# SnowCheetos/CassMantle

Hardware: AMD Instinct MI355X
Metric: SD-1.5 512^2 50-step images/sec (whole node) + p50 guess-score latency (higher is better)
Workload: dtype bf16; 1 GPU; model=sd15 UNet/VAE/CLIP (512x512, 50 steps pndm, cfg 7.5), global_batch=4, seq_len=4096, parallelism=dp1 (rooms)

## Files before the change

### cassmantle_amd/models/layers.py

```python
from __future__ import annotations

import math
import os
from typing import Optional

import torch
import torch.nn as nn

from .. import ops


def _param(shape, std, gen: Optional[torch.Generator], dtype) -> nn.Parameter:
    t = torch.randn(*shape, generator=gen, dtype=torch.float32) * std
    return nn.Parameter(t.to(dtype), requires_grad=False)


def _zeros(shape, dtype) -> nn.Parameter:
    return nn.Parameter(torch.zeros(*shape, dtype=dtype), requires_grad=False)


def _ones(shape, dtype) -> nn.Parameter:
    return nn.Parameter(torch.ones(*shape, dtype=dtype), requires_grad=False)


_GN_FUSE = os.environ.get("CASSMANTLE_GN_FUSE", "1") != "0"
_UP2 = os.environ.get("CASSMANTLE_UP2", "1") != "0"


class StatsArena:

    def __init__(self) -> None:
        self._bufs: dict = {}
        self._need: dict = {}
        self.key = None
        self.buf: Optional[torch.Tensor] = None
        self.off = 0
        self.on = False

    def begin(self, key, x: torch.Tensor) -> "StatsArena":
        self.on = x.device.type == "cuda" and ops.get_mode() == "hip" and _GN_FUSE
        self.key, self.off = key, 0
        if not self.on:
            return self
        self.buf = self._bufs.get(key)
        need = self._need.get(key, 0)
        if need and self.buf is None:
            self.buf = self._bufs[key] = torch.empty(need, device=x.device, dtype=torch.int64)
        if self.buf is not None:
            ops.zero_(self.buf)
        self.device = x.device
        return self

    def take_rows(self, rows: int) -> Optional[torch.Tensor]:
        s = self.take(1, rows)
        return None if s is None else s.view(rows, 2)

    def take(self, B: int, C: int) -> Optional[torch.Tensor]:
        if not self.on:
            return None
        n = B * C * 2
        end = self.off + n
        if self.buf is not None and end <= self.buf.numel():
            s = self.buf[self.off:end].view(B, C, 2)
        else:
            self._need[self.key] = max(self._need.get(self.key, 0), end)
            s = ops.new_stats(B, C, self.device)
        self.off = end
        return s


class Linear(nn.Module):
    def __init__(self, fin: int, fout: int, bias: bool = True, gen=None, dtype=torch.bfloat16,
                 std: Optional[float] = None):
        super().__init__()
        self.fin, self.fout = fin, fout
        self.weight = _param((fout, fin), std if std is not None else 1.0 / math.sqrt(fin), gen, dtype)
        self.bias = _param((fout,), 0.02, gen, dtype) if bias else None

    def forward(self, x, residual=None, act=None, stats=None, row_stats=None):
        return ops.linear(x, self.weight, self.bias, residual=residual, act=act, stats=stats, row_stats=row_stats)


class Conv2d(nn.Module):

    def __init__(self, cin: int, cout: int, k: int = 3, stride: int = 1, padding: Optional[int] = None,
                 bias: bool = True, gen=None, dtype=torch.bfloat16):
        super().__init__()
        self.cin, self.cout, self.k, self.stride = cin, cout, k, stride
        self.padding = (k // 2) if padding is None else padding
        self.weight = _param((cout, k, k, cin), 1.0 / math.sqrt(cin * k * k), gen, dtype)
        self.bias = _param((cout,), 0.02, gen, dtype) if bias else None

    upsampling = False
    pad_in = 0

    def _derived(self, name: str, key, fn):
        buf = self._buffers.get(name)
        if buf is None or getattr(self, "_key_" + name, None) != key or buf.device != self.weight.device:
            self.register_buffer(name, fn(), persistent=False)
            setattr(self, "_key_" + name, key)
        return self._buffers[name]

    def up2_weights(self):
        return self._derived("w4", self.weight._version, lambda: ops.fold_upsample_weights(self.weight))

    def padded_weight(self, cin: int):
        return self._derived("wpad", (self.weight._version, cin),
                             lambda: torch.nn.functional.pad(self.weight, (0, cin - self.cin)).contiguous())

    def prepare(self) -> None:
        if self.upsampling and self.k == 3 and self.cin % 64 == 0:
            self.up2_weights()
        if self.pad_in > self.cin:
            self.padded_weight(self.pad_in)

    def forward(self, x, residual=None, upsample=False, chan_bias=None, stats=None, out=None):
        if out is not None:
            w = self.padded_weight(x.shape[-1]) if x.shape[-1] > self.cin else self.weight
            return ops.conv2d(x, w, self.bias, self.stride, self.padding, residual=residual,
                              upsample=upsample, chan_bias=chan_bias, stats=stats, out=out)
        if x.shape[-1] > self.cin:
            return ops.conv2d(x, self.padded_weight(x.shape[-1]), self.bias, self.stride, self.padding,
                              residual=residual, upsample=upsample, chan_bias=chan_bias, stats=stats)
        if upsample and self.k == 3 and self.stride == 1 and _UP2 and x.device.type == "cuda" \
                and ops.get_mode() == "hip" and self.cin % 64 == 0:
            return ops.conv2d_up2(x, self.weight, self.up2_weights(), self.bias, residual=residual,
                                  chan_bias=chan_bias, stats=stats)
        if self.k == 1 and self.stride == 1 and not upsample and chan_bias is None:
            return ops.linear(x, self.weight.view(self.cout, self.cin), self.bias, residual=residual, stats=stats)
        return ops.conv2d(x, self.weight, self.bias, self.stride, self.padding, residual=residual,
                          upsample=upsample, chan_bias=chan_bias, stats=stats)


class GroupNorm(nn.Module):
    def __init__(self, groups: int, channels: int, eps: float = 1e-5, dtype=torch.bfloat16):
        super().__init__()
        self.groups, self.eps = groups, eps
        self.weight = _ones((channels,), dtype)
        self.bias = _zeros((channels,), dtype)

    def forward(self, x, silu=False, stats=None, stats2=None):
        return ops.group_norm(x, self.groups, self.weight, self.bias, self.eps, silu, stats=stats, stats2=stats2)


class LayerNorm(nn.Module):
    def __init__(self, dim: int, eps: float = 1e-5, dtype=torch.bfloat16):
        super().__init__()
        self.eps = eps
        self.weight = _ones((dim,), dtype)
        self.bias = _zeros((dim,), dtype)

    def forward(self, x):
        return ops.layer_norm(x, self.weight, self.bias, self.eps)


class SelfAttention(nn.Module):

    def __init__(self, dim: int, heads: int, gen=None, dtype=torch.bfloat16, qkv_bias=False,
                 out_bias=True):
        super().__init__()
        self.dim, self.heads = dim, heads
        self.head_dim = dim // heads
        self.to_qkv = Linear(dim, 3 * dim, bias=qkv_bias, gen=gen, dtype=dtype)
        self.to_out = Linear(dim, dim, bias=out_bias, gen=gen, dtype=dtype)

    def forward(self, x, residual=None, causal=False, kv_lens=None, fp8=False, qkv=None, kv8=None,
                row_stats=None):
        if qkv is None:
            qkv = self.to_qkv(x)
        B, N = qkv.shape[0], qkv.shape[1]
        C = self.dim
        qkv = qkv.view(B, N, 3, self.heads, self.head_dim)
        if kv8 is not None:
            assert fp8 and kv_lens is None, "kv8: fp8 self-attention without key lengths"
            o = ops.attention(qkv[:, :, 0], qkv[:, :, 1], qkv[:, :, 2], causal=causal, fp8=True, kv8=kv8)
        else:
            o = ops.attention(qkv[:, :, 0], qkv[:, :, 1], qkv[:, :, 2], causal=causal, kv_lens=kv_lens, fp8=fp8)
        return self.to_out(o.reshape(B, N, C), residual=residual, row_stats=row_stats)


class CrossAttention(nn.Module):
    def __init__(self, dim: int, ctx_dim: int, heads: int, gen=None, dtype=torch.bfloat16):
        super().__init__()
        self.dim, self.heads = dim, heads
        self.head_dim = dim // heads
        self.to_q = Linear(dim, dim, bias=False, gen=gen, dtype=dtype)
        self.to_kv = Linear(ctx_dim, 2 * dim, bias=False, gen=gen, dtype=dtype)
        self.to_out = Linear(dim, dim, bias=True, gen=gen, dtype=dtype)

    _kv = None
    _kv8 = None

    def forward(self, x, ctx, residual=None, fp8=False, q=None, row_stats=None):
        if q is None:
            q = self.to_q(x)
        B, N = q.shape[0], q.shape[1]
        C = self.dim
        q = q.view(B, N, self.heads, self.head_dim)
        kv8 = None
        if self._kv is not None and self._kv.shape[0] == B:
            kv = self._kv.view(B, self._kv.shape[1], 2, self.heads, self.head_dim)
            kv8 = self._kv8 if fp8 else None
        else:
            kv = self.to_kv(ctx).view(B, ctx.shape[1], 2, self.heads, self.head_dim)
        o = ops.attention(q, kv[:, :, 0], kv[:, :, 1], fp8=fp8, kv8=kv8)
        return self.to_out(o.reshape(B, N, C), residual=residual, row_stats=row_stats)


class GEGLUFeedForward(nn.Module):
    def __init__(self, dim: int, mult: int = 4, gen=None, dtype=torch.bfloat16):
        super().__init__()
        inner = dim * mult
        self.proj_in = Linear(dim, 2 * inner, gen=gen, dtype=dtype)
        self.proj_out = Linear(inner, dim, gen=gen, dtype=dtype)

    def forward(self, x, residual=None):
        return self.proj_out(self.proj_in(x, act="geglu"), residual=residual)
```

### cassmantle_amd/models/unet.py

```python
from __future__ import annotations

import os
from dataclasses import dataclass, field
from typing import List, Optional, Sequence, Tuple

import torch
import torch.nn as nn

from .. import ops
from .layers import (Conv2d, CrossAttention, GEGLUFeedForward, GroupNorm, LayerNorm, Linear,
                     SelfAttention, StatsArena)


@dataclass
class UNetConfig:
    in_channels: int = 4
    out_channels: int = 4
    block_out_channels: Tuple[int, ...] = (320, 640, 1280, 1280)
    down_attn: Tuple[bool, ...] = (True, True, True, False)
    transformer_depth: Tuple[int, ...] = (1, 1, 1, 1)
    mid_transformer_depth: int = 1
    layers_per_block: int = 2
    heads: Tuple[int, ...] = (8, 8, 8, 8)
    head_dim: Optional[int] = None
    cross_attention_dim: int = 768
    norm_groups: int = 32
    norm_eps: float = 1e-5
    transformer_norm_eps: float = 1e-6
    time_proj_dim: int = 320
    time_embed_dim: int = 1280
    linear_projection: bool = False
    addition_embed: bool = False
    addition_time_embed_dim: int = 256
    projection_class_embeddings_input_dim: int = 2816
    sample_size: int = 64

    def level_heads(self, i: int) -> int:
        if self.head_dim is not None:
            return self.block_out_channels[i] // self.head_dim
        return self.heads[i]


SD15_UNET = UNetConfig()
SDXL_UNET = UNetConfig(block_out_channels=(320, 640, 1280), down_attn=(False, True, True),
                       transformer_depth=(0, 2, 10), mid_transformer_depth=10, heads=(5, 10, 20),
                       head_dim=64, cross_attention_dim=2048, linear_projection=True,
                       addition_embed=True, sample_size=128)
TINY_UNET = UNetConfig(block_out_channels=(32, 64), down_attn=(True, False), transformer_depth=(1, 1),
                       heads=(2, 2), layers_per_block=1, cross_attention_dim=32, norm_groups=8,
                       time_proj_dim=32, time_embed_dim=64, sample_size=8)


class ResnetBlock(nn.Module):
    def __init__(self, cin: int, cout: int, temb: int, groups: int, eps: float, gen, dtype):
        super().__init__()
        self.norm1 = GroupNorm(groups, cin, eps, dtype)
        self.conv1 = Conv2d(cin, cout, 3, gen=gen, dtype=dtype)
        self.time_emb_proj = Linear(temb, cout, gen=gen, dtype=dtype)
        self.norm2 = GroupNorm(groups, cout, eps, dtype)
        self.conv2 = Conv2d(cout, cout, 3, gen=gen, dtype=dtype)
        self.conv_shortcut = Conv2d(cin, cout, 1, padding=0, gen=gen, dtype=dtype) if cin != cout else None

    def forward(self, x, temb_silu, tb_all=None, arena: Optional[StatsArena] = None, xs=None, xs2=None):
        pair = isinstance(x, tuple)
        B = x[0].shape[0] if pair else x.shape[0]
        cout = self.conv1.cout
        if pair:
            g = self.norm1
            h = ops.group_norm_cat(x[0], x[1], g.groups, g.weight, g.bias, g.eps, True, stats=xs, stats2=xs2)
        else:
            h = self.norm1(x, silu=True, stats=xs, stats2=xs2)
        if tb_all is not None:
            tb = tb_all[:, self._tb_off:self._tb_off + self.time_emb_proj.fout]
        else:
            tb = self.time_emb_proj(temb_silu)
        s1 = arena.take(B, cout) if arena is not None else None
        h = self.conv1(h, chan_bias=tb, stats=s1)
        h = self.norm2(h, silu=True, stats=s1)
        if pair and self.conv_shortcut is None:
            sc = torch.cat(x, dim=-1)
        elif pair:
            cs = self.conv_shortcut
            sc = ops.linear_cat(x[0], x[1], cs.weight.view(cs.cout, cs.cin), cs.bias)
        else:
            sc = self.conv_shortcut(x) if self.conv_shortcut is not None else x
        s2 = arena.take(B, cout) if arena is not None else None
        return self.conv2(h, residual=sc, stats=s2), s2


_LN_FOLD = os.environ.get("CASSMANTLE_LN_FOLD", "1") == "1"
_LN_ROWSTATS = os.environ.get("CASSMANTLE_LN_ROWSTATS", "1") == "1"
_GN_FOLD = os.environ.get("CASSMANTLE_GN_FOLD", "1") == "1"
_FF_ROWSTATS = os.environ.get("CASSMANTLE_FF_ROWSTATS", "1") == "1"


def _row_stats_wanted(x: torch.Tensor) -> bool:
    return (_LN_ROWSTATS and x.device.type == "cuda" and ops.get_mode() == "hip" and ops.LN_FOLD_MODE == 1
            and x.shape[-1] not in (320, 640) and x.shape[-1] % 8 == 0 and x.numel() // x.shape[-1] >= 1024)


_FP8_KV_EPILOGUE = os.environ.get("CASSMANTLE_FP8_KV_EPILOGUE", "1") == "1"


class BasicTransformerBlock(nn.Module):
    def __init__(self, dim: int, heads: int, ctx_dim: int, gen, dtype):
        super().__init__()
        self.norm1 = LayerNorm(dim, 1e-5, dtype)
        self.attn1 = SelfAttention(dim, heads, gen=gen, dtype=dtype)
        self.norm2 = LayerNorm(dim, 1e-5, dtype)
        self.attn2 = CrossAttention(dim, ctx_dim, heads, gen=gen, dtype=dtype)
        self.norm3 = LayerNorm(dim, 1e-5, dtype)
        self.ff = GEGLUFeedForward(dim, 4, gen=gen, dtype=dtype)

    _folds = None

    def _fold_sources(self):
        return ((self.norm1, self.attn1.to_qkv), (self.norm2, self.attn2.to_q), (self.norm3, self.ff.proj_in))

    def folds(self):
        key = tuple((n.weight._version, None if n.bias is None else n.bias._version, l.weight._version,
                     None if l.bias is None else l.bias._version) for n, l in self._fold_sources())
        buf = self._buffers.get("fold0_w")
        if buf is None or self._fold_key != key or buf.device != self.norm1.weight.device:
            for i, (n, l) in enumerate(self._fold_sources()):
                for tag, t in zip(("w", "s", "b"), ops.ln_fold(n.weight, n.bias, l.weight, l.bias)):
                    self.register_buffer(f"fold{i}_{tag}", t, persistent=False)
            self._fold_key = key
        return tuple((self._buffers[f"fold{i}_w"], self._buffers[f"fold{i}_s"], self._buffers[f"fold{i}_b"])
                     for i in range(3))

    def forward(self, x, ctx, fp8=False, arena: Optional[StatsArena] = None, xrs=None, out_stats=False):
        if _LN_FOLD and x.device.type == "cuda" and ops.get_mode() == "hip":
            f = self.folds()
            n1, n2, n3 = self.norm1, self.norm2, self.norm3
            want = arena is not None and _row_stats_wanted(x)
            rows = x.numel() // x.shape[-1]
            kv8 = None
            if fp8 and _FP8_KV_EPILOGUE and ops.kv8_ok(x, self.attn1.head_dim):
                kv8 = ops.kv8_image(x.shape[0], x.shape[1], x.shape[2], x.device)
            qkv = ops.ln_linear(x, n1.weight, n1.bias, n1.eps, self.attn1.to_qkv.weight, fold=f[0], kv8=kv8,
                                row_stats=xrs if want else None)
            r2 = arena.take_rows(rows) if want else None
            x = self.attn1(None, residual=x, fp8=fp8, qkv=qkv, kv8=kv8, row_stats=r2)
            q = ops.ln_linear(x, n2.weight, n2.bias, n2.eps, self.attn2.to_q.weight, fold=f[1], row_stats=r2)
            r3 = arena.take_rows(rows) if want else None
            x = self.attn2(None, ctx, residual=x, fp8=fp8, q=q, row_stats=r3)
            h = ops.ln_linear(x, n3.weight, n3.bias, n3.eps, self.ff.proj_in.weight, act="geglu", fold=f[2],
                              row_stats=r3)
            r4 = arena.take_rows(rows) if (want and out_stats and _FF_ROWSTATS) else None
            return self.ff.proj_out(h, residual=x, row_stats=r4), r4
        x = self.attn1(self.norm1(x), residual=x, fp8=fp8)
        x = self.attn2(self.norm2(x), ctx, residual=x, fp8=fp8)
        x = self.ff(self.norm3(x), residual=x)
        return x, None


class Transformer2D(nn.Module):
    def __init__(self, dim: int, heads: int, depth: int, ctx_dim: int, groups: int, gen, dtype):
        super().__init__()
        self.norm = GroupNorm(groups, dim, 1e-6, dtype)
        self.proj_in = Linear(dim, dim, gen=gen, dtype=dtype)
        self.transformer_blocks = nn.ModuleList(
            [BasicTransformerBlock(dim, heads, ctx_dim, gen, dtype) for _ in range(depth)])
        self.proj_out = Linear(dim, dim, gen=gen, dtype=dtype)

    def forward(self, x, ctx, fp8=False, arena: Optional[StatsArena] = None, xs=None):
        B, H, W, C = x.shape
        hrs = None
        if (_GN_FOLD and xs is not None and C == 320 and (H * W) % 256 == 0 and x.device.type == "cuda"
                and ops.get_mode() == "hip"):
            n = self.norm
            h = ops.gn_linear(x.view(B, H * W, C), xs, n.weight, n.bias, n.groups, n.eps, self.proj_in.weight,
                              self.proj_in.bias)
        else:
            h = self.norm(x, stats=xs).view(B, H * W, C)
            hrs = arena.take_rows(B * H * W) if (arena is not None and _LN_FOLD and _row_stats_wanted(h)) else None
            h = self.proj_in(h, row_stats=hrs)
        rs = hrs
        nblk = len(self.transformer_blocks)
        for i, blk in enumerate(self.transformer_blocks):
            h, rs = blk(h, ctx, fp8=fp8, arena=arena, xrs=rs, out_stats=i + 1 < nblk)
        so = arena.take(B, C) if arena is not None else None
        return self.proj_out(h, residual=x.view(B, H * W, C), stats=so).view(B, H, W, C), so


class Downsample(nn.Module):
    def __init__(self, c: int, gen, dtype):
        super().__init__()
        self.conv = Conv2d(c, c, 3, stride=2, padding=1, gen=gen, dtype=dtype)

    def forward(self, x, arena: Optional[StatsArena] = None):
        so = arena.take(x.shape[0], self.conv.cout) if arena is not None else None
        return self.conv(x, stats=so), so


class Upsample(nn.Module):
    def __init__(self, c: int, gen, dtype):
        super().__init__()
        self.conv = Conv2d(c, c, 3, gen=gen, dtype=dtype)
        self.conv.upsampling = True

    def forward(self, x, arena: Optional[StatsArena] = None):
        so = arena.take(x.shape[0], self.conv.cout) if arena is not None else None
        return self.conv(x, upsample=True, stats=so), so


class UNet(nn.Module):
    def __init__(self, cfg: UNetConfig = SD15_UNET, seed: int = 0, dtype=torch.bfloat16):
        super().__init__()
        self.cfg = cfg
        gen = torch.Generator().manual_seed(seed)
        ch = cfg.block_out_channels
        g, eps, te = cfg.norm_groups, cfg.norm_eps, cfg.time_embed_dim
        self.conv_in = Conv2d(cfg.in_channels, ch[0], 3, gen=gen, dtype=dtype)
        self.conv_in.pad_in = 8 if cfg.in_channels % 8 else 0
        self.time_linear_1 = Linear(cfg.time_proj_dim, te, gen=gen, dtype=dtype)
        self.time_linear_2 = Linear(te, te, gen=gen, dtype=dtype)
        if cfg.addition_embed:
            self.add_linear_1 = Linear(cfg.projection_class_embeddings_input_dim, te, gen=gen, dtype=dtype)
            self.add_linear_2 = Linear(te, te, gen=gen, dtype=dtype)
        self.down = nn.ModuleList()
        skip_ch: List[int] = [ch[0]]
        cur = ch[0]
        n = len(ch)
        for i in range(n):
            blk = nn.Module()
            blk.resnets = nn.ModuleList()
            blk.attentions = nn.ModuleList()
            for j in range(cfg.layers_per_block):
                blk.resnets.append(ResnetBlock(cur, ch[i], te, g, eps, gen, dtype))
                cur = ch[i]
                if cfg.down_attn[i]:
                    blk.attentions.append(Transformer2D(cur, cfg.level_heads(i), cfg.transformer_depth[i],
                                                       cfg.cross_attention_dim, g, gen, dtype))
                skip_ch.append(cur)
            blk.downsampler = Downsample(cur, gen, dtype) if i < n - 1 else None
            if i < n - 1:
                skip_ch.append(cur)
            self.down.append(blk)
        self.mid_res1 = ResnetBlock(cur, cur, te, g, eps, gen, dtype)
        self.mid_attn = Transformer2D(cur, cfg.level_heads(n - 1), cfg.mid_transformer_depth,
                                      cfg.cross_attention_dim, g, gen, dtype)
        self.mid_res2 = ResnetBlock(cur, cur, te, g, eps, gen, dtype)
        self.up = nn.ModuleList()
        rev = list(reversed(range(n)))
        for ui, i in enumerate(rev):
            blk = nn.Module()
            blk.resnets = nn.ModuleList()
            blk.attentions = nn.ModuleList()
            for j in range(cfg.layers_per_block + 1):
                sk = skip_ch.pop()
                blk.resnets.append(ResnetBlock(cur + sk, ch[i], te, g, eps, gen, dtype))
                cur = ch[i]
                if cfg.down_attn[i]:
                    blk.attentions.append(Transformer2D(cur, cfg.level_heads(i), cfg.transformer_depth[i],
                                                       cfg.cross_attention_dim, g, gen, dtype))
            blk.upsampler = Upsample(cur, gen, dtype) if ui < n - 1 else None
            self.up.append(blk)
        self.conv_norm_out = GroupNorm(g, cur, eps, dtype)
        self.conv_out = Conv2d(cur, cfg.out_channels, 3, gen=gen, dtype=dtype)
        self._arena = StatsArena()

    def time_embed(self, t: torch.Tensor, added: Optional[dict] = None) -> torch.Tensor:
        dt = self.time_linear_1.weight.dtype
        tp = ops.timestep_embedding(t, self.cfg.time_proj_dim, out_dtype=dt)
        h = self.time_linear_1(tp, act="silu")
        if not (self.cfg.addition_embed and added is not None):
            return self.time_linear_2(h, act="silu")
        emb = self.time_linear_2(h)
        tid = added["time_ids"]
        B = tid.shape[0]
        te = ops.timestep_embedding(tid.reshape(-1), self.cfg.addition_time_embed_dim).reshape(B, -1)
        a_in = ops.concat_last(added["text_embeds"], te)
        emb = self.add_linear_2(self.add_linear_1(a_in, act="silu"), residual=emb)
        return ops.silu_(emb)

    def resnets(self) -> List[ResnetBlock]:
        return [m for m in self.modules() if isinstance(m, ResnetBlock)]

    def cross_attns(self) -> List[CrossAttention]:
        ca = self.__dict__.get("_ca_list")
        if ca is None:
            ca = self.__dict__["_ca_list"] = [m for m in self.modules() if isinstance(m, CrossAttention)]
        return ca

    def fuse_projections(self) -> None:
        rs = self.resnets()
        off = 0
        for r in rs:
            r._tb_off = off
            off += r.time_emb_proj.fout
        self.register_buffer("_tb_w", torch.cat([r.time_emb_proj.weight for r in rs], 0).contiguous(), persistent=False)
        self.register_buffer("_tb_b", torch.cat([r.time_emb_proj.bias for r in rs], 0).contiguous(), persistent=False)
        ca = self.cross_attns()
        off = 0
        for m in ca:
            m._kv_off = off
            off += m.to_kv.fout
        self.register_buffer("_kv_w", torch.cat([m.to_kv.weight for m in ca], 0).contiguous() if ca else None,
                             persistent=False)
        self._kv_bufs: dict = {}
        self._fused = True

    def prepare(self) -> "UNet":
        self.fuse_projections()
        for m in self.modules():
            if isinstance(m, BasicTransformerBlock):
                m.folds()
            elif isinstance(m, Conv2d):
                m.prepare()
        return self

    def set_context(self, ctx: Optional[torch.Tensor], fp8: bool = False) -> None:
        if not getattr(self, "_fused", False):
            self.fuse_projections()
        ca = self.cross_attns()
        if ctx is None or self._kv_w is None:
            for m in ca:
                m._kv = None
                m._kv8 = None
            return
        key = (*ctx.shape[:-1], self._kv_w.shape[0])
        buf = self._kv_bufs.get(key)
        if buf is None or buf.device != ctx.device:
            self._kv_bufs[key] = buf = ops.linear(ctx, self._kv_w)
        else:
            ops.linear(ctx, self._kv_w, out=buf)
        for m in ca:
            m._kv = buf[:, :, m._kv_off:m._kv_off + m.to_kv.fout]
            m._kv8 = None
            if fp8 and m.head_dim == 64 and ops._use_hip(buf):
                bufs8 = m.__dict__.setdefault("_kv8_bufs", {})
                kv = m._kv.view(buf.shape[0], buf.shape[1], 2, m.heads, m.head_dim)
                k8 = (key, str(buf.device))
                bufs8[k8] = m._kv8 = ops.pack_kv_fp8(kv[:, :, 0], kv[:, :, 1], out=bufs8.get(k8))

    def time_table(self, tsteps: torch.Tensor, nb: int, added: Optional[dict] = None,
                   t_rep: Optional[torch.Tensor] = None, rep_ids: Optional[torch.Tensor] = None):
        if not getattr(self, "_fused", False):
            self.fuse_projections()
        E = tsteps.shape[0]
        t = t_rep if t_rep is not None else tsteps.float().repeat_interleave(nb)
        rep = None
        if added is not None:
            if rep_ids is not None and ops._use_hip(added["text_embeds"]):
                rep = {"text_embeds": ops.gather_add(added["text_embeds"], rep_ids),
                       "time_ids": added["time_ids_rep"] if "time_ids_rep" in added
                       else added["time_ids"].repeat(E, 1)}
            else:
                rep = {k: v.repeat(E, *([1] * (v.dim() - 1))) for k, v in added.items() if k != "time_ids_rep"}
        temb = self.time_embed(t, rep)
        tb = ops.linear(temb, self._tb_w, self._tb_b)
        return temb.view(E, nb, -1), tb.view(E, nb, -1)

    def forward(self, x: torch.Tensor, t: Optional[torch.Tensor], ctx: torch.Tensor,
                added: Optional[dict] = None, fp8: bool = False, time_cond=None,
                out: Optional[torch.Tensor] = None) -> torch.Tensor:
        if not getattr(self, "_fused", False):
            self.fuse_projections()
        if time_cond is not None:
            temb, tb = time_cond
        else:
            temb = self.time_embed(t, added)
            tb = ops.linear(temb, self._tb_w, self._tb_b)
        ar = self._arena.begin(tuple(x.shape), x)
        B = x.shape[0]
        hs = ar.take(B, self.conv_in.cout)
        h = self.conv_in(x, stats=hs)
        skips = [(h, hs)]
        for blk in self.down:
            for j, res in enumerate(blk.resnets):
                h, hs = res(h, temb, tb, ar, hs)
                if len(blk.attentions):
                    h, hs = blk.attentions[j](h, ctx, fp8, ar, hs)
                skips.append((h, hs))
            if blk.downsampler is not None:
                h, hs = blk.downsampler(h, ar)
                skips.append((h, hs))
        h, hs = self.mid_res1(h, temb, tb, ar, hs)
        h, hs = self.mid_attn(h, ctx, fp8, ar, hs)
        h, hs = self.mid_res2(h, temb, tb, ar, hs)
        for blk in self.up:
            for j, res in enumerate(blk.resnets):
                sk, sks = skips.pop()
                two = hs is not None and sks is not None
                h, hs = res((h, sk), temb, tb, ar, hs if two else None, sks if two else None)
                if len(blk.attentions):
                    h, hs = blk.attentions[j](h, ctx, fp8, ar, hs)
            if blk.upsampler is not None:
                h, hs = blk.upsampler(h, ar)
        h = self.conv_norm_out(h, silu=True, stats=hs)
        return self.conv_out(h, out=out)


def _silu(x: torch.Tensor) -> torch.Tensor:
    return torch.nn.functional.silu(x.float()).to(x.dtype)
```

### cassmantle_amd/ops/__init__.py

```python
from __future__ import annotations

import math
import os
import weakref
from typing import List, Optional

import torch

from . import reference as ref
from ._ext import ext, ext_available, ext_error

_MODE = os.environ.get("CASSMANTLE_OPS", "hip").lower()


def set_mode(mode: str) -> None:
    global _MODE
    assert mode in ("hip", "torch")
    _MODE = mode


def get_mode() -> str:
    return _MODE


def _use_hip(t: torch.Tensor) -> bool:
    if t.device.type != "cuda":
        return False
    if _MODE == "torch":
        return False
    if not ext_available():
        raise RuntimeError(
            "cassmantle_amd HIP extension is not loaded on a GPU device "
            f"({ext_error()}); run `python -m cassmantle_amd.build` or set CASSMANTLE_OPS=torch "
            "explicitly for the stock-PyTorch baseline")
    return True


_TUNE_PATH = os.path.join(os.path.dirname(os.path.abspath(__file__)), "gemm_tuning.json")
_RECORD: Optional[list] = None
_tune_loaded = False
_DIAG_TWICE = os.environ.get("CASSMANTLE_DIAG_TWICE", "0") == "1"
if _DIAG_TWICE and os.environ.get("CASSMANTLE_DIAG_TWICE_ACK") != "wrong-results":
    raise RuntimeError("CASSMANTLE_DIAG_TWICE=1 makes every GEMM / conv result WRONG (epilogue "
                       "statistics and residuals applied twice); it is a timing diagnostic for "
                       "tools/diag_twice.py only: also set CASSMANTLE_DIAG_TWICE_ACK=wrong-results")


def load_gemm_tuning(path: Optional[str] = None) -> int:
    global _tune_loaded
    if os.environ.get("CASSMANTLE_GEMM_TUNE", "1") == "0" or not ext_available():
        return 0
    if _tune_loaded and path is None:
        return ext().gemm_tune_size()
    import json
    p = path or os.environ.get("CASSMANTLE_GEMM_TUNE_PATH") or _TUNE_PATH
    _tune_loaded = True
    if not os.path.exists(p):
        return 0
    with open(p) as f:
        data = json.load(f)
    for e in data.get("entries", []):
        ext().gemm_tune_set(e["key"], int(e["cfg"]), int(e["split"]))
    return ext().gemm_tune_size()


def record_gemms(on: bool) -> Optional[list]:
    global _RECORD
    if on:
        _RECORD = []
        ext().gemm_record_keys(True)
        return _RECORD
    rec, _RECORD = _RECORD, None
    ext().gemm_record_keys(False)
    return rec


_PF_SERIAL = os.environ.get("CASSMANTLE_PF_SERIAL", "0") == "1"


def _launch(fn, *args, **kw):
    if not _tune_loaded:
        load_gemm_tuning()
    if _PF_SERIAL:
        prefetch(args[2] if fn is ext().gemm_cat else args[1])
    if _DIAG_TWICE:
        fn(*args, **kw)
    fn(*args, **kw)
    if _RECORD is not None:
        call = lambda: fn(*args, **kw)
        call.fn, call.args, call.kw = fn, args, kw
        _RECORD.append((ext().gemm_last_key(), call))


_ACT = {None: 0, "none": 0, "gelu": 1, "silu": 2, "quick_gelu": 3, "geglu": 4, "gelu_tanh": 5, "swiglu": 6}


STAT_SCALE = (2.0 ** 24, 2.0 ** 16)


def h2d(t: torch.Tensor, device) -> torch.Tensor:
    device = torch.device(device)
    if device.type != "cuda":
        return t.to(device)
    return t.pin_memory().to(device, non_blocking=True)


def new_stats(B: int, C: int, device) -> torch.Tensor:
    return zero_(torch.empty((B, C, 2), device=device, dtype=torch.int64))


def stats_to_float(stats: torch.Tensor) -> torch.Tensor:
    sc = torch.tensor([1.0 / STAT_SCALE[0], 1.0 / STAT_SCALE[1]], dtype=torch.float64, device=stats.device)
    return stats.double() * sc


def channel_stats_ref(y: torch.Tensor, stats: torch.Tensor) -> None:
    B, C = y.shape[0], y.shape[-1]
    yf = y.reshape(B, -1, C).double()
    stats[..., 0] += torch.round(yf.sum(1) * STAT_SCALE[0]).to(torch.int64)
    stats[..., 1] += torch.round((yf * yf).sum(1) * STAT_SCALE[1]).to(torch.int64)


def channel_stats(y: torch.Tensor, stats: torch.Tensor) -> None:
    if _use_hip(y):
        ext().channel_stats(y.contiguous(), stats)
    else:
        channel_stats_ref(y, stats)


def linear(x: torch.Tensor, w: torch.Tensor, bias: Optional[torch.Tensor] = None,
           residual: Optional[torch.Tensor] = None, act: Optional[str] = None,
           stats: Optional[torch.Tensor] = None, out: Optional[torch.Tensor] = None,
           row_stats: Optional[torch.Tensor] = None) -> torch.Tensor:
    if not _use_hip(x):
        if x.device.type == "cuda":
            y = _torch_linear(x, w, bias, residual, act)
        else:
            y = ref.linear(x, w, bias, residual, act)
        if stats is not None:
            channel_stats_ref(y, stats)
        return y if out is None else out.copy_(y)
    K = x.shape[-1]
    x2 = x.reshape(-1, K)
    if not x2.is_contiguous():
        x2 = x2.contiguous()
    N = w.shape[0] // 2 if act in ("geglu", "swiglu") else w.shape[0]
    if out is None:
        out = torch.empty((x2.shape[0], N), device=x.device, dtype=x.dtype)
    else:
        assert out.is_contiguous() and out.dtype == x.dtype and out.numel() == x2.shape[0] * N, "linear: bad out"
    o2 = out.view(x2.shape[0], N)
    r2 = residual.reshape(-1, N) if residual is not None else None
    hw = x2.shape[0] // x.shape[0] if stats is not None else 0
    if row_stats is not None:
        _launch(ext().gemm, x2, w, bias, r2, o2, _ACT[act], stats, hw, row_stats=row_stats)
    else:
        _launch(ext().gemm, x2, w, bias, r2, o2, _ACT[act], stats, hw)
    return out.view(*x.shape[:-1], N)


def gn_linear(x: torch.Tensor, stats: torch.Tensor, gamma: torch.Tensor, beta: torch.Tensor, groups: int,
              eps: float, w: torch.Tensor, bias: Optional[torch.Tensor] = None,
              residual: Optional[torch.Tensor] = None) -> torch.Tensor:
    B, C = x.shape[0], x.shape[-1]
    if not _use_hip(x):
        xn = group_norm(x, groups, gamma, beta, eps, False, stats=stats)
        return linear(xn, w, bias, residual=residual)
    rows = x.numel() // C
    x2 = x.reshape(rows, C)
    if not x2.is_contiguous():
        x2 = x2.contiguous()
    N = w.shape[0]
    out = torch.empty((rows, N), device=x.device, dtype=x.dtype)
    r2 = residual.reshape(rows, N) if residual is not None else None
    _launch(ext().gemm, x2, w, bias, r2, out, 0, None, 0, gn_stats=stats, gn_gamma=gamma, gn_beta=beta,
            gn_groups=int(groups), gn_hw=rows // B, gn_eps=float(eps))
    return out.reshape(*x.shape[:-1], N)


def ln_fold(ln_weight: torch.Tensor, ln_bias: Optional[torch.Tensor], w: torch.Tensor,
            bias: Optional[torch.Tensor] = None):
    wf = (w.float() * ln_weight.float()[None, :]).to(w.dtype).contiguous()
    wsum = wf.float().sum(1).contiguous()
    b = torch.zeros(w.shape[0], device=w.device, dtype=torch.float32)
    if ln_bias is not None:
        b = b + w.float() @ ln_bias.float()
    if bias is not None:
        b = b + bias.float()
    return wf, wsum, b.to(w.dtype).contiguous()


def row_stats(x: torch.Tensor, eps: float) -> torch.Tensor:
    if not _use_hip(x):
        xf = x.float().reshape(-1, x.shape[-1])
        mean = xf.mean(-1)
        var = xf.var(-1, unbiased=False)
        return torch.stack([mean, (var + eps).rsqrt()], dim=-1)
    out = torch.empty((x.numel() // x.shape[-1], 2), device=x.device, dtype=torch.float32)
    ext().row_stats(x.contiguous(), out, float(eps))
    return out


LN_FOLD_MODE = int(os.environ.get("CASSMANTLE_LN_FOLD_MODE", "1"))


def ln_linear(x: torch.Tensor, ln_weight: torch.Tensor, ln_bias: Optional[torch.Tensor], eps: float,
              w: torch.Tensor, bias: Optional[torch.Tensor] = None, residual: Optional[torch.Tensor] = None,
              act: Optional[str] = None, fold=None, kv8: Optional[torch.Tensor] = None,
              row_stats: Optional[torch.Tensor] = None) -> torch.Tensor:
    K = x.shape[-1]
    rows = x.numel() // K
    if fold is None or not _use_hip(x) or rows <= 8 or K % 8 or (LN_FOLD_MODE == 2 and K not in (320, 640)):
        y = linear(layer_norm(x, ln_weight, ln_bias, eps), w, bias, residual=residual, act=act)
        if kv8 is not None:
            _pack_qkv8(y, kv8)
        return y
    wf, wsum, bf = fold
    x2 = x.reshape(rows, K)
    if not x2.is_contiguous():
        x2 = x2.contiguous()
    N = wf.shape[0] // 2 if act in ("geglu", "swiglu") else wf.shape[0]
    out = torch.empty((rows, N), device=x.device, dtype=x.dtype)
    r2 = residual.reshape(rows, N) if residual is not None else None
    fx = {"ln_rows_fx": row_stats} if row_stats is not None else {}
    if kv8 is not None:
        C = N // 3
        _launch(ext().gemm, x2, wf, bf, r2, out, _ACT[act], None, 0, None, wsum, float(eps), kv8, C,
                int(x.shape[-2]), C // 64, **fx)
    elif fx:
        _launch(ext().gemm, x2, wf, bf, r2, out, _ACT[act], None, 0, None, wsum, float(eps), **fx)
    else:
        _launch(ext().gemm, x2, wf, bf, r2, out, _ACT[act], None, 0, None, wsum, float(eps))
    return out.reshape(*x.shape[:-1], N)


def kv8_image(B: int, N: int, C: int, device) -> torch.Tensor:
    return torch.empty(2 * B * N * C, device=device, dtype=torch.uint8)


def kv8_ok(x: torch.Tensor, head_dim: int) -> bool:
    return (_use_hip(x) and x.dim() == 3 and head_dim == 64 and x.shape[1] % 64 == 0 and x.shape[-1] % 64 == 0
            and x.shape[-1] not in (320, 640))


def _pack_qkv8(y: torch.Tensor, kv8: torch.Tensor) -> None:
    B, N, C3 = y.shape
    C = C3 // 3
    qkv = y.view(B, N, 3, C // 64, 64)
    pack_kv_fp8(qkv[:, :, 1], qkv[:, :, 2], out=kv8)


def linear_cat(x: torch.Tensor, x2: torch.Tensor, w: torch.Tensor, bias: Optional[torch.Tensor] = None,
               residual: Optional[torch.Tensor] = None, stats: Optional[torch.Tensor] = None) -> torch.Tensor:
    Ca, K = x.shape[-1], x.shape[-1] + x2.shape[-1]
    rows = x.numel() // Ca
    if not _use_hip(x) or Ca % 64 or K % 64 or rows <= 8:
        return linear(torch.cat([x, x2], dim=-1), w, bias, residual=residual, stats=stats)
    N = w.shape[0]
    out = torch.empty((rows, N), device=x.device, dtype=x.dtype)
    r2 = residual.reshape(rows, N) if residual is not None else None
    hw = rows // x.shape[0] if stats is not None else 0
    _launch(ext().gemm_cat, x.reshape(rows, Ca).contiguous(), x2.reshape(rows, K - Ca).contiguous(), w, bias, r2, out,
            stats, hw)
    return out.reshape(*x.shape[:-1], N)


def _torch_linear(x, w, bias, residual, act):
    import torch.nn.functional as F
    y = F.linear(x, w, bias)
    if act == "geglu":
        h, g = y.chunk(2, dim=-1)
        y = h * F.gelu(g)
    elif act == "swiglu":
        h, g = y.chunk(2, dim=-1)
        y = h * F.silu(g)
    elif act == "gelu":
        y = F.gelu(y)
    elif act == "gelu_tanh":
        y = F.gelu(y, approximate="tanh")
    elif act == "silu":
        y = F.silu(y)
    elif act == "quick_gelu":
        y = y * torch.sigmoid(1.702 * y)
    if residual is not None:
        y = y + residual
    return y


def conv2d(x: torch.Tensor, w: torch.Tensor, bias: Optional[torch.Tensor] = None, stride: int = 1,
           padding: int = 1, residual: Optional[torch.Tensor] = None, upsample: bool = False,
           chan_bias: Optional[torch.Tensor] = None, stats: Optional[torch.Tensor] = None,
           out: Optional[torch.Tensor] = None) -> torch.Tensor:
    if not _use_hip(x):
        if x.device.type == "cuda":
            y = _torch_conv(x, w, bias, stride, padding, residual, upsample, chan_bias)
        else:
            y = ref.conv2d(x, w, bias, stride, padding, residual, upsample, chan_bias)
        if stats is not None:
            channel_stats_ref(y, stats)
        return y if out is None else out.copy_(y)
    B, H, W, Cin = x.shape
    Cout, kh, kw, _ = w.shape
    if Cin % 8 != 0:
        pad = 8 - Cin % 8
        x = torch.nn.functional.pad(x, (0, pad))
        w = torch.nn.functional.pad(w, (0, pad))
        Cin += pad
    Hi, Wi = (2 * H, 2 * W) if upsample else (H, W)
    Ho = (Hi + 2 * padding - kh) // stride + 1
    Wo = (Wi + 2 * padding - kw) // stride + 1
    if out is None:
        out = torch.empty((B, Ho, Wo, Cout), device=x.device, dtype=x.dtype)
    else:
        assert out.shape == (B, Ho, Wo, Cout) and out.dtype == x.dtype and out.is_contiguous(), "conv2d: bad out"
    _launch(ext().conv2d, x.contiguous(), w, bias, residual, chan_bias, out, stride, padding, int(upsample), stats)
    return out


_UP2_ROWS = ([[1.0, 0.0, 0.0], [0.0, 1.0, 1.0]], [[1.0, 1.0, 0.0], [0.0, 0.0, 1.0]])


def fold_upsample_weights(w: torch.Tensor) -> torch.Tensor:
    wf = w.float()
    outs = []
    for a in (0, 1):
        ra = torch.tensor(_UP2_ROWS[a], device=w.device)
        for b in (0, 1):
            rb = torch.tensor(_UP2_ROWS[b], device=w.device)
            outs.append(torch.einsum("tk,sl,oklc->otsc", ra, rb, wf))
    return torch.stack(outs).to(w.dtype).contiguous()


def conv2d_up2(x: torch.Tensor, w: torch.Tensor, w4: Optional[torch.Tensor] = None,
               bias: Optional[torch.Tensor] = None, residual: Optional[torch.Tensor] = None,
               chan_bias: Optional[torch.Tensor] = None, stats: Optional[torch.Tensor] = None) -> torch.Tensor:
    B, H, W, Cin = x.shape
    if not _use_hip(x) or Cin % 64 or w.shape[1] != 3:
        return conv2d(x, w, bias, 1, 1, residual=residual, upsample=True, chan_bias=chan_bias, stats=stats)
    if w4 is None:
        w4 = fold_upsample_weights(w)
    out = torch.empty((B, 2 * H, 2 * W, w.shape[0]), device=x.device, dtype=x.dtype)
    _launch(ext().conv2d_up2, x.contiguous(), w4, bias, residual, chan_bias, out, stats)
    return out


def _torch_conv(x, w, bias, stride, padding, residual, upsample, chan_bias):
    import torch.nn.functional as F
    xi = x.permute(0, 3, 1, 2)
    if upsample:
        xi = F.interpolate(xi, scale_factor=2.0, mode="nearest")
    wi = w.permute(0, 3, 1, 2)
    y = F.conv2d(xi.contiguous(memory_format=torch.channels_last),
                 wi.contiguous(memory_format=torch.channels_last), bias, stride=stride, padding=padding)
    y = y.permute(0, 2, 3, 1)
    if chan_bias is not None:
        y = y + chan_bias[:, None, None, :]
    if residual is not None:
        y = y + residual
    return y.contiguous()


def _group_norm_from_stats_ref(x, num_groups, weight, bias, eps, silu, stats):
    B, C = x.shape[0], x.shape[-1]
    S = x.numel() // (B * C)
    st = stats_to_float(stats).view(B, num_groups, C // num_groups, 2).sum(2)
    n = S * (C // num_groups)
    mean = st[..., 0] / n
    var = (st[..., 1] / n - mean * mean).clamp_min(0)
    rstd = (var + eps).rsqrt()
    cg = C // num_groups
    mean_c = mean.repeat_interleave(cg, 1).float()
    rstd_c = rstd.repeat_interleave(cg, 1).float()
    shape = [B] + [1] * (x.dim() - 2) + [C]
    y = (x.float() - mean_c.view(shape)) * rstd_c.view(shape) * weight.float() + bias.float()
    if silu:
        y = torch.nn.functional.silu(y)
    return y.to(x.dtype)


def group_norm(x: torch.Tensor, num_groups: int, weight: torch.Tensor, bias: torch.Tensor,
               eps: float, silu: bool = False, stats: Optional[torch.Tensor] = None,
               stats2: Optional[torch.Tensor] = None) -> torch.Tensor:
    if stats is not None:
        if not _use_hip(x):
            st = stats if stats2 is None else torch.cat([stats, stats2], dim=1)
            return _group_norm_from_stats_ref(x, num_groups, weight, bias, eps, silu, st)
        out = torch.empty_like(x)
        ext().group_norm_stats(x.contiguous(), stats, stats2, weight, bias, out, num_groups, float(eps), int(silu))
        return out
    if not _use_hip(x):
        if x.device.type == "cuda":
            import torch.nn.functional as F
            B, C = x.shape[0], x.shape[-1]
            xi = x.reshape(B, -1, C).transpose(1, 2)
            y = F.group_norm(xi, num_groups, weight, bias, eps)
            if silu:
                y = F.silu(y)
            return y.transpose(1, 2).reshape(x.shape).contiguous()
        return ref.group_norm(x, num_groups, weight, bias, eps, silu)
    out = torch.empty_like(x)
    ext().group_norm(x.contiguous(), weight, bias, out, num_groups, float(eps), int(silu))
    return out


def group_norm_cat(x: torch.Tensor, x2: torch.Tensor, num_groups: int, weight: torch.Tensor, bias: torch.Tensor,
                   eps: float, silu: bool = False, stats: Optional[torch.Tensor] = None,
                   stats2: Optional[torch.Tensor] = None) -> torch.Tensor:
    if stats is None or stats2 is None or not _use_hip(x) or x.shape[-1] % 8 or x2.shape[-1] % 8:
        return group_norm(torch.cat([x, x2], dim=-1), num_groups, weight, bias, eps, silu, stats=stats, stats2=stats2)
    out = torch.empty((*x.shape[:-1], x.shape[-1] + x2.shape[-1]), device=x.device, dtype=x.dtype)
    ext().group_norm_cat(x.contiguous(), x2.contiguous(), stats, stats2, weight, bias, out, num_groups, float(eps),
                         int(silu))
    return out


def layer_norm(x: torch.Tensor, weight: torch.Tensor, bias: Optional[torch.Tensor], eps: float) -> torch.Tensor:
    if not _use_hip(x):
        if x.device.type == "cuda":
            import torch.nn.functional as F
            return F.layer_norm(x, (x.shape[-1],), weight, bias, eps)
        return ref.layer_norm(x, weight, bias, eps)
    out = torch.empty_like(x)
    ext().layer_norm(x.contiguous(), weight, bias, out, float(eps))
    return out


def embed_layer_norm(word: torch.Tensor, ids: torch.Tensor, pos: torch.Tensor, add: Optional[torch.Tensor],
                     weight: torch.Tensor, bias: Optional[torch.Tensor], eps: float) -> torch.Tensor:
    B, T = ids.shape
    if not _use_hip(word):
        x = word[ids] + pos[:T][None]
        if add is not None:
            x = x + add
        return layer_norm(x, weight, bias, eps)
    out = torch.empty((B, T, word.shape[-1]), device=word.device, dtype=word.dtype)
    ext().embed_layer_norm(word, ids.contiguous().view(-1), pos, T, add, weight, bias, out, float(eps))
    return out


def rms_norm(x: torch.Tensor, weight: torch.Tensor, eps: float) -> torch.Tensor:
    if not _use_hip(x):
        return ref.rms_norm(x, weight, eps)
    out = torch.empty_like(x)
    ext().rms_norm(x.contiguous(), weight, out, float(eps))
    return out


def rms_linear(x: torch.Tensor, gamma: torch.Tensor, eps: float, w: torch.Tensor,
               bias: Optional[torch.Tensor] = None, residual: Optional[torch.Tensor] = None,
               act: Optional[str] = None) -> torch.Tensor:
    K = x.shape[-1]
    rows = x.numel() // K
    if not _use_hip(x) or rows > 8 or K % 8:
        return linear(rms_norm(x, gamma, eps), w, bias, residual=residual, act=act)
    x2 = x.reshape(rows, K)
    if not x2.is_contiguous():
        x2 = x2.contiguous()
    N = w.shape[0] // 2 if act in ("geglu", "swiglu") else w.shape[0]
    out = torch.empty((rows, N), device=x.device, dtype=x.dtype)
    r2 = residual.reshape(rows, N) if residual is not None else None
    ext().gemm_rms(x2, gamma, float(eps), w, bias, r2, out, _ACT[act])
    return out.reshape(*x.shape[:-1], N)


def rope_kv(qkv: torch.Tensor, pos0: torch.Tensor, q_out: torch.Tensor, k_cache: torch.Tensor,
            v_cache: torch.Tensor, heads: int, kv_heads: int, theta: float) -> None:
    if not _use_hip(qkv):
# ... 597 lines not shown
```

### cassmantle_amd/ops/csrc/bindings.cpp

```cpp
#include <torch/extension.h>
#include <atomic>
#include <ATen/hip/HIPContext.h>
#include <c10/hip/HIPStream.h>
#include <hip/hip_ext.h>

#include "gemm_tiles.h"
#include "jpeg_layout.h"
#include "kernels.h"

namespace {

hipStream_t cur_stream() { return c10::hip::getCurrentHIPStream().stream(); }

#define CHECK_DEV(t) TORCH_CHECK((t).is_cuda(), #t " must be a GPU tensor")
#define CHECK_BF16(t) TORCH_CHECK((t).scalar_type() == at::kBFloat16, #t " must be bf16")
#define CHECK_CONTIG(t) TORCH_CHECK((t).is_contiguous(), #t " must be contiguous")

const uint16_t* bptr(const at::Tensor& t) { return reinterpret_cast<const uint16_t*>(t.data_ptr()); }
uint16_t* bptr_mut(at::Tensor& t) { return reinterpret_cast<uint16_t*>(t.data_ptr()); }
const uint16_t* opt_bptr(const c10::optional<at::Tensor>& t) {
  if (!t.has_value() || !t->defined()) return nullptr;
  CHECK_DEV(*t);
  CHECK_BF16(*t);
  CHECK_CONTIG(*t);
  return bptr(*t);
}

long long* opt_stats(const c10::optional<at::Tensor>& t, long long images, int N) {
  if (!t.has_value() || !t->defined()) return nullptr;
  CHECK_DEV(*t);
  CHECK_CONTIG(*t);
  TORCH_CHECK(t->scalar_type() == at::kLong && t->numel() == images * N * 2,
              "stats must be a zeroed int64 fixed-point [images, N, 2] tensor (ops.new_stats)");
  return reinterpret_cast<long long*>(t->data_ptr<int64_t>());
}

static std::atomic<int> g_raster[2] = {{-1}, {-1}};
static void raster_from_env() {
  static const bool once = [] {
    const char* e = getenv("CASSMANTLE_GEMM_RASTER");
    int a = 0, b = -1;
    if (e != nullptr) {
      if (sscanf(e, "%d,%d", &a, &b) < 2) b = a;
    } else {
      b = 0;
    }
    int expect = -1;
    g_raster[0].compare_exchange_strong(expect, a);
    expect = -1;
    g_raster[1].compare_exchange_strong(expect, b);
    return true;
  }();
  (void)once;
}
void gemm_set_raster(int64_t plain, int64_t gated) {
  raster_from_env();
  g_raster[0].store((int)plain);
  g_raster[1].store((int)gated);
}

void run_gemm(GemmArgs& p, const at::Tensor& like) {
  raster_from_env();
  p.raster = g_raster[(p.act == 4 || p.act == 6) ? 1 : 0].load(std::memory_order_relaxed);
  TORCH_CHECK(p.stats == nullptr || (p.N % 8 == 0 && p.ldc == p.N),
              "gemm/conv2d stats: the output channel count must be a multiple of 8 (GroupNorm consumers)");
  const GemmPlan plan = gemm_plan(p);
  p.cfg = plan.cfg;
  p.split = plan.split;
  if (p.kv8 != nullptr) p.split = 1;
  long long* post_stats = nullptr;
  if (p.stats != nullptr && (p.out_f32 || p.M <= 8 || (p.batch != 1 && !p.parity) || p.act == 4 || p.act == 6)) {
    post_stats = p.stats;
    p.stats = nullptr;
  }
  if (p.split > 1) {
    auto ws = at::empty({(long long)p.split * p.batch * p.M * p.N}, like.options().dtype(at::kFloat));
    launch_gemm(p, ws.data_ptr<float>(), cur_stream());
  } else {
    launch_gemm(p, nullptr, cur_stream());
  }
  if (post_stats != nullptr)
    launch_channel_stats(reinterpret_cast<const uint16_t*>(p.C), post_stats, p.M / p.stats_hw, p.stats_hw, p.N,
                         cur_stream());
}

void gemm(const at::Tensor& x, const at::Tensor& w, const c10::optional<at::Tensor>& bias,
          const c10::optional<at::Tensor>& residual, at::Tensor& out, int64_t act,
          const c10::optional<at::Tensor>& stats, int64_t stats_hw,
          const c10::optional<at::Tensor>& ln_rows, const c10::optional<at::Tensor>& ln_wsum, double ln_eps,
          const c10::optional<at::Tensor>& kv8, int64_t kv8_col0, int64_t kv8_ntok, int64_t kv8_hk,
          const c10::optional<at::Tensor>& ln_rows_fx, const c10::optional<at::Tensor>& row_stats,
          const c10::optional<at::Tensor>& gn_stats, const c10::optional<at::Tensor>& gn_gamma,
          const c10::optional<at::Tensor>& gn_beta, int64_t gn_groups, int64_t gn_hw, double gn_eps) {
  CHECK_DEV(x); CHECK_BF16(x); CHECK_BF16(w); CHECK_CONTIG(w); CHECK_CONTIG(out);
  TORCH_CHECK(x.dim() == 2 && w.dim() == 2 && out.dim() == 2, "gemm: 2-D operands expected");
  TORCH_CHECK(x.stride(1) == 1, "gemm: x rows must be contiguous");
  GemmArgs p;
  p.A = bptr(x); p.W = bptr(w); p.bias = opt_bptr(bias); p.residual = opt_bptr(residual);
  p.M = (int)x.size(0); p.K = (int)x.size(1); p.N = (int)out.size(1); p.Nw = (int)w.size(0);
  p.lda = (int)x.stride(0); p.ldc = p.N; p.act = (int)act;
  TORCH_CHECK(w.size(1) == p.K, "gemm: K mismatch");
  TORCH_CHECK(out.size(0) == p.M, "gemm: M mismatch");
  if (act == 4 || act == 6) {
    TORCH_CHECK(p.Nw == 2 * p.N && p.K % 8 == 0 && (p.N % 4 == 0 || (p.M >= 1 && p.M <= 8 && p.lda % 8 == 0)),
                "geglu/swiglu: W must be [2N,K], K%8==0, N%4==0 (any N for <= 8 rows with lda%8==0)");
  } else {
    TORCH_CHECK(p.Nw == p.N, "gemm: N mismatch");
  }
  if (residual.has_value() && residual->defined()) TORCH_CHECK(residual->numel() == out.numel(), "gemm: residual shape");
  if (out.scalar_type() == at::kFloat) {
    p.out_f32 = 1;
  } else {
    CHECK_BF16(out);
  }
  p.C = out.data_ptr();
  if (kv8.has_value() && kv8->defined()) {
    CHECK_DEV(*kv8); CHECK_CONTIG(*kv8);
    TORCH_CHECK(kv8->scalar_type() == at::kByte && kv8_ntok > 0 && kv8_ntok % 64 == 0 && p.M % kv8_ntok == 0 &&
                    kv8_hk > 0 && kv8_col0 % 8 == 0 && kv8_col0 + 128 * kv8_hk == p.N && act == 0 &&
                    !p.out_f32 && !(residual.has_value() && residual->defined()) && !(stats.has_value() && stats->defined()),
                "gemm kv8: uint8 image, 64-aligned tokens per image, K|V heads ending the output, plain epilogue");
    TORCH_CHECK(kv8->numel() == 2LL * p.M * kv8_hk * 64, "gemm kv8: image size");
    p.kv8 = kv8->data_ptr<uint8_t>();
    p.kv8_col0 = (int)kv8_col0; p.kv8_ntok = (int)kv8_ntok; p.kv8_hk = (int)kv8_hk;
  }
  if (stats.has_value() && stats->defined()) {
    TORCH_CHECK(stats_hw > 0 && p.M % stats_hw == 0, "gemm: stats_hw must divide the rows");
    p.stats_hw = (int)stats_hw;
    p.stats = opt_stats(stats, p.M / stats_hw, p.N);
  }
  if (gn_stats.has_value() && gn_stats->defined()) {
    TORCH_CHECK(gn_gamma.has_value() && gn_beta.has_value() && gn_groups > 0 && gn_hw > 0 && p.M % gn_hw == 0,
                "gemm: gn_stats needs gamma, beta, groups and rows per image");
    CHECK_DEV(*gn_stats); CHECK_CONTIG(*gn_stats);
    TORCH_CHECK(gn_stats->scalar_type() == at::kLong && gn_stats->numel() == 2LL * (p.M / gn_hw) * p.K,
                "gemm: gn_stats int64 [images, K, 2]");
    TORCH_CHECK(!(ln_wsum.has_value() && ln_wsum->defined()) && !(row_stats.has_value() && row_stats->defined()) &&
                    !(kv8.has_value() && kv8->defined()) && !(stats.has_value() && stats->defined()),
                "gemm: gn_stats excludes LayerNorm folds, row / GroupNorm output statistics and kv8");
    p.gn_stats = reinterpret_cast<const long long*>(gn_stats->data_ptr<int64_t>());
    p.gn_gamma = opt_bptr(gn_gamma);
    p.gn_beta = opt_bptr(gn_beta);
    p.gn_groups = (int)gn_groups;
    p.gn_hw = (int)gn_hw;
    p.gn_eps = (float)gn_eps;
    if (gemm_areg_ok(p)) {
      run_gemm(p, out);
      return;
    }
    TORCH_CHECK(x.is_contiguous() && p.K % 8 == 0 && p.K % gn_groups == 0, "gemm gn fallback: contiguous rows");
    at::Tensor xn = at::empty_like(x);
    launch_group_norm_cs(bptr(x), nullptr, p.gn_stats, p.K, nullptr, p.gn_gamma, p.gn_beta, bptr_mut(xn),
                         p.M / gn_hw, gn_hw, p.K, (int)gn_groups, (float)gn_eps, 0, cur_stream());
    p.gn_stats = nullptr; p.gn_gamma = nullptr; p.gn_beta = nullptr;
    p.A = bptr(xn);
    run_gemm(p, out);
    return;
  }
  if (row_stats.has_value() && row_stats->defined()) {
    CHECK_DEV(*row_stats); CHECK_CONTIG(*row_stats);
    TORCH_CHECK(row_stats->scalar_type() == at::kLong && row_stats->numel() == 2LL * p.M,
                "gemm: row_stats zeroed int64 [M, 2]");
    TORCH_CHECK(p.stats == nullptr && p.kv8 == nullptr && !p.out_f32 && p.batch == 1 && p.M > 8 && p.N % 8 == 0 &&
                    p.ldc % 8 == 0 && p.K % 8 == 0 && p.lda % 8 == 0,
                "gemm: row_stats needs the LDS-staged bf16 epilogue (no GroupNorm stats / kv8, N % 8 == 0, M > 8)");
    p.row_stats = reinterpret_cast<long long*>(row_stats->data_ptr<int64_t>());
  }
  if (ln_rows_fx.has_value() && ln_rows_fx->defined()) {
    TORCH_CHECK(ln_wsum.has_value() && ln_wsum->defined() && ln_eps > 0 && !(ln_rows.has_value() && ln_rows->defined()),
                "gemm: ln_rows_fx needs ln_wsum and ln_eps, and excludes ln_rows");
    CHECK_DEV(*ln_rows_fx); CHECK_CONTIG(*ln_rows_fx); CHECK_DEV(*ln_wsum); CHECK_CONTIG(*ln_wsum);
    TORCH_CHECK(ln_rows_fx->scalar_type() == at::kLong && ln_rows_fx->numel() == 2LL * p.M, "gemm: ln_rows_fx int64 [M, 2]");
    TORCH_CHECK(ln_wsum->scalar_type() == at::kFloat && ln_wsum->numel() == p.Nw, "gemm: ln_wsum fp32 [Nw]");
    TORCH_CHECK(p.M > 8 && p.K % 8 == 0 && p.lda % 8 == 0 && !p.out_f32, "gemm: folded LayerNorm needs the MFMA path");
    p.ln_rows_fx = reinterpret_cast<const long long*>(ln_rows_fx->data_ptr<int64_t>());
    p.ln_wsum = ln_wsum->data_ptr<float>();
    p.ln_eps = (float)ln_eps;
    run_gemm(p, out);
    return;
  }
  if (ln_rows.has_value() && ln_rows->defined()) {
    TORCH_CHECK(ln_wsum.has_value() && ln_wsum->defined(), "gemm: ln_rows needs ln_wsum");
    CHECK_DEV(*ln_rows); CHECK_CONTIG(*ln_rows); CHECK_DEV(*ln_wsum); CHECK_CONTIG(*ln_wsum);
    TORCH_CHECK(ln_rows->scalar_type() == at::kFloat && ln_rows->numel() == 2LL * p.M, "gemm: ln_rows fp32 [M, 2]");
    TORCH_CHECK(ln_wsum->scalar_type() == at::kFloat && ln_wsum->numel() == p.Nw, "gemm: ln_wsum fp32 [Nw]");
    TORCH_CHECK(p.M > 8 && p.K % 8 == 0 && p.lda % 8 == 0, "gemm: folded LayerNorm needs the MFMA path (M > 8)");
    TORCH_CHECK(!p.out_f32 || p.act == 0, "gemm: folded LayerNorm with fp32 output supports no activation");
    p.ln_rows = ln_rows->data_ptr<float>();
    p.ln_wsum = ln_wsum->data_ptr<float>();
  } else if (ln_wsum.has_value() && ln_wsum->defined() && ln_eps > 0) {
    CHECK_DEV(*ln_wsum); CHECK_CONTIG(*ln_wsum);
    TORCH_CHECK(ln_wsum->scalar_type() == at::kFloat && ln_wsum->numel() == p.Nw, "gemm: ln_wsum fp32 [Nw]");
    TORCH_CHECK(p.M > 8 && p.K % 8 == 0 && p.lda % 8 == 0 && !p.out_f32, "gemm: folded LayerNorm needs the MFMA path");
    p.ln_wsum = ln_wsum->data_ptr<float>();
    p.ln_eps = (float)ln_eps;
    static const bool inkernel = [] { const char* e = getenv("CASSMANTLE_LN_INKERNEL"); return !(e && e[0] == '0'); }();
    if (!inkernel || !gemm_areg_ok(p)) {
      TORCH_CHECK(x.is_contiguous() && p.K <= 4096, "gemm: folded LayerNorm row statistics need contiguous rows");
      at::Tensor rows = at::empty({p.M, 2}, x.options().dtype(at::kFloat));
      launch_row_stats(bptr(x), rows.data_ptr<float>(), p.M, p.K, (float)ln_eps, cur_stream());
      p.ln_rows = rows.data_ptr<float>();
      p.ln_eps = 0.f;
      run_gemm(p, out);
      return;
    }
  }
  run_gemm(p, out);
}

void row_stats(const at::Tensor& x, at::Tensor& out, double eps) {
  CHECK_DEV(x); CHECK_BF16(x); CHECK_CONTIG(x); CHECK_CONTIG(out);
  const int D = (int)x.size(-1);
  TORCH_CHECK(D % 8 == 0 && D <= 4096, "row_stats: D % 8 == 0 and D <= 4096");
  TORCH_CHECK(out.scalar_type() == at::kFloat && out.numel() == 2 * (x.numel() / D), "row_stats: out fp32 [rows, 2]");
  launch_row_stats(bptr(x), out.data_ptr<float>(), x.numel() / D, D, (float)eps, cur_stream());
}

void gemm_cat(const at::Tensor& x, const at::Tensor& x2, const at::Tensor& w, const c10::optional<at::Tensor>& bias,
              const c10::optional<at::Tensor>& residual, at::Tensor& out, const c10::optional<at::Tensor>& stats,
              int64_t stats_hw) {
  CHECK_DEV(x); CHECK_BF16(x); CHECK_CONTIG(x); CHECK_BF16(x2); CHECK_CONTIG(x2); CHECK_BF16(w); CHECK_CONTIG(w);
  CHECK_BF16(out); CHECK_CONTIG(out);
  TORCH_CHECK(x.dim() == 2 && x2.dim() == 2 && w.dim() == 2 && out.dim() == 2 && x.size(0) == x2.size(0),
              "gemm_cat: 2-D operands with equal rows expected");
  GemmArgs p;
  p.A = bptr(x); p.A2 = bptr(x2); p.W = bptr(w); p.bias = opt_bptr(bias); p.residual = opt_bptr(residual);
  p.M = (int)x.size(0); p.ka = (int)x.size(1); p.K = p.ka + (int)x2.size(1);
  p.N = (int)out.size(1); p.Nw = (int)w.size(0);
  p.lda = p.ka; p.lda2 = (int)x2.size(1); p.ldc = p.N;
  TORCH_CHECK(w.size(1) == p.K && p.Nw == p.N && out.size(0) == p.M, "gemm_cat: shape mismatch");
  TORCH_CHECK(p.ka % 64 == 0 && p.K % 64 == 0 && p.M > 8, "gemm_cat: Ca and K must be multiples of 64, M > 8");
  const long long lim = (1LL << 31) - 1;
  TORCH_CHECK(x.numel() * 2 <= lim && x2.numel() * 2 <= lim && w.numel() * 2 <= lim, "gemm_cat: operand too large");
  if (residual.has_value() && residual->defined()) TORCH_CHECK(residual->numel() == out.numel(), "gemm_cat: residual shape");
  p.C = out.data_ptr();
  if (stats.has_value() && stats->defined()) {
    TORCH_CHECK(stats_hw > 0 && p.M % stats_hw == 0, "gemm_cat: stats_hw must divide the rows");
    p.stats_hw = (int)stats_hw;
    p.stats = opt_stats(stats, p.M / stats_hw, p.N);
  }
  run_gemm(p, out);
}

void gemm_rms(const at::Tensor& x, const at::Tensor& gamma, double eps, const at::Tensor& w,
              const c10::optional<at::Tensor>& bias, const c10::optional<at::Tensor>& residual, at::Tensor& out,
              int64_t act) {
  CHECK_DEV(x); CHECK_BF16(x); CHECK_BF16(gamma); CHECK_CONTIG(gamma); CHECK_BF16(w); CHECK_CONTIG(w);
  CHECK_CONTIG(out);
  TORCH_CHECK(x.dim() == 2 && x.stride(1) == 1 && x.size(0) <= 8, "gemm_rms: x [<=8, K] rows contiguous");
  GemmArgs p;
  p.A = bptr(x); p.W = bptr(w); p.bias = opt_bptr(bias); p.residual = opt_bptr(residual);
  p.M = (int)x.size(0); p.K = (int)x.size(1); p.N = (int)out.size(1); p.Nw = (int)w.size(0);
  p.lda = (int)x.stride(0); p.ldc = p.N; p.act = (int)act;
  p.rms_gamma = bptr(gamma); p.rms_eps = (float)eps;
  TORCH_CHECK(gamma.numel() == p.K && w.size(1) == p.K, "gemm_rms: K mismatch");
  TORCH_CHECK(p.Nw == ((act == 4 || act == 6) ? 2 * p.N : p.N), "gemm_rms: N mismatch");
  if (out.scalar_type() == at::kFloat) p.out_f32 = 1;
  else CHECK_BF16(out);
  p.C = out.data_ptr();
  TORCH_CHECK(launch_gemv(p, cur_stream()), "gemm_rms: shape not supported by the GEMV path (K % 8)");
}

void conv2d(const at::Tensor& x, const at::Tensor& w, const c10::optional<at::Tensor>& bias,
            const c10::optional<at::Tensor>& residual, const c10::optional<at::Tensor>& chan_bias, at::Tensor& out,
            int64_t stride, int64_t pad, int64_t upsample, const c10::optional<at::Tensor>& stats) {
  CHECK_DEV(x); CHECK_BF16(x); CHECK_CONTIG(x); CHECK_BF16(w); CHECK_CONTIG(w); CHECK_CONTIG(out); CHECK_BF16(out);
  TORCH_CHECK(x.dim() == 4 && w.dim() == 4 && out.dim() == 4, "conv2d: NHWC 4-D tensors expected");
  GemmArgs p;
  p.conv = 1;
  p.A = bptr(x); p.W = bptr(w); p.bias = opt_bptr(bias); p.residual = opt_bptr(residual);
  if (chan_bias.has_value() && chan_bias->defined()) {
    CHECK_DEV(*chan_bias);
    CHECK_BF16(*chan_bias);
    TORCH_CHECK(chan_bias->dim() == 2 && chan_bias->stride(1) == 1, "conv2d: chan_bias must be [B, Cout] rows");
    p.chan_bias = bptr(*chan_bias);
    p.ldcb = (int)chan_bias->stride(0);
  }
  p.IH = (int)x.size(1); p.IW = (int)x.size(2); p.Cin = (int)x.size(3);
  p.ksize = (int)w.size(1);
  TORCH_CHECK(w.size(2) == p.ksize && w.size(3) == p.Cin, "conv2d: weight must be [Cout,k,k,Cin]");
  p.Ho = (int)out.size(1); p.Wo = (int)out.size(2);
  p.N = (int)out.size(3); p.Nw = (int)w.size(0);
  TORCH_CHECK(p.Nw == p.N && out.size(0) == x.size(0), "conv2d: shape mismatch");
  p.M = (int)(x.size(0) * p.Ho * p.Wo);
  p.K = p.ksize * p.ksize * p.Cin;
  p.lda = p.Cin; p.ldc = p.N;
  p.stride = (int)stride; p.pad = (int)pad; p.upsample = (int)upsample;
  if (residual.has_value() && residual->defined()) TORCH_CHECK(residual->numel() == out.numel(), "conv2d: residual shape");
  if (chan_bias.has_value() && chan_bias->defined())
    TORCH_CHECK(chan_bias->size(0) == x.size(0) && chan_bias->size(1) == p.N, "conv2d: chan_bias must be [B, Cout]");
  p.C = out.data_ptr();
  p.stats_hw = p.Ho * p.Wo;
  p.stats = opt_stats(stats, x.size(0), p.N);
  run_gemm(p, out);
}

void conv2d_up2(const at::Tensor& x, const at::Tensor& w4, const c10::optional<at::Tensor>& bias,
                const c10::optional<at::Tensor>& residual, const c10::optional<at::Tensor>& chan_bias, at::Tensor& out,
                const c10::optional<at::Tensor>& stats) {
  CHECK_DEV(x); CHECK_BF16(x); CHECK_CONTIG(x); CHECK_BF16(w4); CHECK_CONTIG(w4); CHECK_CONTIG(out); CHECK_BF16(out);
  TORCH_CHECK(x.dim() == 4 && w4.dim() == 5 && w4.size(0) == 4 && w4.size(2) == 2 && w4.size(3) == 2 &&
              w4.size(4) == x.size(3), "conv2d_up2: x [B,H,W,Cin], w4 [4,Cout,2,2,Cin]");
  TORCH_CHECK(out.dim() == 4 && out.size(0) == x.size(0) && out.size(1) == 2 * x.size(1) &&
              out.size(2) == 2 * x.size(2) && out.size(3) == w4.size(1), "conv2d_up2: out [B,2H,2W,Cout]");
  GemmArgs p;
  p.conv = 1;
  p.parity = 1;
  p.A = bptr(x); p.W = bptr(w4); p.bias = opt_bptr(bias); p.residual = opt_bptr(residual);
  if (chan_bias.has_value() && chan_bias->defined()) {
    CHECK_DEV(*chan_bias);
    CHECK_BF16(*chan_bias);
    TORCH_CHECK(chan_bias->dim() == 2 && chan_bias->stride(1) == 1 && chan_bias->size(0) == x.size(0) &&
                chan_bias->size(1) == out.size(3), "conv2d_up2: chan_bias must be [B, Cout] rows");
    p.chan_bias = bptr(*chan_bias);
    p.ldcb = (int)chan_bias->stride(0);
  }
  p.IH = (int)x.size(1); p.IW = (int)x.size(2); p.Cin = (int)x.size(3);
  p.ksize = 2; p.stride = 1; p.pad = 1; p.upsample = 0;
  p.Ho = p.IH; p.Wo = p.IW;
  p.N = (int)out.size(3); p.Nw = p.N;
  p.M = (int)(x.size(0) * p.Ho * p.Wo);
  p.K = 4 * p.Cin;
  p.lda = p.Cin; p.ldc = p.N;
  p.batch = 4;
  p.sA = 0; p.sW = (long long)p.N * 4 * p.Cin; p.sC = 0;
  TORCH_CHECK(p.Cin % 64 == 0, "conv2d_up2: Cin % 64 == 0 (buffer-DMA conv path)");
  if (residual.has_value() && residual->defined()) TORCH_CHECK(residual->numel() == out.numel(), "conv2d_up2: residual shape");
  p.C = out.data_ptr();
  p.stats_hw = p.Ho * p.Wo;
  p.stats = opt_stats(stats, x.size(0), p.N);
  run_gemm(p, out);
}

void bmm_nt(const at::Tensor& a, const at::Tensor& b, at::Tensor& out, double alpha) {
  CHECK_DEV(a); CHECK_BF16(a); CHECK_BF16(b); CHECK_CONTIG(out);
  TORCH_CHECK(a.dim() == 3 && b.dim() == 3 && out.dim() == 3, "bmm_nt: 3-D operands");
  TORCH_CHECK(a.stride(2) == 1 && b.stride(2) == 1, "bmm_nt: K must be contiguous");
  GemmArgs p;
  p.A = bptr(a); p.W = bptr(b);
  p.batch = (int)a.size(0);
  p.M = (int)a.size(1); p.K = (int)a.size(2); p.N = (int)b.size(1); p.Nw = p.N;
  p.lda = (int)a.stride(1); p.ldw = (int)b.stride(1); p.sA = a.stride(0); p.sW = b.stride(0);
  p.ldc = p.N; p.sC = (long long)p.M * p.N;
  p.alpha = (float)alpha;
  if (out.scalar_type() == at::kFloat) {
    p.out_f32 = 1;
  } else {
    CHECK_BF16(out);
  }
  p.C = out.data_ptr();
  run_gemm(p, out);
}

void group_norm(const at::Tensor& x, const at::Tensor& gamma, const at::Tensor& beta, at::Tensor& out,
                int64_t groups, double eps, int64_t silu) {
  CHECK_DEV(x); CHECK_BF16(x); CHECK_CONTIG(x); CHECK_BF16(gamma); CHECK_BF16(beta); CHECK_CONTIG(out);
  const int B = (int)x.size(0);
  const int C = (int)x.size(-1);
  const long long S = x.numel() / ((long long)B * C);
  TORCH_CHECK(C % 8 == 0 && C % groups == 0, "group_norm: C must be a multiple of 8 and of groups");
  auto ws = at::empty({group_norm_workspace(B, S, C)}, x.options().dtype(at::kFloat));
  launch_group_norm(bptr(x), bptr(gamma), bptr(beta), bptr_mut(out), ws.data_ptr<float>(), B, S, C, (int)groups,
                    (float)eps, (int)silu, cur_stream());
}

void group_norm_stats(const at::Tensor& x, const at::Tensor& stats_a, const c10::optional<at::Tensor>& stats_b,
                      const at::Tensor& gamma, const at::Tensor& beta, at::Tensor& out, int64_t groups, double eps,
                      int64_t silu) {
  CHECK_DEV(x); CHECK_BF16(x); CHECK_CONTIG(x); CHECK_BF16(gamma); CHECK_BF16(beta); CHECK_CONTIG(out);
  const int B = (int)x.size(0);
  const int C = (int)x.size(-1);
  const long long S = x.numel() / ((long long)B * C);
  TORCH_CHECK(C % 8 == 0 && C % groups == 0, "group_norm_stats: C must be a multiple of 8 and of groups");
  TORCH_CHECK(stats_a.scalar_type() == at::kLong && stats_a.is_contiguous() && stats_a.dim() == 3 &&
              stats_a.size(0) == B && stats_a.size(2) == 2, "group_norm_stats: stats_a must be int64 [B, Ca, 2]");
  const int Ca = (int)stats_a.size(1);
  const long long* sb = nullptr;
  if (stats_b.has_value() && stats_b->defined()) {
    TORCH_CHECK(stats_b->scalar_type() == at::kLong && stats_b->is_contiguous() && stats_b->dim() == 3 &&
                stats_b->size(0) == B && stats_b->size(1) == C - Ca && stats_b->size(2) == 2,
                "group_norm_stats: stats_b must be int64 [B, C - Ca, 2]");
    sb = reinterpret_cast<const long long*>(stats_b->data_ptr<int64_t>());
  } else {
    TORCH_CHECK(Ca == C, "group_norm_stats: stats_a must cover every channel");
  }
  launch_group_norm_cs(bptr(x), nullptr, reinterpret_cast<const long long*>(stats_a.data_ptr<int64_t>()), Ca, sb, bptr(gamma), bptr(beta), bptr_mut(out), B, S, C,
                       (int)groups, (float)eps, (int)silu, cur_stream());
}

void group_norm_cat(const at::Tensor& x, const at::Tensor& x2, const at::Tensor& stats_a, const at::Tensor& stats_b,
                    const at::Tensor& gamma, const at::Tensor& beta, at::Tensor& out, int64_t groups, double eps,
                    int64_t silu) {
  CHECK_DEV(x); CHECK_BF16(x); CHECK_CONTIG(x); CHECK_BF16(x2); CHECK_CONTIG(x2); CHECK_BF16(gamma); CHECK_BF16(beta);
  CHECK_CONTIG(out); CHECK_BF16(out);
  const int B = (int)x.size(0);
  const int Ca = (int)x.size(-1), Cb = (int)x2.size(-1), C = Ca + Cb;
  const long long S = x.numel() / ((long long)B * Ca);
  TORCH_CHECK(x2.size(0) == B && x2.numel() == (long long)B * S * Cb && out.numel() == (long long)B * S * C &&
              out.size(-1) == C, "group_norm_cat: shapes must agree on batch and pixels");
  TORCH_CHECK(Ca % 8 == 0 && Cb % 8 == 0 && C % groups == 0, "group_norm_cat: channel counts");
  TORCH_CHECK(stats_a.scalar_type() == at::kLong && stats_a.is_contiguous() && stats_a.numel() == (long long)B * Ca * 2 &&
              stats_b.scalar_type() == at::kLong && stats_b.is_contiguous() && stats_b.numel() == (long long)B * Cb * 2,
              "group_norm_cat: int64 [B, C, 2] statistics of both inputs expected");
  launch_group_norm_cs(bptr(x), bptr(x2), reinterpret_cast<const long long*>(stats_a.data_ptr<int64_t>()), Ca, reinterpret_cast<const long long*>(stats_b.data_ptr<int64_t>()), bptr(gamma),
                       bptr(beta), bptr_mut(out), B, S, C, (int)groups, (float)eps, (int)silu, cur_stream());
}

void channel_stats(const at::Tensor& x, at::Tensor& stats) {
  CHECK_DEV(x); CHECK_BF16(x); CHECK_CONTIG(x);
  const int B = (int)x.size(0);
  const int C = (int)x.size(-1);
  const long long S = x.numel() / ((long long)B * C);
  TORCH_CHECK(C % 8 == 0, "channel_stats: C % 8 == 0");
  launch_channel_stats(bptr(x), opt_stats(stats, B, C), B, S, C, cur_stream());
}

void layer_norm(const at::Tensor& x, const at::Tensor& gamma, const c10::optional<at::Tensor>& beta, at::Tensor& out,
                double eps) {
  CHECK_DEV(x); CHECK_BF16(x); CHECK_CONTIG(x); CHECK_BF16(gamma); CHECK_CONTIG(out);
  const int D = (int)x.size(-1);
  TORCH_CHECK(D % 8 == 0 && D <= 4096, "layer_norm: D % 8 == 0 and D <= 4096");
  launch_layer_norm(bptr(x), bptr(gamma), opt_bptr(beta), bptr_mut(out), x.numel() / D, D, (float)eps, cur_stream());
}

void embed_layer_norm(const at::Tensor& word, const at::Tensor& ids, const at::Tensor& pos, int64_t seq,
                      const c10::optional<at::Tensor>& add, const at::Tensor& gamma,
                      const c10::optional<at::Tensor>& beta, at::Tensor& out, double eps) {
  CHECK_DEV(word); CHECK_BF16(word); CHECK_CONTIG(word); CHECK_DEV(ids); CHECK_CONTIG(ids);
  CHECK_BF16(pos); CHECK_CONTIG(pos); CHECK_BF16(gamma); CHECK_BF16(out); CHECK_CONTIG(out);
  TORCH_CHECK(ids.scalar_type() == at::kLong, "embed_layer_norm: int64 ids");
  const int D = (int)word.size(-1);
  TORCH_CHECK(D % 8 == 0 && D <= 4096 && pos.size(-1) == D && out.numel() == ids.numel() * D,
              "embed_layer_norm: D % 8 == 0, D <= 4096, out [rows, D]");
  TORCH_CHECK(seq > 0 && pos.size(0) >= seq, "embed_layer_norm: position table shorter than seq");
  launch_embed_layer_norm(bptr(word), reinterpret_cast<const long long*>(ids.data_ptr<int64_t>()), bptr(pos), (int)seq,
                          opt_bptr(add), bptr(gamma), opt_bptr(beta), bptr_mut(out), ids.numel(), D, (float)eps,
                          cur_stream());
}

static AttnArgs attn_args(const at::Tensor& q, const at::Tensor& k, const at::Tensor& v, at::Tensor& out, double scale,
                          int64_t causal, const c10::optional<at::Tensor>& kv_lens) {
  CHECK_DEV(q); CHECK_BF16(q); CHECK_BF16(k); CHECK_BF16(v); CHECK_BF16(out);
  TORCH_CHECK(q.dim() == 4 && k.dim() == 4 && v.dim() == 4 && out.dim() == 4, "attention: [B,N,H,d] tensors");
  TORCH_CHECK(q.stride(3) == 1 && k.stride(3) == 1 && v.stride(3) == 1 && out.stride(3) == 1,
              "attention: head dim must be contiguous");
  AttnArgs a;
  a.q = bptr(q); a.k = bptr(k); a.v = bptr(v); a.o = bptr_mut(out);
// ... 476 lines not shown
  if (l.refusal != nullptr) throw py::value_error(l.refusal);
  using namespace py::literals;
  return py::dict("nb"_a = l.g.nb, "mx"_a = l.g.mx, "my"_a = l.g.my, "mcus"_a = l.g.mcus, "restart"_a = l.g.restart,
                  "per"_a = l.g.per, "nint"_a = l.g.nint, "coef"_a = l.coef, "work"_a = l.work, "blk"_a = l.blk,
                  "scratch"_a = l.scratch, "hopt"_a = l.hopt, "hdrs"_a = l.hdrs, "stride"_a = l.stride,
                  "hdr_cap"_a = l.hdr_cap, "prefix"_a = l.prefix, "err"_a = l.err, "hdr_lens"_a = l.hdr_lens,
                  "lens"_a = l.lens, "offs"_a = l.offs, "slack"_a = l.slack);
}

void jpeg_reconstruct(const at::Tensor& coef, const at::Tensor& tables, at::Tensor& planes, at::Tensor& out,
                      int64_t H, int64_t W, int64_t s420) {
  CHECK_DEV(coef); CHECK_CONTIG(coef); CHECK_DEV(tables); CHECK_CONTIG(tables); CHECK_DEV(planes);
  CHECK_CONTIG(planes); CHECK_DEV(out); CHECK_CONTIG(out);
  TORCH_CHECK(tables.scalar_type() == at::kInt && tables.numel() == 128 + 544, "jpeg: tables int32 [672]");
  TORCH_CHECK(H > 0 && W > 0 && H < 65536 && W < 65536, "jpeg: image sides must be in 1..65535");
  TORCH_CHECK(out.scalar_type() == at::kByte && out.dim() == 4 && out.size(0) > 0 && out.size(1) == H &&
              out.size(2) == W && out.size(3) == 3, "jpeg: out uint8 [B, H, W, 3]");
  const JpegGeometry g = jpeg_geometry(H, W, s420 != 0, 0);
  JpegArgs a;
  a.B = (int)out.size(0); a.H = (int)H; a.W = (int)W;
  a.nb = g.nb; a.mx = g.mx; a.my = g.my;
  const long long ncoef = a.B * g.mcus * g.nb * 64;
  TORCH_CHECK(coef.scalar_type() == at::kShort && coef.numel() == ncoef, "jpeg: coef int16 [B, mcus, blocks, 64]");
  TORCH_CHECK(planes.scalar_type() == at::kByte && planes.numel() == ncoef, "jpeg: planes uint8 [B * mcus * blocks * 64]");
  TORCH_CHECK((double)a.B * a.H * ((a.W + 3) / 4) < 256.0 * 2147483647.0, "jpeg: batch too large for one launch");
  a.qtab = tables.data_ptr<int>();
  a.coef = coef.data_ptr<int16_t>();
  a.planes = planes.data_ptr<uint8_t>();
  a.dec = out.data_ptr<uint8_t>();
  TORCH_CHECK(reinterpret_cast<uintptr_t>(a.planes) % 4 == 0 && reinterpret_cast<uintptr_t>(a.dec) % 4 == 0 &&
              reinterpret_cast<uintptr_t>(a.coef) % 4 == 0, "jpeg: buffers must be 4-byte aligned");
  launch_jpeg_reconstruct(a, cur_stream());
}

struct JpegDecodeCall {
  JpegArgs a;
  JpegDecodeIn d;
  JpegDecodeLayout l;
};

JpegDecodeCall jpeg_decode_args(const at::Tensor& staged, int64_t nbytes, const at::Tensor& tables, at::Tensor& buf,
                                int64_t B, int64_t H, int64_t W, int64_t s420, int64_t restart, int64_t extra = -1,
                                int64_t ngroups = 0) {
  const bool chunked = extra >= 0;
  CHECK_DEV(staged); CHECK_CONTIG(staged); CHECK_DEV(tables); CHECK_CONTIG(tables); CHECK_DEV(buf); CHECK_CONTIG(buf);
  JpegDecodeCall c;
  const JpegDecodeLayout& l = c.l = jpeg_decode_layout(B, H, W, s420 != 0, restart, chunked);
  TORCH_CHECK(l.refusal == nullptr, l.refusal);
  TORCH_CHECK(tables.scalar_type() == at::kInt && tables.numel() == 128 + 544 + 1024,
              "jpeg: decode tables int32 [672 + 1024]");
  TORCH_CHECK(buf.scalar_type() == at::kShort && buf.numel() == l.buf,
              chunked ? "jpeg: buf int16 [B * mcus * blocks * 64 + 16]" : "jpeg: buf int16 [B * mcus * blocks * 64 + 8]");
  const bool bytes_ok = nbytes >= 0 && nbytes < 4294967295LL && staged.scalar_type() == at::kByte;
  if (chunked) {
    TORCH_CHECK(bytes_ok && extra % 4 == 0 && extra >= l.staged_min(nbytes) && staged.numel() >= extra + l.sync_bytes(ngroups),
                "jpeg: staged uint8 [8 * B * intervals + nbytes | 4 * B * intervals + 8 * groups]");
  } else {
    TORCH_CHECK(bytes_ok && staged.numel() >= l.staged_min(nbytes), "jpeg: staged uint8 [8 * B * intervals + nbytes]");
  }
  TORCH_CHECK(reinterpret_cast<uintptr_t>(staged.data_ptr()) % 4 == 0 && reinterpret_cast<uintptr_t>(buf.data_ptr()) % 16 == 0,
              "jpeg: staged 4-byte aligned, buf 16-byte aligned");
  JpegArgs& a = c.a;
  a.B = (int)B; a.H = (int)H; a.W = (int)W;
  a.nb = l.g.nb; a.mx = l.g.mx; a.my = l.g.my;
  a.restart = (int)l.g.restart;
  a.nint = (int)l.g.nint;
  a.coef = buf.data_ptr<int16_t>();
  JpegDecodeIn& d = c.d;
  d.intervals = reinterpret_cast<const uint32_t*>(staged.data_ptr<uint8_t>());
  d.bytes = staged.data_ptr<uint8_t>() + 8 * l.nivals;
  d.nbytes = (uint32_t)nbytes;
  d.tables = reinterpret_cast<const uint32_t*>(tables.data_ptr<int>()) + 128 + 544;
  d.status = reinterpret_cast<unsigned long long*>(a.coef + l.ncoef);
  d.zero_bytes = l.buf * 2;
  return c;
}

void jpeg_entropy_decode(const at::Tensor& staged, int64_t nbytes, const at::Tensor& tables, at::Tensor& buf,
                         int64_t B, int64_t H, int64_t W, int64_t s420, int64_t restart) {
  const JpegDecodeCall c = jpeg_decode_args(staged, nbytes, tables, buf, B, H, W, s420, restart);
  launch_jpeg_entropy_decode(c.a, c.d, cur_stream());
}

void jpeg_entropy_decode_chunked(const at::Tensor& staged, int64_t nbytes, const at::Tensor& tables, at::Tensor& buf,
                                 int64_t B, int64_t H, int64_t W, int64_t s420, int64_t restart, int64_t extra,
                                 int64_t ngroups, int64_t chunk, int64_t threads) {
  TORCH_CHECK(extra >= 0 && ngroups >= 0, "jpeg: staged uint8 [8 * B * intervals + nbytes | 4 * B * intervals + 8 * groups]");
  const JpegDecodeCall c = jpeg_decode_args(staged, nbytes, tables, buf, B, H, W, s420, restart, extra, ngroups);
  TORCH_CHECK(chunk >= 16 && chunk % 16 == 0 && chunk < (1LL << 28), "jpeg: chunk bytes a multiple of 16");
  TORCH_CHECK(threads >= 64 && threads <= 1024 && threads % 64 == 0, "jpeg: 64..1024 lanes per workgroup");
  TORCH_CHECK(ngroups <= c.l.nivals, "jpeg: at most one group per interval");
  JpegSyncIn y;
  y.lane0 = reinterpret_cast<const uint32_t*>(staged.data_ptr<uint8_t>() + extra);
  y.groups = y.lane0 + c.l.nivals;
  y.ngroups = (int)ngroups;
  y.cb = (uint32_t)chunk;
  y.words = reinterpret_cast<uint32_t*>(c.a.coef + c.l.ncoef + 4);
  launch_jpeg_entropy_decode_chunked(c.a, c.d, y, (int)threads, cur_stream());
}

void blur_pil_check(const at::Tensor& img, const at::Tensor& out) {
  CHECK_DEV(img); CHECK_CONTIG(img); CHECK_DEV(out); CHECK_CONTIG(out);
  TORCH_CHECK(img.scalar_type() == at::kByte && img.dim() == 3 && img.size(2) == 3 && img.numel() > 0,
              "blur_pil: img uint8 [H, W, 3]");
  TORCH_CHECK(img.size(0) < 65536 && img.size(1) < 65536, "blur_pil: image sides must be below 65536");
  TORCH_CHECK(out.scalar_type() == at::kByte && out.dim() == 4 && out.size(0) > 0 && out.size(1) == img.size(0) &&
              out.size(2) == img.size(1) && out.size(3) == 3, "blur_pil: out uint8 [N, H, W, 3]");
  TORCH_CHECK(out.device() == img.device(), "blur_pil: img and out on one device");
  const char* i0 = static_cast<const char*>(img.data_ptr());
  const char* o0 = static_cast<const char*>(out.data_ptr());
  TORCH_CHECK(i0 + img.numel() <= o0 || o0 + out.numel() <= i0, "blur_pil: out overlaps img");
}

void blur_pil_tiled(const at::Tensor& img, const at::Tensor& table, at::Tensor& out, int64_t rmax) {
  blur_pil_check(img, out);
  CHECK_DEV(table); CHECK_CONTIG(table);
  TORCH_CHECK(table.scalar_type() == at::kInt && table.dim() == 2 && table.size(1) == 4 && table.size(0) > 0 &&
              table.size(0) < 65536 && table.device() == img.device(), "blur_pil: table int32 [n, 4], n < 65536");
  TORCH_CHECK(rmax >= 0 && rmax <= blur_pil_max_tiled_radius(), "blur_pil: the tiled kernel covers box radius <= ",
              blur_pil_max_tiled_radius());
  launch_blur_pil_tiled(img.data_ptr<uint8_t>(), (int)img.size(0), (int)img.size(1), table.data_ptr<int>(),
                        (int)table.size(0), (int)rmax, (int)out.size(0), out.data_ptr<uint8_t>(), cur_stream());
}

void blur_pil_general(const at::Tensor& img, at::Tensor& out, int64_t slot, at::Tensor& scratch, int64_t r,
                      int64_t ww, int64_t fw) {
  blur_pil_check(img, out);
  blur_pil_check(img, scratch);
  TORCH_CHECK(scratch.size(0) == 2, "blur_pil: scratch uint8 [2, H, W, 3]");
  TORCH_CHECK(slot >= 0 && slot < out.size(0), "blur_pil: slot outside out");
  const int64_t one = (int64_t)1 << 24;
  TORCH_CHECK(r >= 0 && r < 32768 && ww >= 0 && fw >= 0 && (2 * r + 1) * ww + 2 * fw <= one,
              "blur_pil: box weights must sum to at most 2^24");
  const char* s0 = static_cast<const char*>(scratch.data_ptr());
  const char* o0 = static_cast<const char*>(out.data_ptr());
  TORCH_CHECK(s0 + scratch.numel() <= o0 || o0 + out.numel() <= s0, "blur_pil: scratch overlaps out");
  const int64_t n = img.numel();
  uint8_t* sp = scratch.data_ptr<uint8_t>();
  launch_blur_pil_general(img.data_ptr<uint8_t>(), (int)img.size(0), (int)img.size(1), (int)r, (uint32_t)ww,
                          (uint32_t)fw, sp, sp + n, out.data_ptr<uint8_t>() + slot * n, cur_stream());
}

}

using nogil = py::call_guard<py::gil_scoped_release>;

PYBIND11_MODULE(_C, m) {
  m.doc() = "cassmantle_amd gfx950 (CDNA4) HIP kernel library";
  m.def("gemm", &gemm, py::arg("x"), py::arg("w"), py::arg("bias"), py::arg("residual"), py::arg("out"),
        py::arg("act"), py::arg("stats"), py::arg("stats_hw"), py::arg("ln_rows") = py::none(),
        py::arg("ln_wsum") = py::none(), py::arg("ln_eps") = 0.0, py::arg("kv8") = py::none(),
        py::arg("kv8_col0") = 0, py::arg("kv8_ntok") = 0, py::arg("kv8_hk") = 0, py::arg("ln_rows_fx") = py::none(),
        py::arg("row_stats") = py::none(), py::arg("gn_stats") = py::none(), py::arg("gn_gamma") = py::none(),
        py::arg("gn_beta") = py::none(), py::arg("gn_groups") = 0, py::arg("gn_hw") = 0, py::arg("gn_eps") = 0.0, nogil());
  m.def("row_stats", &row_stats, nogil());
  m.def("gemm_cat", &gemm_cat, nogil());
  m.def("group_norm_cat", &group_norm_cat, nogil());
  m.def("gemm_tile_menu", []() {
    static const char* const fam[] = {"static", "pingpong", "deep", "areg"};
    py::list rows;
    for (const GemmTile& t : kGemmTiles)
      rows.append(py::make_tuple(t.id, fam[t.family], t.BM, t.BN, std::to_string(t.WM) + "x" + std::to_string(t.WN), t.stages,
                                 t.producers, t.gated()));
    return rows;
  });
  m.def("gemm_set_override", [](int64_t cfg, int64_t split) { gemm_set_override((int)cfg, (int)split); });
  m.def("gemm_tune_set", [](const std::string& key, int64_t cfg, int64_t split) { gemm_tune_set(key, (int)cfg, (int)split); });
  m.def("gemm_tune_clear", []() { gemm_tune_clear(); });
  m.def("gemm_tune_size", []() { return (int64_t)gemm_tune_size(); });
  m.def("gemm_record_keys", [](bool on) { gemm_record_keys(on); });
  m.def("gemm_last_key", []() { return gemm_last_key(); });
  m.def("gemm_last_plan", []() { int c, sp; gemm_last_plan(&c, &sp); return std::vector<int64_t>{c, sp}; });
  m.def("gemm_rms", &gemm_rms, nogil());
  m.def("conv2d", &conv2d, nogil());
  m.def("conv2d_up2", &conv2d_up2, nogil());
  m.def("bmm_nt", &bmm_nt, nogil());
  m.def("group_norm", &group_norm, nogil());
  m.def("layer_norm", &layer_norm, nogil());
  m.def("embed_layer_norm", &embed_layer_norm, nogil());
  m.def("group_norm_stats", &group_norm_stats, nogil());
  m.def("channel_stats", &channel_stats, nogil());
  m.def("attention", &attention, nogil());
  m.def("attention_fp8_pack", &attention_fp8_pack, nogil());
  m.def("attention_fp8_bytes", &attention_fp8_bytes, nogil());
  m.def("gather_cosine", &gather_cosine, nogil());
  m.def("pair_cosine", &pair_cosine, nogil());
  m.def("cosine_gemv", &cosine_gemv, nogil());
  m.def("cosine_topk", &cosine_topk, nogil());
  m.def("mean_pool_l2", &mean_pool_l2, nogil());
  m.def("gaussian_blur", &gaussian_blur, nogil());
  m.def("blur_pil_tiled", &blur_pil_tiled, nogil());
  m.def("blur_pil_general", &blur_pil_general, nogil());
  m.def("blur_pil_max_tiled_radius", []() { return (int64_t)blur_pil_max_tiled_radius(); });
  m.def("to_uint8", &to_uint8, nogil());
  m.def("jpeg_count", &jpeg_count, nogil());
  m.def("jpeg_write", &jpeg_write, nogil());
  m.def("jpeg_encode_layout", &jpeg_encode_layout_dict);
  m.def("jpeg_reconstruct", &jpeg_reconstruct, nogil());
  m.def("jpeg_entropy_decode", &jpeg_entropy_decode, nogil());
  m.def("jpeg_entropy_decode_chunked", &jpeg_entropy_decode_chunked, nogil());
  m.def("timestep_embedding", &timestep_embedding, nogil());
  m.def("gather_add", &gather_add, nogil());
  m.def("concat2", &concat2, nogil());
  m.def("silu_", &silu_, nogil());
  m.def("latent_init", &latent_init, nogil());
  m.def("finalize_latents", &finalize_latents, nogil());
  m.def("dcopy", &dcopy, nogil());
  m.def("set_fp8_attn_variant", [](int64_t v) { set_fp8_attn_variant((int)v); });
  m.def("set_attn_d40_variant", [](int64_t v) { set_attn_d40_variant((int)v); });
  m.def("gemm_set_raster", &gemm_set_raster);
  m.def("latent_step", &latent_step, nogil());
  m.def("advance_step", &advance_step, nogil());
  m.def("zero_", &zero_, nogil());
  m.def("prefetch", &prefetch, nogil());
  m.def("lm_sample", &lm_sample, nogil());
  m.def("cu_mask_stream", &cu_mask_stream);
  m.def("cu_count", &cu_count);
  m.def("softmax_rows", &softmax_rows, nogil());
  m.def("rms_norm", &rms_norm, nogil());
  m.def("rope_kv", &rope_kv, nogil());
  m.def("decode_attention", &decode_attention, nogil());
  m.attr("arch") = "gfx950";
}
```

### cassmantle_amd/ops/csrc/common.h

```cpp
#pragma once
#include <hip/hip_runtime.h>
#include <stdint.h>

typedef __attribute__((ext_vector_type(8))) __bf16 bf16x8_t;
typedef __attribute__((ext_vector_type(4))) __bf16 bf16x4_t;
typedef __attribute__((ext_vector_type(4))) short s16x4_t;
typedef __attribute__((ext_vector_type(4))) float f32x4_t;
typedef __attribute__((ext_vector_type(16))) float f32x16_t;
typedef __attribute__((ext_vector_type(4))) int i32x4_t;

#define CM_DEVICE __device__ __forceinline__

CM_DEVICE float bf2f(uint16_t u) { return __uint_as_float(((uint32_t)u) << 16); }

typedef __attribute__((ext_vector_type(2))) __bf16 bf16x2_t;

CM_DEVICE uint16_t f2bf(float f) { return __builtin_bit_cast(uint16_t, (__bf16)f); }

CM_DEVICE uint32_t pack2(float a, float b) {
  bf16x2_t v = {(__bf16)a, (__bf16)b};
  return __builtin_bit_cast(uint32_t, v);
}

CM_DEVICE uint32_t f8x4(float a, float b, float c, float d) {
  uint32_t w;
  asm("v_cvt_pk_fp8_f32 %0, %1, %2\n\tv_cvt_pk_fp8_f32 %0, %3, %4 op_sel:[0,0,1]"
      : "=&v"(w) : "v"(a), "v"(b), "v"(c), "v"(d));
  return w;
}

CM_DEVICE int f8_slot(int kk) {
  const int hf = kk >> 5, w = kk & 31;
  const int h = (w >> 2) & 1, r = (w & 3) + 4 * (w >> 3);
  return 32 * h + 16 * hf + r;
}

template <class Args>
CM_DEVICE bool kv8_store4(const Args& p, int m, int n, const float* o) {
  if (p.kv8 == nullptr || n < p.kv8_col0) return false;
  const int C = p.kv8_hk * 64, rel = n - p.kv8_col0;
  const int b = m / p.kv8_ntok, key = m - b * p.kv8_ntok;
  const uint32_t w = f8x4(o[0], o[1], o[2], o[3]);
  if (rel < C) {
    const long long bh = (long long)b * p.kv8_hk + (rel >> 6);
    *reinterpret_cast<uint32_t*>(p.kv8 + (bh * p.kv8_ntok + key) * 64 + (rel & 63)) = w;
  } else {
    const long long B = p.M / p.kv8_ntok;
    uint8_t* V8t = p.kv8 + B * p.kv8_hk * p.kv8_ntok * 64;
    const long long bh = (long long)b * p.kv8_hk + ((rel - C) >> 6);
    const long long col = (key & ~63) + f8_slot(key & 63);
    uint8_t* dst = V8t + (bh * 64 + ((rel - C) & 63)) * p.kv8_ntok + col;
#pragma unroll
    for (int e = 0; e < 4; ++e) dst[(long long)e * p.kv8_ntok] = (uint8_t)(w >> (8 * e));
  }
  return true;
}


CM_DEVICE void unpack8(const uint4& v, float* f) {
  f[0] = __uint_as_float(v.x << 16); f[1] = __uint_as_float(v.x & 0xffff0000u);
  f[2] = __uint_as_float(v.y << 16); f[3] = __uint_as_float(v.y & 0xffff0000u);
  f[4] = __uint_as_float(v.z << 16); f[5] = __uint_as_float(v.z & 0xffff0000u);
  f[6] = __uint_as_float(v.w << 16); f[7] = __uint_as_float(v.w & 0xffff0000u);
}

CM_DEVICE uint4 pack8(const float* f) {
  uint4 v;
  v.x = pack2(f[0], f[1]); v.y = pack2(f[2], f[3]);
  v.z = pack2(f[4], f[5]); v.w = pack2(f[6], f[7]);
  return v;
}

CM_DEVICE bf16x8_t as_bf16x8(const uint4& v) { return __builtin_bit_cast(bf16x8_t, v); }

template <int HI_OFF>
CM_DEVICE void ds_read_tr16_x4x2(const uint32_t (&a)[4], s16x4_t (&lo)[4], s16x4_t (&hi)[4]) {
  asm volatile(
      "ds_read_b64_tr_b16 %0, %8\n\t"
      "ds_read_b64_tr_b16 %1, %8 offset:%c12\n\t"
      "ds_read_b64_tr_b16 %2, %9\n\t"
      "ds_read_b64_tr_b16 %3, %9 offset:%c12\n\t"
      "ds_read_b64_tr_b16 %4, %10\n\t"
      "ds_read_b64_tr_b16 %5, %10 offset:%c12\n\t"
      "ds_read_b64_tr_b16 %6, %11\n\t"
      "ds_read_b64_tr_b16 %7, %11 offset:%c12\n\t"
      "s_waitcnt lgkmcnt(0)"
      : "=&v"(lo[0]), "=&v"(hi[0]), "=&v"(lo[1]), "=&v"(hi[1]), "=&v"(lo[2]), "=&v"(hi[2]), "=&v"(lo[3]), "=&v"(hi[3])
      : "v"(a[0]), "v"(a[1]), "v"(a[2]), "v"(a[3]), "i"(HI_OFF)
      : "memory");
}
CM_DEVICE uint32_t lds_addr(const void* p) {
  return (uint32_t)(uintptr_t)(const __attribute__((address_space(3))) void*)p;
}

template <typename T>
CM_DEVICE void lds_use(T& v) { asm volatile("" : "+v"(v)); }

CM_DEVICE float silu_f(float x) { return x * __builtin_amdgcn_rcpf(1.0f + __expf(-x)); }
CM_DEVICE float erf_fast(float x) {
  const float ax = fabsf(x);
  const float t = __builtin_amdgcn_rcpf(fmaf(0.3275911f, ax, 1.0f));
  float y = fmaf(fmaf(fmaf(fmaf(1.061405429f, t, -1.453152027f), t, 1.421413741f), t, -0.284496736f), t, 0.254829592f) * t;
  y = 1.0f - y * __expf(-ax * ax);
  return copysignf(y, x);
}
CM_DEVICE float gelu_f(float x) { return 0.5f * x * (1.0f + erf_fast(x * 0.70710678118654752f)); }
CM_DEVICE float gelu_tanh_f(float x) {
  const float k = 0.7978845608028654f;
  return 0.5f * x * (1.0f + tanhf(k * (x + 0.044715f * x * x * x)));
}
CM_DEVICE float quick_gelu_f(float x) { return x * __builtin_amdgcn_rcpf(1.0f + __expf(-1.702f * x)); }

constexpr double STAT_SCALE_SUM = 16777216.0;
constexpr double STAT_SCALE_SQ = 65536.0;
CM_DEVICE void stat_atomic_add(long long* st, int which, float v) {
  const double sc = which ? STAT_SCALE_SQ : STAT_SCALE_SUM;
  atomicAdd(reinterpret_cast<unsigned long long*>(st), (unsigned long long)__double2ll_rn((double)v * sc));
}
CM_DEVICE double stat_decode(long long v, int which) {
  return (double)v * (which ? (1.0 / STAT_SCALE_SQ) : (1.0 / STAT_SCALE_SUM));
}

enum Act { ACT_NONE = 0, ACT_GELU = 1, ACT_SILU = 2, ACT_QUICK_GELU = 3, ACT_GEGLU = 4, ACT_GELU_TANH = 5,
           ACT_SWIGLU = 6 };

__host__ __device__ inline bool is_gated(int act) { return act == ACT_GEGLU || act == ACT_SWIGLU; }
CM_DEVICE float gelu_geglu_f(float x) {
#ifdef CASSMANTLE_GELU_EXACT
  return gelu_f(x);
#else
  const float xc = __builtin_amdgcn_fmed3f(x, -8.f, 8.f);
  const float x2 = xc * xc;
  const float z = xc * fmaf(x2, fmaf(x2, 0.0010350826722789555f, -0.10690469751684778f), -2.300978763043183f);
  return x * __builtin_amdgcn_rcpf(1.f + __builtin_amdgcn_exp2f(z));
#endif
}

CM_DEVICE float gate_f(float h, float g, int act) { return h * (act == ACT_SWIGLU ? silu_f(g) : gelu_geglu_f(g)); }

CM_DEVICE float apply_act(float x, int act) {
  switch (act) {
    case ACT_GELU: return gelu_f(x);
    case ACT_SILU: return silu_f(x);
    case ACT_QUICK_GELU: return quick_gelu_f(x);
    case ACT_GELU_TANH: return gelu_tanh_f(x);
    default: return x;
  }
}

CM_DEVICE float wave_sum(float v) {
#pragma unroll
  for (int o = 32; o > 0; o >>= 1) v += __shfl_xor(v, o, 64);
  return v;
}
CM_DEVICE float wave_max(float v) {
#pragma unroll
  for (int o = 32; o > 0; o >>= 1) v = fmaxf(v, __shfl_xor(v, o, 64));
  return v;
}

CM_DEVICE int xcd_remap(int bid, int nblocks) {
  const int nx = 8;
  int q = nblocks / nx, r = nblocks % nx;
  int xcd = bid % nx, idx = bid / nx;
  return (xcd < r ? xcd * (q + 1) : r * (q + 1) + (xcd - r) * q) + idx;
}
```

### cassmantle_amd/ops/csrc/gemm_impl.h

```cpp
#pragma once
#include <stdlib.h>

#include "common.h"
#include "gemm_tiles.h"
#include "kernels.h"

#ifndef GEMM_DIAG_APRO
#define GEMM_DIAG_APRO 0
#endif
#ifndef GEMM_FRAG_PREFETCH
#define GEMM_FRAG_PREFETCH 0
#endif

namespace {

__device__ uint4 g_zero_page[4];

constexpr int BK = 64;

CM_DEVICE int swz(int row, int chunk) { return chunk ^ ((row >> 1) & 7); }

#ifndef GEMM_PF_SELF
#define GEMM_PF_SELF 0
#endif
#ifndef GEMM_RASTER_G
#define GEMM_RASTER_G 4
#endif
CM_DEVICE void tile_of(int lin, int nM, int nN, int raster, int& tm, int& tn) {
  const int G = min(raster > 0 ? raster : GEMM_RASTER_G, nM);
  if (G > 1) {
    const int grp = lin / (G * nN);
    const int gs = min(G, nM - grp * G);
    const int r = lin - grp * G * nN;
    tm = grp * G + r % gs;
    tn = r / gs;
  } else {
    tn = lin % nN;
    tm = lin / nN;
  }
}

typedef __attribute__((address_space(3))) void lds_void;

CM_DEVICE void glds16(const void* src, uint4* lds_wave_base) {
  __builtin_amdgcn_global_load_lds(src, (lds_void*)lds_wave_base, 16, 0, 0);
}

CM_DEVICE void blds16(__amdgpu_buffer_rsrc_t rs, uint4* lds_wave_base, int voff, int soff) {
  __builtin_amdgcn_raw_ptr_buffer_load_lds(rs, (lds_void*)lds_wave_base, 16, voff, soff, 0, 0);
}

CM_DEVICE __amdgpu_buffer_rsrc_t make_rsrc(const void* base, long long bytes) {
  return __builtin_amdgcn_make_buffer_rsrc(const_cast<void*>(base), (short)0, (int)bytes, 0x00020000);
}

template <int N>
CM_DEVICE void wait_vmcnt() { asm volatile("s_waitcnt vmcnt(%0)" ::"n"(N) : "memory"); }

CM_DEVICE void add4(float* o, uint2 v) {
  o[0] += bf2f(v.x & 0xffff); o[1] += bf2f(v.x >> 16); o[2] += bf2f(v.y & 0xffff); o[3] += bf2f(v.y >> 16);
}

CM_DEVICE float2 ln_row(const GemmArgs& p, int m, double inv_k) {
  if (p.ln_rows_fx != nullptr) {
    const longlong2 v = reinterpret_cast<const longlong2*>(p.ln_rows_fx)[m];
    const double mean = (double)v.x * (inv_k * (1.0 / STAT_SCALE_SUM));
    const double var = fmax((double)v.y * (inv_k * (1.0 / STAT_SCALE_SQ)) - mean * mean, 0.0);
    return make_float2((float)mean, rsqrtf((float)var + p.ln_eps));
  }
  return reinterpret_cast<const float2*>(p.ln_rows)[m];
}
CM_DEVICE void ln_apply4(float2 ms, const float* __restrict__ wsum, float* o) {
#pragma unroll
  for (int r = 0; r < 4; ++r) o[r] = ms.y * fmaf(-ms.x, wsum[r], o[r]);
}
CM_DEVICE void ln_fold4(const GemmArgs& p, int m, int wn, float* o) {
  const float2 ms = ln_row(p, m, 1.0 / (double)p.K);
#pragma unroll
  for (int r = 0; r < 4; ++r) o[r] = ms.y * fmaf(-ms.x, p.ln_wsum[wn + r], o[r]);
}

CM_DEVICE long long out_row(const GemmArgs& p, int m, int z) {
  if (!p.parity) return m;
  const int hw = p.Ho * p.Wo;
  const int img = m / hw;
  const int r = m - img * hw;
  const int i = r / p.Wo, j = r - i * p.Wo;
  return ((long long)img * 2 * p.Ho + 2 * i + (z >> 1)) * (2 * p.Wo) + 2 * j + (z & 1);
}

template <bool OUTF32>
CM_DEVICE void epilogue4(const GemmArgs& p, int batch, int m, int n, float* o) {
  const int hw = p.Ho * p.Wo;
  const int bimg = (p.chan_bias != nullptr) ? (m / hw) : 0;
  const long long cbs = p.ldcb ? p.ldcb : p.N;
  const bool full = (n + 4 <= p.N) && (p.N % 4 == 0) && (p.ldc % 4 == 0) && (cbs % 4 == 0);
  const long long om = out_row(p, m, batch);
  if (p.ln_rows || p.ln_rows_fx) ln_fold4(p, m, n, o);
#pragma unroll
  for (int r = 0; r < 4; ++r) o[r] *= p.alpha;
  if (full) {
    if (p.bias) add4(o, *reinterpret_cast<const uint2*>(p.bias + n));
    if (p.chan_bias) add4(o, *reinterpret_cast<const uint2*>(p.chan_bias + (long long)bimg * cbs + n));
    if (p.act != ACT_NONE) {
#pragma unroll
      for (int r = 0; r < 4; ++r) o[r] = apply_act(o[r], p.act);
    }
    if (p.residual) add4(o, *reinterpret_cast<const uint2*>(p.residual + om * p.ldc + n));
    if (!OUTF32 && kv8_store4(p, m, n, o)) return;
    if constexpr (OUTF32) {
      float* C = reinterpret_cast<float*>(p.C) + (long long)batch * p.sC + om * p.ldc + n;
      *reinterpret_cast<float4*>(C) = make_float4(o[0], o[1], o[2], o[3]);
    } else {
      uint16_t* C = reinterpret_cast<uint16_t*>(p.C) + (long long)batch * p.sC + om * p.ldc + n;
      *reinterpret_cast<uint2*>(C) = make_uint2(pack2(o[0], o[1]), pack2(o[2], o[3]));
    }
  } else {
#pragma unroll
    for (int r = 0; r < 4; ++r) {
      if (n + r >= p.N) break;
      float v = o[r];
      if (p.bias) v += bf2f(p.bias[n + r]);
      if (p.chan_bias) v += bf2f(p.chan_bias[(long long)bimg * cbs + n + r]);
      v = apply_act(v, p.act);
      if (p.residual) v += bf2f(p.residual[om * p.ldc + n + r]);
      if constexpr (OUTF32)
        reinterpret_cast<float*>(p.C)[(long long)batch * p.sC + om * p.ldc + n + r] = v;
      else
        reinterpret_cast<uint16_t*>(p.C)[(long long)batch * p.sC + om * p.ldc + n + r] = f2bf(v);
    }
  }
}

template <bool OUTF32>
CM_DEVICE void epilogue4_call(const GemmArgs& p, int batch, int m, int n, f32x4_t v) {
  float o[4] = {v[0], v[1], v[2], v[3]};
  epilogue4<OUTF32>(p, batch, m, n, o);
}

CM_DEVICE void gated_epilogue4_call(const GemmArgs& p, int batch, int m, int n, f32x4_t hv, f32x4_t gv) {
  float o[4], hh[4] = {hv[0], hv[1], hv[2], hv[3]}, gg[4] = {gv[0], gv[1], gv[2], gv[3]};
  if (p.ln_rows || p.ln_rows_fx) { ln_fold4(p, m, n, hh); ln_fold4(p, m, p.N + n, gg); }
#pragma unroll
  for (int r = 0; r < 4; ++r) {
    float h = hh[r], g = gg[r];
    if (p.bias) { h += bf2f(p.bias[n + r]); g += bf2f(p.bias[p.N + n + r]); }
    o[r] = gate_f(h, g, p.act);
  }
  uint16_t* C = reinterpret_cast<uint16_t*>(p.C) + (long long)batch * p.sC + (long long)m * p.ldc + n;
  if (p.residual) add4(o, *reinterpret_cast<const uint2*>(p.residual + (long long)m * p.ldc + n));
  *reinterpret_cast<uint2*>(C) = make_uint2(pack2(o[0], o[1]), pack2(o[2], o[3]));
}

template <int BM, int BN, int WM, int WN, bool GEGLU, bool OUTF32, int TI, int TJ, int THREADS, bool SPLIT_DIRECT = false>
CM_DEVICE void tile_epilogue(const GemmArgs& p, f32x4_t (&acc)[TI][TJ], uint4* smem, float* __restrict__ partial,
                             int m0, int n0, int batch, int wm, int wn, int tid, int nsplit, int split_id,
                             bool has_acc = true) {
  const int lane = tid & 63;
  const int fr = lane & 15, fq = lane >> 4;
  if constexpr (!OUTF32) {
    constexpr int OBN = GEGLU ? BN / 2 : BN;
    constexpr int OST = OBN + 8;
    const long long cbs = p.ldcb ? p.ldcb : p.N;
    const bool lds_ok = nsplit == 1 && (p.N % 8 == 0) && (p.ldc % 8 == 0) && (cbs % 4 == 0);
    if (lds_ok) {
      __syncthreads();
      uint16_t* T = reinterpret_cast<uint16_t*>(smem);
      const int hw = p.Ho * p.Wo;
      const double inv_k = 1.0 / (double)p.K;
      if (has_acc) {
#pragma unroll
      for (int j = 0; j < TJ; ++j) {
        const int ml = wm * (BM / WM) + 16 * j + fr;
        const int m = m0 + ml;
        const int bimg = (p.chan_bias != nullptr && m < p.M) ? (m / hw) : 0;
        const bool lnf = (p.ln_rows != nullptr || p.ln_rows_fx != nullptr) && m < p.M;
        const float2 lnm = lnf ? ln_row(p, m, inv_k) : make_float2(0.f, 1.f);
        if constexpr (GEGLU) {
#pragma unroll
          for (int pi = 0; pi < TI / 2; ++pi) {
            const int nl = wn * (BN / WN / 2) + 16 * pi + 4 * fq;
            const int n = n0 + nl;
            float o[4], hh[4], gg[4];
#pragma unroll
            for (int r = 0; r < 4; ++r) { hh[r] = acc[2 * pi][j][r]; gg[r] = acc[2 * pi + 1][j][r]; }
            if (lnf && n < p.N) { ln_apply4(lnm, p.ln_wsum + n, hh); ln_apply4(lnm, p.ln_wsum + p.N + n, gg); }
#pragma unroll
            for (int r = 0; r < 4; ++r) {
              float h = hh[r], g = gg[r];
              if (p.bias && n < p.N) { h += bf2f(p.bias[n + r]); g += bf2f(p.bias[p.N + n + r]); }
              o[r] = gate_f(h, g, p.act);
            }
            *reinterpret_cast<uint2*>(T + ml * OST + nl) = make_uint2(pack2(o[0], o[1]), pack2(o[2], o[3]));
          }
        } else {
#pragma unroll
          for (int i = 0; i < TI; ++i) {
            const int nl = wn * (BN / WN) + 16 * i + 4 * fq;
            const int n = n0 + nl;
            float o[4] = {acc[i][j][0], acc[i][j][1], acc[i][j][2], acc[i][j][3]};
            if (lnf && n < p.N) ln_apply4(lnm, p.ln_wsum + n, o);
#pragma unroll
            for (int r = 0; r < 4; ++r) o[r] *= p.alpha;
            if (n < p.N && m < p.M) {
              if (p.bias) add4(o, *reinterpret_cast<const uint2*>(p.bias + n));
              if (p.chan_bias) add4(o, *reinterpret_cast<const uint2*>(p.chan_bias + (long long)bimg * cbs + n));
              if (p.act != ACT_NONE) {
#pragma unroll
                for (int r = 0; r < 4; ++r) o[r] = apply_act(o[r], p.act);
              }
            }
            *reinterpret_cast<uint2*>(T + ml * OST + nl) = make_uint2(pack2(o[0], o[1]), pack2(o[2], o[3]));
          }
        }
      }
      }
      __syncthreads();
      constexpr int CPR = OBN / 8;
      uint16_t* Cb = reinterpret_cast<uint16_t*>(p.C) + (long long)batch * p.sC;
      auto finish = [&](int row, int c8) -> uint4 {
        const int m = m0 + row, n = n0 + c8 * 8;
        const long long om = out_row(p, m, batch);
        uint4 v = *reinterpret_cast<const uint4*>(T + row * OST + c8 * 8);
        if (p.residual) {
          const uint4 rv = *reinterpret_cast<const uint4*>(p.residual + om * p.ldc + n);
          float a[8], b[8];
          unpack8(v, a);
          unpack8(rv, b);
#pragma unroll
          for (int e = 0; e < 8; ++e) a[e] += b[e];
          v = pack8(a);
        }
        if (p.kv8 != nullptr && n >= p.kv8_col0) {
          if (n < p.kv8_col0 + 64 * p.kv8_hk) {
            float a[8];
            unpack8(v, a);
            const int rel = n - p.kv8_col0, b = m / p.kv8_ntok, key = m - b * p.kv8_ntok;
            const long long bh = (long long)b * p.kv8_hk + (rel >> 6);
            *reinterpret_cast<uint2*>(p.kv8 + (bh * p.kv8_ntok + key) * 64 + (rel & 63)) =
                make_uint2(f8x4(a[0], a[1], a[2], a[3]), f8x4(a[4], a[5], a[6], a[7]));
          }
          return v;
        }
        *reinterpret_cast<uint4*>(Cb + om * p.ldc + n) = v;
        return v;
      };
      if (p.stats == nullptr) {
        for (int c = tid; c < BM * CPR; c += THREADS) {
          const int row = c / CPR, c8 = c - row * CPR;
          if (m0 + row >= p.M || n0 + c8 * 8 >= p.N) continue;
          const uint4 v = finish(row, c8);
          if (p.row_stats != nullptr) *reinterpret_cast<uint4*>(T + row * OST + c8 * 8) = v;
        }
        if (p.row_stats != nullptr) {
          __syncthreads();
          for (int row = tid; row < BM; row += THREADS) {
            const int m = m0 + row;
            if (m >= p.M) break;
            float sm = 0.f, sq = 0.f;
            for (int c8 = 0; c8 < CPR && n0 + c8 * 8 < p.N; ++c8) {
              float f[8];
// ... 469 lines not shown
  }
#endif

  if constexpr (STAGES == 2) {
    if (nk > 0) stage(kt0, 0);
    __syncthreads();
    for (int t = 0; t < nk; t += 2) {
      if (t + 1 < nk) stage(kt0 + t + 1, 1);
      compute(0);
      __syncthreads();
      if (t + 1 >= nk) break;
      if (t + 2 < nk) stage(kt0 + t + 2, 0);
      compute(1);
      __syncthreads();
    }
  } else {
    constexpr int S = STAGES;
    const int npt = w_last_round ? NPT : NPT - 1;
    auto wait_tiles = [&](int k) {
      if (npt == NPT) {
        if (k <= 0) wait_vmcnt<0>();
        else if (k == 1) wait_vmcnt<NPT>();
        else if (k == 2) wait_vmcnt<2 * NPT>();
        else wait_vmcnt<3 * NPT>();
      } else {
        if (k <= 0) wait_vmcnt<0>();
        else if (k == 1) wait_vmcnt<NPT - 1>();
        else if (k == 2) wait_vmcnt<2 * (NPT - 1)>();
        else wait_vmcnt<3 * (NPT - 1)>();
      }
    };
    if (dma_wave) {
#pragma unroll
      for (int s0 = 0; s0 < S - 1; ++s0)
        if (s0 < nk) stage(kt0 + s0, s0);
    }
    for (int t = 0; t < nk; ++t) {
      if (dma_wave) wait_tiles(min(S - 2, nk - 1 - t));
      asm volatile("s_waitcnt lgkmcnt(0)" ::: "memory");
      __builtin_amdgcn_s_barrier();
      if (dma_wave && t + S - 1 < nk) stage(kt0 + t + S - 1, (t + S - 1) % S);
      if (mma_wave) compute(t % S);
    }
  }

  tile_epilogue<BM, BN, WM, WN, GEGLU, OUTF32, TI, TJ, THREADS>(p, acc, smem, partial, m0, n0, batch, wm, wn, tid,
                                                               gridDim.y, blockIdx.y, mma_wave);
#if GEMM_PF_SELF
  asm volatile("" ::"v"(pf_acc));
#endif
}

template <bool OUTF32>
__global__ void splitk_reduce_kernel(GemmArgs p, const float* __restrict__ partial, int split) {
  const int bz = blockIdx.y;
  partial += (long long)bz * split * p.M * p.N;
  const long long nq = (long long)p.M * (p.N / 4);
  for (long long i = (long long)blockIdx.x * blockDim.x + threadIdx.x; i < nq; i += (long long)gridDim.x * blockDim.x) {
    const int m = (int)(i / (p.N / 4));
    const int n = (int)(i - (long long)m * (p.N / 4)) * 4;
    float o[4] = {0.f, 0.f, 0.f, 0.f};
    for (int s = 0; s < split; ++s) {
      const float4 v = *reinterpret_cast<const float4*>(partial + ((long long)s * p.M + m) * p.N + n);
      o[0] += v.x; o[1] += v.y; o[2] += v.z; o[3] += v.w;
    }
    epilogue4<OUTF32>(p, bz, m, n, o);
  }
}

constexpr int SK_RB = 64;
constexpr int SK_QB = 16;
constexpr int SK_RL = 256 / SK_QB;
template <bool OUTF32>
__global__ void __launch_bounds__(256) splitk_reduce_stats_kernel(GemmArgs p, const float* __restrict__ partial,
                                                                  int split, int rb) {
  __shared__ float red[2][SK_RL][SK_QB * 4];
  const int bz = blockIdx.z;
  partial += (long long)bz * split * p.M * p.N;
  const int qd = threadIdx.x % SK_QB, rl = threadIdx.x / SK_QB;
  const int n = (blockIdx.x * SK_QB + qd) * 4;
  const int m0 = blockIdx.y * rb;
  const int m1 = min(p.M, m0 + rb);
  const bool on = n < p.N;
  const int shw = p.stats_hw;
  const bool single = (m0 / shw) == ((m1 - 1) / shw);
  float s4[4] = {0.f, 0.f, 0.f, 0.f}, q4[4] = {0.f, 0.f, 0.f, 0.f};
  int cur = -1;
  auto flush = [&]() {
    if (cur < 0) return;
#pragma unroll
    for (int e = 0; e < 4; ++e) {
      stat_atomic_add(p.stats + ((long long)cur * p.N + n + e) * 2 + 0, 0, s4[e]);
      stat_atomic_add(p.stats + ((long long)cur * p.N + n + e) * 2 + 1, 1, q4[e]);
      s4[e] = 0.f;
      q4[e] = 0.f;
    }
  };
  if (on) {
    for (int m = m0 + rl; m < m1; m += SK_RL) {
      float o[4] = {0.f, 0.f, 0.f, 0.f};
      const float* src = partial + (long long)m * p.N + n;
      const long long slab = (long long)p.M * p.N;
      int sl = 0;
      for (; sl + 4 <= split; sl += 4) {
        const float4 v0 = *reinterpret_cast<const float4*>(src + (sl + 0) * slab);
        const float4 v1 = *reinterpret_cast<const float4*>(src + (sl + 1) * slab);
        const float4 v2 = *reinterpret_cast<const float4*>(src + (sl + 2) * slab);
        const float4 v3 = *reinterpret_cast<const float4*>(src + (sl + 3) * slab);
        o[0] += (v0.x + v1.x) + (v2.x + v3.x);
        o[1] += (v0.y + v1.y) + (v2.y + v3.y);
        o[2] += (v0.z + v1.z) + (v2.z + v3.z);
        o[3] += (v0.w + v1.w) + (v2.w + v3.w);
      }
      for (; sl < split; ++sl) {
        const float4 v = *reinterpret_cast<const float4*>(src + sl * slab);
        o[0] += v.x; o[1] += v.y; o[2] += v.z; o[3] += v.w;
      }
      epilogue4<OUTF32>(p, bz, m, n, o);
      if (!single) {
        const int img = m / shw;
        if (img != cur) { flush(); cur = img; }
      }
#pragma unroll
      for (int e = 0; e < 4; ++e) {
        const float f = OUTF32 ? o[e] : bf2f(f2bf(o[e]));
        s4[e] += f;
        q4[e] = fmaf(f, f, q4[e]);
      }
    }
  }
  if (!single) {
    flush();
    return;
  }
#pragma unroll
  for (int e = 0; e < 4; ++e) {
    red[0][rl][qd * 4 + e] = s4[e];
    red[1][rl][qd * 4 + e] = q4[e];
  }
  __syncthreads();
  const int img = m0 / shw;
  if (threadIdx.x < 2 * SK_QB * 4) {
    const int st = threadIdx.x / (SK_QB * 4), col = threadIdx.x % (SK_QB * 4);
    const int nn = blockIdx.x * SK_QB * 4 + col;
    if (nn < p.N) {
      float a = 0.f;
#pragma unroll
      for (int r = 0; r < SK_RL; ++r) a += red[st][r][col];
      stat_atomic_add(p.stats + ((long long)img * p.N + nn) * 2 + st, st, a);
    }
  }
}

template <bool OUTF32>
void launch_splitk_reduce(const GemmArgs& p, float* ws, int split, hipStream_t s) {
  if (p.stats != nullptr) {
    static const int adapt = [] { const char* e = getenv("CASSMANTLE_SK_ADAPT"); return e ? atoi(e) : 1; }();
    const long long cols = (p.N / 4 + SK_QB - 1) / SK_QB;
    int rb = SK_RB;
    while (adapt && rb > SK_RL && cols * ((p.M + rb - 1) / rb) * p.batch < 512) rb /= 2;
    dim3 g2((unsigned)cols, (unsigned)((p.M + rb - 1) / rb), (unsigned)p.batch);
    hipLaunchKernelGGL(splitk_reduce_stats_kernel<OUTF32>, g2, dim3(256), 0, s, p, ws, split, rb);
  } else {
    const long long nq = (long long)p.M * (p.N / 4);
    const long long nb = (nq + 255) / 256;
    const unsigned rb = (unsigned)(nb < 2048 ? nb : 2048);
    hipLaunchKernelGGL(splitk_reduce_kernel<OUTF32>, dim3(rb, (unsigned)p.batch), dim3(256), 0, s, p, ws, split);
  }
}

template <int BM, int BN, int WM, int WN, int CONV, bool GEGLU, bool OUTF32, int STAGES, bool BUF, int NP = 0>
void launch_t(const GemmArgs& p, float* ws, hipStream_t s) {
  const int nN = GEGLU ? (p.N + BN / 2 - 1) / (BN / 2) : (p.N + BN - 1) / BN;
  const int nM = (p.M + BM - 1) / BM;
  const int split = (ws != nullptr && p.split > 1) ? p.split : 1;
  dim3 grid(nN * nM, split, p.batch);
  constexpr size_t lds_stage = (size_t)STAGES * (BM + BN) * BK * 2;
  constexpr size_t lds_epi = (size_t)BM * ((GEGLU ? BN / 2 : BN) + 8) * 2;
  constexpr size_t lds = lds_stage > lds_epi ? lds_stage : lds_epi;
  auto* kfn = &gemm_kernel<BM, BN, WM, WN, CONV, GEGLU, OUTF32, STAGES, BUF, NP>;
  if constexpr (lds > 65536) {
    static const bool once = [&] {
      (void)hipFuncSetAttribute((const void*)kfn, hipFuncAttributeMaxDynamicSharedMemorySize, (int)lds);
      return true;
    }();
    (void)once;
  }
  hipLaunchKernelGGL(kfn, grid, dim3(64 * (WM * WN + NP)), lds, s, p, ws);
  if (split > 1) launch_splitk_reduce<OUTF32>(p, ws, split, s);
}

template <int I, int CONV, bool GEGLU, bool OUTF32, bool BUF>
bool launch_row(int cfg, const GemmArgs& p, float* ws, hipStream_t s) {
  constexpr GemmTile t = kGemmTiles[I];
  if constexpr ((t.family == kTileStatic || (t.family == kTileDeep && BUF && !OUTF32)) && (!GEGLU || t.gated())) {
    if (t.id != cfg) return false;
    launch_t<t.BM, t.BN, GEGLU ? t.GWM : t.WM, GEGLU ? t.GWN : t.WN, CONV, GEGLU, OUTF32, t.stages, BUF, t.producers>(p, ws, s);
    return true;
  }
  return false;
}

template <int CONV, bool GEGLU, bool OUTF32, bool BUF, int... I>
void launch_cfg(const GemmArgs& p, float* ws, hipStream_t s, std::integer_sequence<int, I...>) {
  if (!(launch_row<I, CONV, GEGLU, OUTF32, BUF>(p.cfg, p, ws, s) || ...))
    (void)(launch_row<I, CONV, GEGLU, OUTF32, BUF>(gemm_default_tile(kTileStatic, GEGLU), p, ws, s) || ...);
}

template <int CONV, bool BUF>
void launch_tiles(const GemmArgs& p, float* ws, hipStream_t s) {
  if (p.act == ACT_GEGLU || p.act == ACT_SWIGLU) launch_cfg<CONV, true, false, BUF>(p, ws, s, GemmTileRows{});
  else if (p.out_f32) launch_cfg<CONV, false, true, BUF>(p, ws, s, GemmTileRows{});
  else launch_cfg<CONV, false, false, BUF>(p, ws, s, GemmTileRows{});
}

}

#define GEMM_TU_ENTRY(NAME, CONV, BUF) \
  void NAME(const GemmArgs& p, float* ws, hipStream_t s) { launch_tiles<CONV, BUF>(p, ws, s); }
```

### cassmantle_amd/ops/csrc/gemm_pp.h

```cpp
#pragma once
#include <type_traits>

#include "gemm_impl.h"

namespace {

template <int N>
CM_DEVICE void wait_lgkm() { asm volatile("s_waitcnt lgkmcnt(%0)" ::"n"(N) : "memory"); }

template <int BM, int BN, int WM, int WN>
struct PPGeom {
  static constexpr int TI = BN / WN / 16, TJ = BM / WM / 16;
  static constexpr int TIa = (TI + 1) / 2, TIb = TI / 2, TJa = (TJ + 1) / 2, TJb = TJ / 2;
  static constexpr int R0 = WM * 16 * TJa, R1 = WN * 16 * TIa, R2 = WM * 16 * TJb, R3 = WN * 16 * TIb;
  static constexpr int O0 = 0, O2 = R0, O1 = BM, O3 = BM + R1;
  static constexpr int TILE_ROWS = BM + BN;
  static constexpr int NR0 = (R0 + 63) / 64, NR1 = (R1 + 63) / 64, NR2 = (R2 + 63) / 64, NR3 = (R3 + 63) / 64;
  static constexpr bool JUNK = (R0 % 64) || (R1 % 64) || (R2 % 64) || (R3 % 64);
  static constexpr int JUNK_ROW = 2 * TILE_ROWS;
  static constexpr int STAGE_ROWS = 2 * TILE_ROWS + (JUNK ? 64 : 0);
  static constexpr int PERIOD = NR0 + NR1 + NR2 + NR3;
  static constexpr int OBN_ = BN;
};

// ... 304 lines not shown
#pragma unroll
    for (int ks = 0; ks < 2; ++ks) {
      if constexpr (J == 0 || J == 1) {
#pragma unroll
        for (int i = 0; i < TIa; ++i) {
          if constexpr (J == 0) {
#pragma unroll
            for (int j = 0; j < TJa; ++j)
              acc[i][j] = __builtin_amdgcn_mfma_f32_16x16x32_bf16(wfa[i][ks], afa[j][ks], acc[i][j], 0, 0, 0);
          } else {
#pragma unroll
            for (int j = 0; j < TJb; ++j)
              acc[i][TJa + j] = __builtin_amdgcn_mfma_f32_16x16x32_bf16(wfa[i][ks], afb[j][ks], acc[i][TJa + j], 0, 0, 0);
          }
        }
      } else {
#pragma unroll
        for (int i = 0; i < TIb; ++i) {
          if constexpr (J == 3) {
#pragma unroll
            for (int j = 0; j < TJa; ++j)
              acc[TIa + i][j] = __builtin_amdgcn_mfma_f32_16x16x32_bf16(wfb[i][ks], afa[j][ks], acc[TIa + i][j], 0, 0, 0);
          } else {
#pragma unroll
            for (int j = 0; j < TJb; ++j)
              acc[TIa + i][TJa + j] =
                  __builtin_amdgcn_mfma_f32_16x16x32_bf16(wfb[i][ks], afb[j][ks], acc[TIa + i][TJa + j], 0, 0, 0);
          }
        }
      }
    }
    __builtin_amdgcn_s_setprio(0);
    if constexpr (!(DIAG & 2)) __builtin_amdgcn_s_barrier();
  };

  auto mphase = [&](auto Pc, auto Bc, int t) {
    constexpr int P = decltype(Pc)::value;
    constexpr int B = decltype(Bc)::value;
    const uint4* Bs = smem + B * TILE;
    if constexpr (P == 0) {
#pragma unroll
      for (int ks = 0; ks < 2; ++ks) {
#pragma unroll
        for (int i = 0; i < TIa; ++i) wfa[i][ks] = as_bf16x8(Bs[wbase_a + 128 * i + lo[ks]]);
#pragma unroll
        for (int j = 0; j < TJa; ++j) afa[j][ks] = as_bf16x8(Bs[abase_a + 128 * j + lo[ks]]);
#pragma unroll
        for (int j = 0; j < TJb; ++j) afb[j][ks] = as_bf16x8(Bs[abase_b + 128 * j + lo[ks]]);
      }
    } else {
#pragma unroll
      for (int ks = 0; ks < 2; ++ks)
#pragma unroll
        for (int i = 0; i < TIb; ++i) wfb[i][ks] = as_bf16x8(Bs[wbase_b + 128 * i + lo[ks]]);
    }
    const int u = t + (P == 0 ? 1 : 2);
    if (!(DIAG & 1) && u < nk) {
      if constexpr (P == 0) {
        stage(I1{}, kt0 + u, B ^ 1);
        stage(I3{}, kt0 + u, B ^ 1);
        wait_vmcnt<G::NR1 + G::NR3>();
      } else {
        stage(I0{}, kt0 + u, B);
        stage(I2{}, kt0 + u, B);
        wait_vmcnt<G::NR0 + G::NR2>();
      }
    } else {
      wait_vmcnt<0>();
    }
    wait_lgkm<0>();
    if constexpr ((DIAG & 4) && P == 0) {
#pragma unroll
      for (int ks = 0; ks < 2; ++ks) {
#pragma unroll
        for (int j = 0; j < TJa; ++j) afa[j][ks] = gn_silu_probe(afa[j][ks], lane);
#pragma unroll
        for (int j = 0; j < TJb; ++j) afb[j][ks] = gn_silu_probe(afb[j][ks], lane);
      }
    }
    if constexpr (!(DIAG & 2)) __builtin_amdgcn_s_barrier();
    __builtin_amdgcn_s_setprio(1);
#pragma unroll
    for (int ks = 0; ks < 2; ++ks) {
      if constexpr (P == 0) {
#pragma unroll
        for (int i = 0; i < TIa; ++i) {
#pragma unroll
          for (int j = 0; j < TJa; ++j)
            acc[i][j] = __builtin_amdgcn_mfma_f32_16x16x32_bf16(wfa[i][ks], afa[j][ks], acc[i][j], 0, 0, 0);
#pragma unroll
          for (int j = 0; j < TJb; ++j)
            acc[i][TJa + j] = __builtin_amdgcn_mfma_f32_16x16x32_bf16(wfa[i][ks], afb[j][ks], acc[i][TJa + j], 0, 0, 0);
        }
      } else {
#pragma unroll
        for (int i = 0; i < TIb; ++i) {
#pragma unroll
          for (int j = 0; j < TJb; ++j)
            acc[TIa + i][TJa + j] =
                __builtin_amdgcn_mfma_f32_16x16x32_bf16(wfb[i][ks], afb[j][ks], acc[TIa + i][TJa + j], 0, 0, 0);
#pragma unroll
          for (int j = 0; j < TJa; ++j)
            acc[TIa + i][j] = __builtin_amdgcn_mfma_f32_16x16x32_bf16(wfb[i][ks], afa[j][ks], acc[TIa + i][j], 0, 0, 0);
        }
      }
    }
    __builtin_amdgcn_s_setprio(0);
    if constexpr (!(DIAG & 2)) __builtin_amdgcn_s_barrier();
  };

  if constexpr (SCHED == 2) {
    for (int t = 0; t < nk; t += 2) {
      mphase(I0{}, I0{}, t);
      mphase(I1{}, I0{}, t);
      if (t + 1 >= nk) break;
      mphase(I0{}, I1{}, t + 1);
      mphase(I1{}, I1{}, t + 1);
    }
  } else {
    for (int t = 0; t < nk; t += 2) {
      phase(I0{}, I0{}, t);
      phase(I1{}, I0{}, t);
      phase(I2{}, I0{}, t);
      phase(I3{}, I0{}, t);
      if (t + 1 >= nk) break;
      phase(I0{}, I1{}, t + 1);
      phase(I1{}, I1{}, t + 1);
      phase(I2{}, I1{}, t + 1);
      phase(I3{}, I1{}, t + 1);
    }
  }
  if (!late) __builtin_amdgcn_s_barrier();
  wait_vmcnt<0>();
  __syncthreads();

  tile_epilogue<BM, BN, WM, WN, GEGLU, false, TI, TJ, 512, true>(p, acc, smem, partial, m0, n0, batch, wm, wn, tid,
                                                          gridDim.y, blockIdx.y);
}

template <int BM, int BN, int WM, int WN, int CONV, bool GEGLU>
void launch_pp(const GemmArgs& p, float* ws, hipStream_t s) {
  const int nN = GEGLU ? (p.N + BN / 2 - 1) / (BN / 2) : (p.N + BN - 1) / BN;
  const int nM = (p.M + BM - 1) / BM;
  const int split = (ws != nullptr && p.split > 1) ? p.split : 1;
  dim3 grid(nN * nM, split, p.batch);
  constexpr size_t lds = pp_lds_bytes<BM, BN, WM, WN, GEGLU>();
  auto* kfn = &gemm_pp_kernel<BM, BN, WM, WN, CONV, GEGLU, 2, PP_DIAG_DEFAULT>;
  static const bool once = [&] {
    (void)hipFuncSetAttribute((const void*)kfn, hipFuncAttributeMaxDynamicSharedMemorySize, (int)lds);
    return true;
  }();
  (void)once;
  hipLaunchKernelGGL(kfn, grid, dim3(512), lds, s, p, ws);
  if (split > 1) launch_splitk_reduce<false>(p, ws, split, s);
}

template <int I, int CONV, bool GEGLU>
bool launch_pp_row(int cfg, const GemmArgs& p, float* ws, hipStream_t s) {
  constexpr GemmTile t = kGemmTiles[I];
  if constexpr (t.family == kTilePingPong && (!GEGLU || t.gated())) {
    if (t.id != cfg) return false;
    launch_pp<t.BM, t.BN, GEGLU ? t.GWM : t.WM, GEGLU ? t.GWN : t.WN, CONV, GEGLU>(p, ws, s);
    return true;
  }
  return false;
}

template <int CONV, bool GEGLU, int... I>
void launch_pp_menu(const GemmArgs& p, float* ws, hipStream_t s, std::integer_sequence<int, I...>) {
  if (!(launch_pp_row<I, CONV, GEGLU>(p.cfg, p, ws, s) || ...))
    (void)(launch_pp_row<I, CONV, GEGLU>(gemm_default_tile(kTilePingPong, GEGLU), p, ws, s) || ...);
}

template <int CONV>
void launch_pp_cfg(const GemmArgs& p, float* ws, hipStream_t s) {
  if (is_gated(p.act)) launch_pp_menu<CONV, true>(p, ws, s, GemmTileRows{});
  else launch_pp_menu<CONV, false>(p, ws, s, GemmTileRows{});
}

}

#define GEMM_PP_TU_ENTRY(NAME, CONV) \
  void NAME(const GemmArgs& p, float* ws, hipStream_t s) { launch_pp_cfg<CONV>(p, ws, s); }
```

### cassmantle_amd/ops/csrc/kernels.h

```cpp
#pragma once
#include <hip/hip_runtime.h>
#include <stdint.h>

struct GemmArgs {
  const uint16_t* A = nullptr;
  const uint16_t* W = nullptr;
  const uint16_t* bias = nullptr;
  const uint16_t* residual = nullptr;
  const uint16_t* chan_bias = nullptr;
  int ldcb = 0;
  void* C = nullptr;
  int M = 0, N = 0, K = 0, Nw = 0;
  int lda = 0, ldc = 0, ldw = 0;
  long long sA = 0, sW = 0, sC = 0;
  int batch = 1;
  float alpha = 1.f;
  int act = 0;
  int out_f32 = 0;
  int split = 1;
  int cfg = 0;
  int raster = 0;
  int conv = 0, IH = 0, IW = 0, Cin = 0, Ho = 0, Wo = 0, stride = 1, pad = 0, ksize = 1, upsample = 0;
  int parity = 0;
  const uint16_t* rms_gamma = nullptr;
  float rms_eps = 0.f;
  const uint16_t* A2 = nullptr;
  int lda2 = 0, ka = 0;
  const float* ln_rows = nullptr;
  const float* ln_wsum = nullptr;
  float ln_eps = 0.f;
  const long long* ln_rows_fx = nullptr;
  long long* row_stats = nullptr;
  const long long* gn_stats = nullptr;
  const uint16_t* gn_gamma = nullptr;
  const uint16_t* gn_beta = nullptr;
  int gn_groups = 0, gn_hw = 0;
  float gn_eps = 0.f;
  long long* stats = nullptr;
  int stats_hw = 0;
  uint8_t* kv8 = nullptr;
  int kv8_col0 = 0, kv8_ntok = 0, kv8_hk = 0;
};
#define GEMM_MAX_SPLIT 16
struct GemmPlan { int cfg; int split; };
GemmPlan gemm_plan(const GemmArgs& p);
int gemm_plan_split(const GemmArgs& p);
void gemm_set_override(int cfg, int split);
#include <string>
std::string gemm_key(const GemmArgs& p);
void gemm_tune_set(const std::string& key, int cfg, int split);
void gemm_tune_clear();
int gemm_tune_size();
void gemm_record_keys(bool on);
std::string gemm_last_key();
void gemm_last_plan(int* cfg, int* split);
void launch_gemm(const GemmArgs& p, float* ws, hipStream_t s);

struct AttnArgs {
  const uint16_t* q; const uint16_t* k; const uint16_t* v; uint16_t* o;
  long long q_sb, q_sn, q_sh;
  long long k_sb, k_sn, k_sh;
  long long v_sb, v_sn, v_sh;
  long long o_sb, o_sn, o_sh;
  int B, H, Nq, Nk, d;
  float scale;
  int causal;
  const int* kv_lens;
  int group = 1;
};
void launch_attention(const AttnArgs& a, hipStream_t s);
long long attention_d512_workspace(const AttnArgs& a);
void launch_attention_d512(const AttnArgs& a, float* ws, hipStream_t s);
long long attention_fp8_workspace(const AttnArgs& a, int Hk);
void set_fp8_attn_variant(int v);
void set_attn_d40_variant(int v);
void launch_attention_fp8(const AttnArgs& a, int Hk, uint8_t* ws, hipStream_t s, bool packed = false);
void launch_attention_fp8_pack(const AttnArgs& a, int Hk, uint8_t* ws, hipStream_t s);

void launch_group_norm(const uint16_t* x, const uint16_t* gamma, const uint16_t* beta, uint16_t* y,
                       float* ws, int B, long long S, int C, int G, float eps, int silu, hipStream_t s);
void launch_group_norm_cs(const uint16_t* x, const uint16_t* x2, const long long* stats_a, int Ca, const long long* stats_b,
                          const uint16_t* gamma, const uint16_t* beta, uint16_t* y, int B, long long S, int C,
                          int G, float eps, int silu, hipStream_t s);
void launch_channel_stats(const uint16_t* x, long long* stats, int B, long long S, int C, hipStream_t s);
long long group_norm_workspace(int B, long long S, int C);
void launch_layer_norm(const uint16_t* x, const uint16_t* gamma, const uint16_t* beta, uint16_t* y,
                       long long rows, int D, float eps, hipStream_t s);
bool gemm_areg_ok(const GemmArgs& p);
void launch_gemm_areg(const GemmArgs& p, hipStream_t s);
void launch_row_stats(const uint16_t* x, float* stats, long long rows, int D, float eps, hipStream_t s);
void launch_embed_layer_norm(const uint16_t* word, const long long* ids, const uint16_t* pos, int seq,
                             const uint16_t* add, const uint16_t* gamma, const uint16_t* beta, uint16_t* y,
                             long long rows, int D, float eps, hipStream_t s);
void launch_rms_norm(const uint16_t* x, const uint16_t* gamma, uint16_t* y, long long rows, int D, float eps,
                     hipStream_t s);

bool launch_gemv(const GemmArgs& p, hipStream_t s);
struct RopeArgs {
  const uint16_t* qkv; long long ld;
  const int* pos0;
  uint16_t* q_out;
  uint16_t* k_cache; uint16_t* v_cache;
  int B, T, H, Hk, d, L;
  float log2_theta;
};
void launch_rope_kv(const RopeArgs& a, hipStream_t s);
struct DecodeArgs {
  const uint16_t* q; long long q_sb;
  const uint16_t* k_cache; const uint16_t* v_cache;
  const int* lens;
  uint16_t* o; long long o_sb;
  float* ws;
  int* tickets;
  int B, H, Hk, d, L;
  float scale;
};
int decode_splits(int B, int Hk, int L);
void launch_lm_sample(const void* logits, int logits_f32, int V, const float* noise, const float* eos_bias, int eos,
                      float temperature, int k, long long* step, long long* out, long long* tok, int* pos, int* lens,
                      hipStream_t s);
void launch_decode_attention(const DecodeArgs& a, int ns, hipStream_t s);

void launch_gather_cosine(const void* table, int table_f32, int D, const int* ia, const int* ib,
                          float* out, int n, hipStream_t s);
void launch_pair_cosine(const float* a, const float* b, int D, float* out, int n, hipStream_t s);
void launch_cosine_gemv(const void* table, int table_f32, int V, int D, const void* vec, int vec_f32,
                        float* out, hipStream_t s);
int cosine_topk_workspace(int V, int k);
void launch_cosine_topk(const void* table, int table_f32, int V, int D, const void* vec, int vec_f32, int k,
                        unsigned long long* ws, float* vals, long long* idx, hipStream_t s);
void launch_mean_pool_l2(const uint16_t* h, const int* lens, float* out, int B, int T, int D, hipStream_t s);

void launch_gaussian_blur(const void* img, int u8, int H, int W, int C, const float* w, int R,
                          float* tmp, void* out, hipStream_t s);
void launch_to_uint8(const uint16_t* x, uint8_t* out, long long n, hipStream_t s);
void launch_timestep_embedding(const float* t, void* out, int B, int dim, int flip, float shift, int out_bf16,
                               hipStream_t s);
void launch_gather_add(const uint16_t* table, const int* ids, const uint16_t* pos, int seq, int D, long long rows,
                       uint16_t* out, hipStream_t s);
void launch_concat2(const uint16_t* a, int Da, const void* b, int Db, int b_f32, long long rows, uint16_t* out,
                    hipStream_t s);
void launch_silu_bf16(uint16_t* x, long long n, hipStream_t s);
void launch_latent_init(const float* x0, float c_in0, float* x, float* xs, float* hist, int nhist, uint16_t* unet_in,
                        long long n, int cfg, int cin, int cstride, hipStream_t s);
void launch_copy(const void* src, void* dst, long long bytes, hipStream_t s);
void launch_finalize_latents(const float* x, uint16_t* z, long long n, uint8_t* finite, hipStream_t s);
void launch_latent_step(const uint16_t* eps, float* x, float* hist, float* xs, const float* coef, const int* step,
                        uint16_t* unet_in, long long n, int cfg, int cin, int cstride, const void* tab0, void* buf0,
                        long long row_bytes0, const void* tab1, void* buf1, long long row_bytes1, int rows,
                        const void* seeds, int images, hipStream_t s);
void launch_advance_step(int* step, hipStream_t s);
void launch_zero(void* p, long long bytes, hipStream_t s);
void launch_prefetch(const void* p, long long bytes, int blocks, void* sink, hipStream_t s);
void launch_softmax_rows(const float* S, uint16_t* P, int rows, int cols, int Nq, int causal,
                         const int* kv_lens, hipStream_t s);

struct JpegArgs {
  const uint8_t* img = nullptr;
  int B = 0, H = 0, W = 0;
  int nb = 0;
  int mx = 0, my = 0;
  int restart = 0, nint = 0;
  const int* qtab = nullptr;
  const int* huff = nullptr;
  int16_t* coef = nullptr;
  uint32_t* lens = nullptr;
  uint32_t* offs = nullptr;
  uint32_t* base = nullptr;
  const uint8_t* header = nullptr;
  int hdr_len = 0;
  int lj = 0;
  uint8_t* out = nullptr;
  uint8_t* planes = nullptr;
  uint8_t* dec = nullptr;
  uint32_t* freq = nullptr;
  uint32_t* ihuff = nullptr;
  uint8_t* hdrs = nullptr;
  uint32_t* hdr_lens = nullptr;
  int hdr_cap = 0, hdr_split = 0;
};
void launch_jpeg_count(const JpegArgs& a, hipStream_t s);
void launch_jpeg_write(const JpegArgs& a, hipStream_t s);
struct JpegBlkArgs {
  uint32_t* bits = nullptr;
  uint32_t* ubits = nullptr;
  uint32_t* scratch = nullptr;
  uint32_t stride = 0;
  uint32_t* err = nullptr;
  uint32_t out_size = 0;
};
void launch_jpeg_count_blocks(const JpegArgs& a, const JpegBlkArgs& k, hipStream_t s);
void launch_jpeg_write_blocks(const JpegArgs& a, const JpegBlkArgs& k, hipStream_t s);
void launch_jpeg_reconstruct(const JpegArgs& a, hipStream_t s);
struct JpegDecodeIn {
  const uint8_t* bytes = nullptr;
  uint32_t nbytes = 0;
  const uint32_t* intervals = nullptr;
  const uint32_t* tables = nullptr;
  unsigned long long* status = nullptr;
  long long zero_bytes = 0;
};
void launch_jpeg_entropy_decode(const JpegArgs& a, const JpegDecodeIn& d, hipStream_t s);
struct JpegSyncIn {
  const uint32_t* lane0 = nullptr;
  const uint32_t* groups = nullptr;
  int ngroups = 0;
  uint32_t cb = 0;
  uint32_t* words = nullptr;
};
// ... 9 lines not shown
```

### cassmantle_amd/ops/csrc/norm.hip

```cpp
#include <stdlib.h>

#include "common.h"
#include "kernels.h"

namespace {

constexpr int GN_THREADS = 256;
constexpr int GN_UNROLL = 4;

struct GnGeom { int V, VPT, T, R; };
GnGeom gn_geom(int C) {
  GnGeom g;
  g.V = C / 8;
  g.VPT = (g.V + GN_THREADS - 1) / GN_THREADS;
  g.T = (g.V + g.VPT - 1) / g.VPT;
  g.R = GN_THREADS / g.T;
  if (g.R < 1) g.R = 1;
  return g;
}

template <int VPT>
__global__ void __launch_bounds__(GN_THREADS) gn_stats_kernel(const uint16_t* __restrict__ x, float* __restrict__ part,
                                                              long long S, int C, int G, int T, int R, int chunks,
                                                              long long rows_per_chunk) {
// ... 102 lines not shown
                                                              const float* __restrict__ stats,
                                                              const uint16_t* __restrict__ gamma,
                                                              const uint16_t* __restrict__ beta,
                                                              uint16_t* __restrict__ y, long long S, int C, int G,
                                                              int T, int R, long long rows_per_block, int silu) {
  const int V = C / 8;
  const int tid = threadIdx.x;
  const int b = blockIdx.y;
  const int tv = tid % T, rl = tid / T;
  if (rl >= R) return;
  const int Cg = C / G;
  float sc[VPT][8], sf[VPT][8];
#pragma unroll
  for (int j = 0; j < VPT; ++j) {
    const int v = tv + T * j;
    if (v >= V) continue;
    float ga[8], be[8];
    unpack8(*reinterpret_cast<const uint4*>(gamma + v * 8), ga);
    unpack8(*reinterpret_cast<const uint4*>(beta + v * 8), be);
#pragma unroll
    for (int i = 0; i < 8; ++i) {
      const int g = (v * 8 + i) / Cg;
      const float2 ms = *reinterpret_cast<const float2*>(stats + ((long long)b * G + g) * 2);
      sc[j][i] = ga[i] * ms.y;
      sf[j][i] = be[i] - ms.x * sc[j][i];
    }
  }
  const long long rbeg = (long long)blockIdx.x * rows_per_block;
  const long long rend = min(S, rbeg + rows_per_block);
  const long long off = (long long)b * S * C;
  const uint16_t* xb = x + off;
  uint16_t* yb = y + off;
  auto emit = [&](long long r, int j, uint4 u) {
    float f[8];
    unpack8(u, f);
#pragma unroll
    for (int i = 0; i < 8; ++i) {
      const float o = fmaf(f[i], sc[j][i], sf[j][i]);
      f[i] = silu ? silu_f(o) : o;
    }
    *reinterpret_cast<uint4*>(yb + r * C + (tv + T * j) * 8) = pack8(f);
  };
  long long r = rbeg + rl;
  for (; r + (GN_UNROLL - 1) * R < rend; r += GN_UNROLL * R) {
    uint4 u[GN_UNROLL][VPT];
#pragma unroll
    for (int k = 0; k < GN_UNROLL; ++k)
#pragma unroll
      for (int j = 0; j < VPT; ++j) {
        const int v = tv + T * j;
        if (v < V) u[k][j] = *reinterpret_cast<const uint4*>(xb + (r + (long long)k * R) * C + v * 8);
      }
#pragma unroll
    for (int k = 0; k < GN_UNROLL; ++k)
#pragma unroll
      for (int j = 0; j < VPT; ++j)
        if (tv + T * j < V) emit(r + (long long)k * R, j, u[k][j]);
  }
  for (; r < rend; r += R)
#pragma unroll
    for (int j = 0; j < VPT; ++j)
      if (tv + T * j < V) emit(r, j, *reinterpret_cast<const uint4*>(xb + r * C + (tv + T * j) * 8));
}

template <int VPT, int U>
__global__ void __launch_bounds__(GN_THREADS) gn_apply_cs_kernel(const uint16_t* __restrict__ x,
                                                                 const uint16_t* __restrict__ x2,
                                                                 const long long* __restrict__ sa, int Ca,
                                                                 const long long* __restrict__ sb,
                                                                 const uint16_t* __restrict__ gamma,
                                                                 const uint16_t* __restrict__ beta,
                                                                 uint16_t* __restrict__ y, long long S, int C,
                                                                 int G, int T, int R, long long rows_per_block,
                                                                 float eps, int silu) {
  extern __shared__ float gst[];
  const int V = C / 8;
  const int tid = threadIdx.x;
  const int b = blockIdx.y;
  const int Cg = C / G;
  const int Cb = C - Ca;
  const int tv = tid % T, rl = tid / T;
  const bool act = rl < R;
  const long long rbeg = (long long)blockIdx.x * rows_per_block;
  const long long rend = min(S, rbeg + rows_per_block);
  uint16_t* yb = y + (long long)b * S * C;
  const uint16_t* src[VPT];
  int lds_[VPT];
  bool von[VPT];
#pragma unroll
  for (int j = 0; j < VPT; ++j) {
    von[j] = act && (tv + T * j) < V;
    const int c0 = (von[j] ? tv + T * j : 0) * 8;
    if (x2 == nullptr) {
      src[j] = x + (long long)b * S * C + c0;
      lds_[j] = C;
    } else if (c0 < Ca) {
      src[j] = x + (long long)b * S * Ca + c0;
      lds_[j] = Ca;
    } else {
      src[j] = x2 + (long long)b * S * Cb + (c0 - Ca);
      lds_[j] = Cb;
    }
  }
  uint4 u[U][VPT];
  long long r = rbeg + rl;
  auto load_group = [&](long long r0) {
#pragma unroll
    for (int k = 0; k < U; ++k)
#pragma unroll
      for (int j = 0; j < VPT; ++j) {
        const long long rr = min(r0 + (long long)k * R, rend - 1);
        u[k][j] = *reinterpret_cast<const uint4*>(src[j] + rr * lds_[j]);
      }
  };
  load_group(r);
  uint4 gv[VPT], bv[VPT];
#pragma unroll
  for (int j = 0; j < VPT; ++j) {
    const int v = von[j] ? tv + T * j : 0;
    gv[j] = *reinterpret_cast<const uint4*>(gamma + v * 8);
    bv[j] = *reinterpret_cast<const uint4*>(beta + v * 8);
  }
  const int tpg = G >= GN_THREADS ? 1 : (GN_THREADS / G >= 8 ? 8 : (GN_THREADS / G >= 4 ? 4 : (GN_THREADS / G >= 2 ? 2 : 1)));
  for (int g0 = 0; g0 < G; g0 += GN_THREADS / tpg) {
    const int g = g0 + tid / tpg, sub = tid % tpg;
    long long si = 0, qi = 0;
    if (g < G) {
      const int c0 = g * Cg + sub, c1 = (g + 1) * Cg;
      longlong2 v[16];
#pragma unroll
      for (int q = 0; q < 16; ++q) {
        const int c = min(c0 + q * tpg, c1 - 1);
        const long long* sp = c < Ca ? sa + ((long long)b * Ca + c) * 2 : sb + ((long long)b * Cb + (c - Ca)) * 2;
        v[q] = *reinterpret_cast<const longlong2*>(sp);
      }
#pragma unroll
      for (int q = 0; q < 16; ++q) {
        const bool live = c0 + q * tpg < c1;
        si += live ? v[q].x : 0;
        qi += live ? v[q].y : 0;
      }
      for (int c = c0 + 16 * tpg; c < c1; c += tpg) {
        const long long* sp = c < Ca ? sa + ((long long)b * Ca + c) * 2 : sb + ((long long)b * Cb + (c - Ca)) * 2;
        const longlong2 vv = *reinterpret_cast<const longlong2*>(sp);
        si += vv.x;
        qi += vv.y;
      }
    }
    for (int o = 1; o < tpg; o <<= 1) {
      si += __shfl_xor(si, o, 64);
      qi += __shfl_xor(qi, o, 64);
    }
    if (g < G && sub == 0) {
      const double sm = stat_decode(si, 0), q = stat_decode(qi, 1);
      const double n = (double)S * Cg;
      const double mean = sm / n;
      double var = q / n - mean * mean;
      if (var < 0) var = 0;
      gst[2 * g] = (float)mean;
      gst[2 * g + 1] = (float)(1.0 / sqrt(var + (double)eps));
    }
  }
  __syncthreads();
  if (!act) return;
  float sc[VPT][8], sf[VPT][8];
#pragma unroll
  for (int j = 0; j < VPT; ++j) {
    const int v = tv + T * j;
    float ga[8], be[8];
    unpack8(gv[j], ga);
    unpack8(bv[j], be);
#pragma unroll
    for (int i = 0; i < 8; ++i) {
      const int g = von[j] ? (v * 8 + i) / Cg : 0;
      sc[j][i] = ga[i] * gst[2 * g + 1];
      sf[j][i] = be[i] - gst[2 * g] * sc[j][i];
    }
  }
  auto emit = [&](long long rr, int j, uint4 w) {
    float f[8];
    unpack8(w, f);
#pragma unroll
    for (int i = 0; i < 8; ++i) {
      const float o = fmaf(f[i], sc[j][i], sf[j][i]);
      f[i] = silu ? silu_f(o) : o;
    }
#if GN_NT_STORE
    typedef __attribute__((ext_vector_type(4))) unsigned int u32x4_nt;
    const uint4 pk = pack8(f);
    __builtin_nontemporal_store(u32x4_nt{pk.x, pk.y, pk.z, pk.w}, reinterpret_cast<u32x4_nt*>(yb + rr * C + (tv + T * j) * 8));
#else
    *reinterpret_cast<uint4*>(yb + rr * C + (tv + T * j) * 8) = pack8(f);
#endif
  };
  for (; r < rend; r += U * R) {
    uint4 cur[U][VPT];
#pragma unroll
    for (int k = 0; k < U; ++k)
#pragma unroll
      for (int j = 0; j < VPT; ++j) cur[k][j] = u[k][j];
    const long long rn = r + (long long)U * R;
    if (rn < rend) load_group(rn);
#pragma unroll
    for (int k = 0; k < U; ++k)
#pragma unroll
      for (int j = 0; j < VPT; ++j)
        if (von[j] && r + (long long)k * R < rend) emit(r + (long long)k * R, j, cur[k][j]);
  }
}

template <int VPT>
__global__ void __launch_bounds__(GN_THREADS) channel_stats_kernel(const uint16_t* __restrict__ x,
                                                                   long long* __restrict__ stats, long long S, int C,
                                                                   int T, int R, long long rows_per_chunk) {
  extern __shared__ float sh[];
  const int V = C / 8;
  const int tid = threadIdx.x;
  const int b = blockIdx.y;
  const long long rbeg = (long long)blockIdx.x * rows_per_chunk;
  const long long rend = min(S, rbeg + rows_per_chunk);
  const uint16_t* base = x + (long long)b * S * C;
  const int tv = tid % T, rl = tid / T;
  float s[VPT][8], q[VPT][8];
#pragma unroll
  for (int j = 0; j < VPT; ++j)
#pragma unroll
    for (int i = 0; i < 8; ++i) { s[j][i] = 0.f; q[j][i] = 0.f; }
  if (rl < R) {
    for (long long r = rbeg + rl; r < rend; r += R)
#pragma unroll
      for (int j = 0; j < VPT; ++j) {
        const int v = tv + T * j;
        if (v >= V) continue;
        float f[8];
        unpack8(*reinterpret_cast<const uint4*>(base + r * C + v * 8), f);
#pragma unroll
        for (int i = 0; i < 8; ++i) { s[j][i] += f[i]; q[j][i] = fmaf(f[i], f[i], q[j][i]); }
      }
#pragma unroll
    for (int j = 0; j < VPT; ++j) {
      const int v = tv + T * j;
      if (v >= V) continue;
#pragma unroll
      for (int i = 0; i < 8; ++i) {
        sh[(long long)rl * C + v * 8 + i] = s[j][i];
        sh[(long long)(R + rl) * C + v * 8 + i] = q[j][i];
      }
    }
  }
  __syncthreads();
  for (int c = tid; c < 2 * C; c += GN_THREADS) {
    const int stat = c / C, ch = c - stat * C;
    float acc = 0.f;
    for (int k = 0; k < R; ++k) acc += sh[(long long)(stat * R + k) * C + ch];
    stat_atomic_add(stats + ((long long)b * C + ch) * 2 + stat, stat, acc);
  }
}

struct EmbArgs {
  const long long* ids = nullptr;
  const uint16_t* pos = nullptr;
  const uint16_t* add = nullptr;
  int seq = 1;
};

template <int VPL, bool RMS, bool STATS = false, bool EMB = false>
__global__ void ln_kernel(const uint16_t* __restrict__ x, const uint16_t* __restrict__ gamma,
                          const uint16_t* __restrict__ beta, uint16_t* __restrict__ y,
                          long long rows, int D, int T, float eps, EmbArgs e = EmbArgs()) {
  const int lane = threadIdx.x & 63;
  const int seg = lane / T, sl = lane - seg * T;
  const int rows_per_wave = 64 / T;
  const long long row = ((long long)blockIdx.x * (blockDim.x / 64) + (threadIdx.x >> 6)) * rows_per_wave + seg;
  const bool ok = row < rows;
  const int V = D / 8;
  const long long src_row = EMB ? (ok ? e.ids[row] : 0) : (ok ? row : 0);
  const uint4* xr = reinterpret_cast<const uint4*>(x + src_row * D);
  float f[VPL][8];
  float s = 0.f;
#pragma unroll
  for (int j = 0; j < VPL; ++j) {
    const int v = sl + T * j;
    if (ok && v < V) {
      unpack8(xr[v], f[j]);
      if constexpr (EMB) {
        float a[8];
        unpack8(reinterpret_cast<const uint4*>(e.pos + (row % e.seq) * D)[v], a);
#pragma unroll
        for (int k = 0; k < 8; ++k) f[j][k] = bf2f(f2bf(f[j][k] + a[k]));
        if (e.add) {
          unpack8(reinterpret_cast<const uint4*>(e.add)[v], a);
#pragma unroll
          for (int k = 0; k < 8; ++k) f[j][k] = bf2f(f2bf(f[j][k] + a[k]));
        }
      }
#pragma unroll
      for (int k = 0; k < 8; ++k) s += f[j][k];
    } else {
#pragma unroll
      for (int k = 0; k < 8; ++k) f[j][k] = 0.f;
    }
  }
  for (int o = T >> 1; o > 0; o >>= 1) s += __shfl_xor(s, o, 64);
  const float mean = RMS ? 0.f : s / D;
  float ss = 0.f;
#pragma unroll
  for (int j = 0; j < VPL; ++j) {
    const int v = sl + T * j;
    if (v < V) {
#pragma unroll
      for (int k = 0; k < 8; ++k) { const float t = f[j][k] - mean; ss = fmaf(t, t, ss); }
    }
  }
  for (int o = T >> 1; o > 0; o >>= 1) ss += __shfl_xor(ss, o, 64);
  const float rstd = rsqrtf(ss / D + eps);
  if (!ok) return;
  if constexpr (STATS) {
    if (sl == 0) reinterpret_cast<float2*>(y)[row] = make_float2(mean, rstd);
    return;
  }
  uint4* yr = reinterpret_cast<uint4*>(y + row * D);
#pragma unroll
  for (int j = 0; j < VPL; ++j) {
    const int v = sl + T * j;
    if (v < V) {
      float g[8], bb[8];
      unpack8(reinterpret_cast<const uint4*>(gamma)[v], g);
      if (beta) unpack8(reinterpret_cast<const uint4*>(beta)[v], bb);
      else for (int k = 0; k < 8; ++k) bb[k] = 0.f;
      float o[8];
#pragma unroll
      for (int k = 0; k < 8; ++k) o[k] = fmaf((f[j][k] - mean) * rstd, g[k], bb[k]);
      yr[v] = pack8(o);
    }
  }
}

int gn_chunks(int B, long long S, int R) {
  long long want = (512 + B - 1) / B;
// ... 178 lines not shown
```

Baseline: 7.792 images/s.

## Fuse following GroupNorm into split-K conv/GEMM reduction epilogue

Adds a GroupNorm-consumer path to conv2d and linear. When split-K is active and one block per (batch, group) fills the GPU, a new reduce kernel sums the partials, computes group statistics in LDS, and writes the normalized (optionally SiLU) output directly. The UNet now passes the next block's GroupNorm into each resnet conv1, conv2 and downsampler, which removes separate group_norm launches and a re-read of the activation. This adds LDS-heavy kernels with one block per group, so parallelism may drop, and falls back to separate norm calls when conditions fail.

```diff
diff --git a/cassmantle_amd/models/layers.py b/cassmantle_amd/models/layers.py
--- a/cassmantle_amd/models/layers.py
+++ b/cassmantle_amd/models/layers.py
@@ -77,7 +77,9 @@
         self.weight = _param((fout, fin), std if std is not None else 1.0 / math.sqrt(fin), gen, dtype)
         self.bias = _param((fout,), 0.02, gen, dtype) if bias else None
 
-    def forward(self, x, residual=None, act=None, stats=None, row_stats=None):
+    def forward(self, x, residual=None, act=None, stats=None, row_stats=None, gn=None):
+        if gn is not None:
+            return ops.linear(x, self.weight, self.bias, residual=residual, act=act, stats=stats, gn=gn)
         return ops.linear(x, self.weight, self.bias, residual=residual, act=act, stats=stats, row_stats=row_stats)
 
 
@@ -114,7 +116,16 @@
         if self.pad_in > self.cin:
             self.padded_weight(self.pad_in)
 
-    def forward(self, x, residual=None, upsample=False, chan_bias=None, stats=None, out=None):
+    def forward(self, x, residual=None, upsample=False, chan_bias=None, stats=None, out=None, gn=None):
+        if gn is not None:
+            if out is None and x.shape[-1] == self.cin and not upsample:
+                if self.k == 1 and self.stride == 1 and chan_bias is None:
+                    return ops.linear(x, self.weight.view(self.cout, self.cin), self.bias, residual=residual,
+                                      stats=stats, gn=gn)
+                return ops.conv2d(x, self.weight, self.bias, self.stride, self.padding, residual=residual,
+                                  chan_bias=chan_bias, stats=stats, gn=gn)
+            y = self.forward(x, residual, upsample, chan_bias, stats, out)
+            return (y if gn.keep_raw else None), gn_module_apply(y, gn, stats)
         if out is not None:
             w = self.padded_weight(x.shape[-1]) if x.shape[-1] > self.cin else self.weight
             return ops.conv2d(x, w, self.bias, self.stride, self.padding, residual=residual,
@@ -142,6 +153,13 @@
     def forward(self, x, silu=False, stats=None, stats2=None):
         return ops.group_norm(x, self.groups, self.weight, self.bias, self.eps, silu, stats=stats, stats2=stats2)
 
+    def of(self, silu=False, keep_raw=True) -> "ops.GroupNormOf":
+        return ops.GroupNormOf(self.weight, self.bias, self.groups, self.eps, silu, keep_raw)
+
+
+def gn_module_apply(y, gn, stats):
+    return ops.group_norm(y, gn.groups, gn.weight, gn.bias, gn.eps, gn.silu, stats=stats)
+
 
 class LayerNorm(nn.Module):
     def __init__(self, dim: int, eps: float = 1e-5, dtype=torch.bfloat16):
diff --git a/cassmantle_amd/models/unet.py b/cassmantle_amd/models/unet.py
--- a/cassmantle_amd/models/unet.py
+++ b/cassmantle_amd/models/unet.py
@@ -61,11 +61,17 @@
         self.conv2 = Conv2d(cout, cout, 3, gen=gen, dtype=dtype)
         self.conv_shortcut = Conv2d(cin, cout, 1, padding=0, gen=gen, dtype=dtype) if cin != cout else None
 
-    def forward(self, x, temb_silu, tb_all=None, arena: Optional[StatsArena] = None, xs=None, xs2=None):
+    def input_gn(self):
+        return self.norm1.of(silu=True)
+
+    def forward(self, x, temb_silu, tb_all=None, arena: Optional[StatsArena] = None, xs=None, xs2=None, xn=None,
+                next_gn=None):
         pair = isinstance(x, tuple)
         B = x[0].shape[0] if pair else x.shape[0]
         cout = self.conv1.cout
-        if pair:
+        if xn is not None:
+            h = xn
+        elif pair:
             g = self.norm1
             h = ops.group_norm_cat(x[0], x[1], g.groups, g.weight, g.bias, g.eps, True, stats=xs, stats2=xs2)
         else:
@@ -75,8 +81,7 @@
         else:
             tb = self.time_emb_proj(temb_silu)
         s1 = arena.take(B, cout) if arena is not None else None
-        h = self.conv1(h, chan_bias=tb, stats=s1)
-        h = self.norm2(h, silu=True, stats=s1)
+        _, h = self.conv1(h, chan_bias=tb, stats=s1, gn=self.norm2.of(silu=True, keep_raw=False))
         if pair and self.conv_shortcut is None:
             sc = torch.cat(x, dim=-1)
         elif pair:
@@ -85,7 +90,10 @@
         else:
             sc = self.conv_shortcut(x) if self.conv_shortcut is not None else x
         s2 = arena.take(B, cout) if arena is not None else None
-        return self.conv2(h, residual=sc, stats=s2), s2
+        if next_gn is not None:
+            out, outn = self.conv2(h, residual=sc, stats=s2, gn=next_gn)
+            return out, s2, outn
+        return self.conv2(h, residual=sc, stats=s2), s2, None
 
 
 _LN_FOLD = os.environ.get("CASSMANTLE_LN_FOLD", "1") == "1"
@@ -164,16 +172,22 @@
             [BasicTransformerBlock(dim, heads, ctx_dim, gen, dtype) for _ in range(depth)])
         self.proj_out = Linear(dim, dim, gen=gen, dtype=dtype)
 
-    def forward(self, x, ctx, fp8=False, arena: Optional[StatsArena] = None, xs=None):
+    def _folds_norm(self, H, W, C, device, have_stats) -> bool:
+        return (_GN_FOLD and have_stats and C == 320 and (H * W) % 256 == 0 and device.type == "cuda"
+                and ops.get_mode() == "hip")
+
+    def input_gn(self, H, W, device, have_stats):
+        return None if self._folds_norm(H, W, self.proj_in.fin, device, have_stats) else self.norm.of()
+
+    def forward(self, x, ctx, fp8=False, arena: Optional[StatsArena] = None, xs=None, xn=None):
         B, H, W, C = x.shape
         hrs = None
-        if (_GN_FOLD and xs is not None and C == 320 and (H * W) % 256 == 0 and x.device.type == "cuda"
-                and ops.get_mode() == "hip"):
+        if xn is None and self._folds_norm(H, W, C, x.device, xs is not None):
             n = self.norm
             h = ops.gn_linear(x.view(B, H * W, C), xs, n.weight, n.bias, n.groups, n.eps, self.proj_in.weight,
                               self.proj_in.bias)
         else:
-            h = self.norm(x, stats=xs).view(B, H * W, C)
+            h = (xn if xn is not None else self.norm(x, stats=xs)).view(B, H * W, C)
             hrs = arena.take_rows(B * H * W) if (arena is not None and _LN_FOLD and _row_stats_wanted(h)) else None
             h = self.proj_in(h, row_stats=hrs)
         rs = hrs
@@ -189,9 +203,12 @@
         super().__init__()
         self.conv = Conv2d(c, c, 3, stride=2, padding=1, gen=gen, dtype=dtype)
 
-    def forward(self, x, arena: Optional[StatsArena] = None):
+    def forward(self, x, arena: Optional[StatsArena] = None, next_gn=None):
         so = arena.take(x.shape[0], self.conv.cout) if arena is not None else None
-        return self.conv(x, stats=so), so
+        if next_gn is not None:
+            y, yn = self.conv(x, stats=so, gn=next_gn)
+            return y, so, yn
+        return self.conv(x, stats=so), so, None
 
 
 class Upsample(nn.Module):
@@ -368,25 +385,36 @@
         hs = ar.take(B, self.conv_in.cout)
         h = self.conv_in(x, stats=hs)
         skips = [(h, hs)]
-        for blk in self.down:
+        tgn = lambda t, x: t.input_gn(x.shape[1], x.shape[2], x.device, ar.on)
+        hn = None
+        for bi, blk in enumerate(self.down):
+            nres = len(blk.resnets)
             for j, res in enumerate(blk.resnets):
-                h, hs = res(h, temb, tb, ar, hs)
                 if len(blk.attentions):
-                    h, hs = blk.attentions[j](h, ctx, fp8, ar, hs)
+                    nxt = tgn(blk.attentions[j], h)
+                elif j + 1 < nres:
+                    nxt = blk.resnets[j + 1].input_gn()
+                else:
+                    nxt = self.mid_res1.input_gn() if blk.downsampler is None else None
+                h, hs, hn = res(h, temb, tb, ar, hs, xn=hn, next_gn=nxt)
+                if len(blk.attentions):
+                    h, hs = blk.attentions[j](h, ctx, fp8, ar, hs, hn)
+                    hn = None
                 skips.append((h, hs))
             if blk.downsampler is not None:
-                h, hs = blk.downsampler(h, ar)
+                h, hs, hn = blk.downsampler(h, ar, self.down[bi + 1].resnets[0].input_gn())
                 skips.append((h, hs))
-        h, hs = self.mid_res1(h, temb, tb, ar, hs)
-        h, hs = self.mid_attn(h, ctx, fp8, ar, hs)
-        h, hs = self.mid_res2(h, temb, tb, ar, hs)
+        h, hs, hn = self.mid_res1(h, temb, tb, ar, hs, xn=hn, next_gn=tgn(self.mid_attn, h))
+        h, hs = self.mid_attn(h, ctx, fp8, ar, hs, hn)
+        h, hs, _ = self.mid_res2(h, temb, tb, ar, hs)
         for blk in self.up:
             for j, res in enumerate(blk.resnets):
                 sk, sks = skips.pop()
                 two = hs is not None and sks is not None
-                h, hs = res((h, sk), temb, tb, ar, hs if two else None, sks if two else None)
+                nxt = tgn(blk.attentions[j], h) if len(blk.attentions) else None
+                h, hs, hn = res((h, sk), temb, tb, ar, hs if two else None, sks if two else None, next_gn=nxt)
                 if len(blk.attentions):
-                    h, hs = blk.attentions[j](h, ctx, fp8, ar, hs)
+                    h, hs = blk.attentions[j](h, ctx, fp8, ar, hs, hn)
             if blk.upsampler is not None:
                 h, hs = blk.upsampler(h, ar)
         h = self.conv_norm_out(h, silu=True, stats=hs)
diff --git a/cassmantle_amd/ops/__init__.py b/cassmantle_amd/ops/__init__.py
--- a/cassmantle_amd/ops/__init__.py
+++ b/cassmantle_amd/ops/__init__.py
@@ -3,7 +3,7 @@
 import math
 import os
 import weakref
-from typing import List, Optional
+from typing import List, NamedTuple, Optional
 
 import torch
 
@@ -128,10 +128,29 @@
         channel_stats_ref(y, stats)
 
 
+class GroupNormOf(NamedTuple):
+    weight: torch.Tensor
+    bias: torch.Tensor
+    groups: int
+    eps: float
+    silu: bool = False
+    keep_raw: bool = True
+
+
+def _gn_of(y: torch.Tensor, gn: GroupNormOf, stats: Optional[torch.Tensor]):
+    yn = group_norm(y, gn.groups, gn.weight, gn.bias, gn.eps, gn.silu, stats=stats)
+    return (y if gn.keep_raw else None), yn
+
+
+def _gn_kw(gn: GroupNormOf, out: torch.Tensor) -> dict:
+    return dict(cgn_out=torch.empty_like(out), cgn_gamma=gn.weight, cgn_beta=gn.bias, cgn_groups=int(gn.groups),
+                cgn_eps=float(gn.eps), cgn_silu=int(gn.silu), cgn_keep_raw=int(gn.keep_raw))
+
+
 def linear(x: torch.Tensor, w: torch.Tensor, bias: Optional[torch.Tensor] = None,
            residual: Optional[torch.Tensor] = None, act: Optional[str] = None,
            stats: Optional[torch.Tensor] = None, out: Optional[torch.Tensor] = None,
-           row_stats: Optional[torch.Tensor] = None) -> torch.Tensor:
+           row_stats: Optional[torch.Tensor] = None, gn: Optional[GroupNormOf] = None):
     if not _use_hip(x):
         if x.device.type == "cuda":
             y = _torch_linear(x, w, bias, residual, act)
@@ -139,7 +158,10 @@
             y = ref.linear(x, w, bias, residual, act)
         if stats is not None:
             channel_stats_ref(y, stats)
-        return y if out is None else out.copy_(y)
+        y = y if out is None else out.copy_(y)
+        return y if gn is None else _gn_of(y, gn, stats)
+    if gn is not None and (stats is None or row_stats is not None or act in ("geglu", "swiglu")):
+        return _gn_of(linear(x, w, bias, residual, act, stats, out, row_stats), gn, stats)
     K = x.shape[-1]
     x2 = x.reshape(-1, K)
     if not x2.is_contiguous():
@@ -152,6 +174,10 @@
     o2 = out.view(x2.shape[0], N)
     r2 = residual.reshape(-1, N) if residual is not None else None
     hw = x2.shape[0] // x.shape[0] if stats is not None else 0
+    if gn is not None:
+        kw = _gn_kw(gn, out)
+        _launch(ext().gemm, x2, w, bias, r2, o2, _ACT[act], stats, hw, **kw)
+        return (out.view(*x.shape[:-1], N) if gn.keep_raw else None), kw["cgn_out"].view(*x.shape[:-1], N)
     if row_stats is not None:
         _launch(ext().gemm, x2, w, bias, r2, o2, _ACT[act], stats, hw, row_stats=row_stats)
     else:
@@ -290,7 +316,7 @@
 def conv2d(x: torch.Tensor, w: torch.Tensor, bias: Optional[torch.Tensor] = None, stride: int = 1,
            padding: int = 1, residual: Optional[torch.Tensor] = None, upsample: bool = False,
            chan_bias: Optional[torch.Tensor] = None, stats: Optional[torch.Tensor] = None,
-           out: Optional[torch.Tensor] = None) -> torch.Tensor:
+           out: Optional[torch.Tensor] = None, gn: Optional[GroupNormOf] = None):
     if not _use_hip(x):
         if x.device.type == "cuda":
             y = _torch_conv(x, w, bias, stride, padding, residual, upsample, chan_bias)
@@ -298,7 +324,10 @@
             y = ref.conv2d(x, w, bias, stride, padding, residual, upsample, chan_bias)
         if stats is not None:
             channel_stats_ref(y, stats)
-        return y if out is None else out.copy_(y)
+        y = y if out is None else out.copy_(y)
+        return y if gn is None else _gn_of(y, gn, stats)
+    if gn is not None and stats is None:
+        return _gn_of(conv2d(x, w, bias, stride, padding, residual, upsample, chan_bias, None, out), gn, None)
     B, H, W, Cin = x.shape
     Cout, kh, kw, _ = w.shape
     if Cin % 8 != 0:
@@ -313,6 +342,11 @@
         out = torch.empty((B, Ho, Wo, Cout), device=x.device, dtype=x.dtype)
     else:
         assert out.shape == (B, Ho, Wo, Cout) and out.dtype == x.dtype and out.is_contiguous(), "conv2d: bad out"
+    if gn is not None:
+        kw = _gn_kw(gn, out)
+        _launch(ext().conv2d, x.contiguous(), w, bias, residual, chan_bias, out, stride, padding, int(upsample), stats,
+                **kw)
+        return (out if gn.keep_raw else None), kw["cgn_out"]
     _launch(ext().conv2d, x.contiguous(), w, bias, residual, chan_bias, out, stride, padding, int(upsample), stats)
     return out
 
diff --git a/cassmantle_amd/ops/csrc/bindings.cpp b/cassmantle_amd/ops/csrc/bindings.cpp
--- a/cassmantle_amd/ops/csrc/bindings.cpp
+++ b/cassmantle_amd/ops/csrc/bindings.cpp
@@ -59,7 +59,39 @@
   g_raster[1].store((int)gated);
 }
 
-void run_gemm(GemmArgs& p, const at::Tensor& like) {
+int compute_units() {
+  static std::atomic<int> cus[64];
+  int dev = 0;
+  if (hipGetDevice(&dev) != hipSuccess || dev < 0 || dev >= 64) return 1 << 30;
+  int n = cus[dev].load(std::memory_order_relaxed);
+  if (n == 0) {
+    if (hipDeviceGetAttribute(&n, hipDeviceAttributeMultiprocessorCount, dev) != hipSuccess || n <= 0) n = 1 << 30;
+    cus[dev].store(n, std::memory_order_relaxed);
+  }
+  return n;
+}
+static std::atomic<long long> g_gn_reduce_calls{0};
+bool opt_gn_consumer(GnConsumer& g, const c10::optional<at::Tensor>& y, const c10::optional<at::Tensor>& gamma,
+                     const c10::optional<at::Tensor>& beta, int64_t groups, double eps, int64_t silu, int64_t keep_raw,
+                     const at::Tensor& out) {
+  if (!y.has_value() || !y->defined()) return false;
+  TORCH_CHECK(gamma.has_value() && beta.has_value() && groups > 0, "cgn_out needs cgn_gamma, cgn_beta and cgn_groups");
+  CHECK_DEV(*y); CHECK_BF16(*y); CHECK_CONTIG(*y); CHECK_BF16(out);
+  const int64_t C = out.size(-1);
+  TORCH_CHECK(y->numel() == out.numel() && y->data_ptr() != out.data_ptr(), "cgn_out: a second tensor shaped like out");
+  TORCH_CHECK(C % 8 == 0 && C % groups == 0, "cgn: the output channels must be a multiple of 8 and of the groups");
+  TORCH_CHECK(gamma->numel() == C && beta->numel() == C, "cgn: gamma / beta must have one value per output channel");
+  g.gamma = opt_bptr(gamma);
+  g.beta = opt_bptr(beta);
+  g.y = reinterpret_cast<uint16_t*>(y->data_ptr());
+  g.groups = (int)groups;
+  g.eps = (float)eps;
+  g.silu = (int)silu;
+  g.keep_raw = keep_raw != 0;
+  return true;
+}
+
+void run_gemm(GemmArgs& p, const at::Tensor& like, const GnConsumer* gn = nullptr) {
   raster_from_env();
   p.raster = g_raster[(p.act == 4 || p.act == 6) ? 1 : 0].load(std::memory_order_relaxed);
   TORCH_CHECK(p.stats == nullptr || (p.N % 8 == 0 && p.ldc == p.N),
@@ -73,6 +105,23 @@
     post_stats = p.stats;
     p.stats = nullptr;
   }
+  if (gn != nullptr) {
+    TORCH_CHECK((p.stats != nullptr || post_stats != nullptr) && p.stats_hw > 0 && !p.out_f32,
+                "cgn_out needs stats (the GroupNorm's statistics) and a bf16 output");
+    const char* e = getenv("CASSMANTLE_GN_REDUCE");
+    const int mode = e ? atoi(e) : 1;
+    const bool fills = mode == 2 || (long long)gn->groups * (p.M / p.stats_hw) >= compute_units();
+    const bool slabs = p.split > 1 && post_stats == nullptr && p.M > 8 && p.K % 8 == 0 && (!p.conv || p.Cin % 8 == 0) &&
+                       (p.conv || p.lda % 8 == 0) && p.ldw % 8 == 0;
+    if (mode != 0 && fills && slabs && splitk_reduce_gn_lds(p, *gn) > 0) {
+      auto ws = at::empty({(long long)p.split * p.M * p.N}, like.options().dtype(at::kFloat));
+      p.defer_reduce = true;
+      launch_gemm(p, ws.data_ptr<float>(), cur_stream());
+      launch_splitk_reduce_gn(p, *gn, ws.data_ptr<float>(), cur_stream());
+      g_gn_reduce_calls.fetch_add(1, std::memory_order_relaxed);
+      return;
+    }
+  }
   if (p.split > 1) {
     auto ws = at::empty({(long long)p.split * p.batch * p.M * p.N}, like.options().dtype(at::kFloat));
     launch_gemm(p, ws.data_ptr<float>(), cur_stream());
@@ -82,6 +131,10 @@
   if (post_stats != nullptr)
     launch_channel_stats(reinterpret_cast<const uint16_t*>(p.C), post_stats, p.M / p.stats_hw, p.stats_hw, p.N,
                          cur_stream());
+  if (gn != nullptr)
+    launch_group_norm_cs(reinterpret_cast<const uint16_t*>(p.C), nullptr, post_stats != nullptr ? post_stats : p.stats,
+                         p.N, nullptr, gn->gamma, gn->beta, gn->y, p.M / p.stats_hw, p.stats_hw, p.N, gn->groups,
+                         gn->eps, gn->silu, cur_stream());
 }
 
 void gemm(const at::Tensor& x, const at::Tensor& w, const c10::optional<at::Tensor>& bias,
@@ -91,7 +144,10 @@
           const c10::optional<at::Tensor>& kv8, int64_t kv8_col0, int64_t kv8_ntok, int64_t kv8_hk,
           const c10::optional<at::Tensor>& ln_rows_fx, const c10::optional<at::Tensor>& row_stats,
           const c10::optional<at::Tensor>& gn_stats, const c10::optional<at::Tensor>& gn_gamma,
-          const c10::optional<at::Tensor>& gn_beta, int64_t gn_groups, int64_t gn_hw, double gn_eps) {
+          const c10::optional<at::Tensor>& gn_beta, int64_t gn_groups, int64_t gn_hw, double gn_eps,
+          const c10::optional<at::Tensor>& cgn_out, const c10::optional<at::Tensor>& cgn_gamma,
+          const c10::optional<at::Tensor>& cgn_beta, int64_t cgn_groups, double cgn_eps, int64_t cgn_silu,
+          int64_t cgn_keep_raw) {
   CHECK_DEV(x); CHECK_BF16(x); CHECK_BF16(w); CHECK_CONTIG(w); CHECK_CONTIG(out);
   TORCH_CHECK(x.dim() == 2 && w.dim() == 2 && out.dim() == 2, "gemm: 2-D operands expected");
   TORCH_CHECK(x.stride(1) == 1, "gemm: x rows must be contiguous");
@@ -128,6 +184,15 @@
     TORCH_CHECK(stats_hw > 0 && p.M % stats_hw == 0, "gemm: stats_hw must divide the rows");
     p.stats_hw = (int)stats_hw;
     p.stats = opt_stats(stats, p.M / stats_hw, p.N);
+  }
+  GnConsumer cgn;
+  if (opt_gn_consumer(cgn, cgn_out, cgn_gamma, cgn_beta, cgn_groups, cgn_eps, cgn_silu, cgn_keep_raw, out)) {
+    TORCH_CHECK(p.stats != nullptr && p.row_stats == nullptr && p.kv8 == nullptr && act != 4 && act != 6 &&
+                    !(gn_stats.has_value() && gn_stats->defined()) && !(row_stats.has_value() && row_stats->defined()) &&
+                    !(ln_wsum.has_value() && ln_wsum->defined()),
+                "gemm: cgn_out needs stats and excludes gated acts, LayerNorm / GroupNorm folds, row statistics and kv8");
+    run_gemm(p, out, &cgn);
+    return;
   }
   if (gn_stats.has_value() && gn_stats->defined()) {
     TORCH_CHECK(gn_gamma.has_value() && gn_beta.has_value() && gn_groups > 0 && gn_hw > 0 && p.M % gn_hw == 0,
@@ -263,7 +328,10 @@
 
 void conv2d(const at::Tensor& x, const at::Tensor& w, const c10::optional<at::Tensor>& bias,
             const c10::optional<at::Tensor>& residual, const c10::optional<at::Tensor>& chan_bias, at::Tensor& out,
-            int64_t stride, int64_t pad, int64_t upsample, const c10::optional<at::Tensor>& stats) {
+            int64_t stride, int64_t pad, int64_t upsample, const c10::optional<at::Tensor>& stats,
+            const c10::optional<at::Tensor>& cgn_out, const c10::optional<at::Tensor>& cgn_gamma,
+            const c10::optional<at::Tensor>& cgn_beta, int64_t cgn_groups, double cgn_eps, int64_t cgn_silu,
+            int64_t cgn_keep_raw) {
   CHECK_DEV(x); CHECK_BF16(x); CHECK_CONTIG(x); CHECK_BF16(w); CHECK_CONTIG(w); CHECK_CONTIG(out); CHECK_BF16(out);
   TORCH_CHECK(x.dim() == 4 && w.dim() == 4 && out.dim() == 4, "conv2d: NHWC 4-D tensors expected");
   GemmArgs p;
@@ -292,7 +360,10 @@
   p.C = out.data_ptr();
   p.stats_hw = p.Ho * p.Wo;
   p.stats = opt_stats(stats, x.size(0), p.N);
-  run_gemm(p, out);
+  GnConsumer cgn;
+  const bool has = opt_gn_consumer(cgn, cgn_out, cgn_gamma, cgn_beta, cgn_groups, cgn_eps, cgn_silu, cgn_keep_raw, out);
+  TORCH_CHECK(!has || p.stats != nullptr, "conv2d: cgn_out needs stats");
+  run_gemm(p, out, has ? &cgn : nullptr);
 }
 
 void conv2d_up2(const at::Tensor& x, const at::Tensor& w4, const c10::optional<at::Tensor>& bias,
@@ -1075,7 +1146,9 @@
         py::arg("ln_wsum") = py::none(), py::arg("ln_eps") = 0.0, py::arg("kv8") = py::none(),
         py::arg("kv8_col0") = 0, py::arg("kv8_ntok") = 0, py::arg("kv8_hk") = 0, py::arg("ln_rows_fx") = py::none(),
         py::arg("row_stats") = py::none(), py::arg("gn_stats") = py::none(), py::arg("gn_gamma") = py::none(),
-        py::arg("gn_beta") = py::none(), py::arg("gn_groups") = 0, py::arg("gn_hw") = 0, py::arg("gn_eps") = 0.0, nogil());
+        py::arg("gn_beta") = py::none(), py::arg("gn_groups") = 0, py::arg("gn_hw") = 0, py::arg("gn_eps") = 0.0,
+        py::arg("cgn_out") = py::none(), py::arg("cgn_gamma") = py::none(), py::arg("cgn_beta") = py::none(),
+        py::arg("cgn_groups") = 0, py::arg("cgn_eps") = 0.0, py::arg("cgn_silu") = 0, py::arg("cgn_keep_raw") = 0, nogil());
   m.def("row_stats", &row_stats, nogil());
   m.def("gemm_cat", &gemm_cat, nogil());
   m.def("group_norm_cat", &group_norm_cat, nogil());
@@ -1094,8 +1167,12 @@
   m.def("gemm_record_keys", [](bool on) { gemm_record_keys(on); });
   m.def("gemm_last_key", []() { return gemm_last_key(); });
   m.def("gemm_last_plan", []() { int c, sp; gemm_last_plan(&c, &sp); return std::vector<int64_t>{c, sp}; });
+  m.def("gn_reduce_calls", []() { return (int64_t)g_gn_reduce_calls.load(); });
   m.def("gemm_rms", &gemm_rms, nogil());
-  m.def("conv2d", &conv2d, nogil());
+  m.def("conv2d", &conv2d, py::arg("x"), py::arg("w"), py::arg("bias"), py::arg("residual"), py::arg("chan_bias"),
+        py::arg("out"), py::arg("stride"), py::arg("pad"), py::arg("upsample"), py::arg("stats"),
+        py::arg("cgn_out") = py::none(), py::arg("cgn_gamma") = py::none(), py::arg("cgn_beta") = py::none(),
+        py::arg("cgn_groups") = 0, py::arg("cgn_eps") = 0.0, py::arg("cgn_silu") = 0, py::arg("cgn_keep_raw") = 0, nogil());
   m.def("conv2d_up2", &conv2d_up2, nogil());
   m.def("bmm_nt", &bmm_nt, nogil());
   m.def("group_norm", &group_norm, nogil());
diff --git a/cassmantle_amd/ops/csrc/common.h b/cassmantle_amd/ops/csrc/common.h
--- a/cassmantle_amd/ops/csrc/common.h
+++ b/cassmantle_amd/ops/csrc/common.h
@@ -121,6 +121,22 @@
   return (double)v * (which ? (1.0 / STAT_SCALE_SQ) : (1.0 / STAT_SCALE_SUM));
 }
 
+CM_DEVICE float2 gn_mean_rstd(long long si, long long qi, double n, float eps) {
+  const double sm = stat_decode(si, 0), q = stat_decode(qi, 1);
+  const double mean = sm / n;
+  double var = q / n - mean * mean;
+  if (var < 0) var = 0;
+  return make_float2((float)mean, (float)(1.0 / sqrt(var + (double)eps)));
+}
+CM_DEVICE void gn_scale_shift(float gamma, float beta, float mean, float rstd, float& sc, float& sf) {
+  sc = gamma * rstd;
+  sf = beta - mean * sc;
+}
+CM_DEVICE float gn_norm(float f, float sc, float sf, int silu) {
+  const float o = fmaf(f, sc, sf);
+  return silu ? silu_f(o) : o;
+}
+
 enum Act { ACT_NONE = 0, ACT_GELU = 1, ACT_SILU = 2, ACT_QUICK_GELU = 3, ACT_GEGLU = 4, ACT_GELU_TANH = 5,
            ACT_SWIGLU = 6 };
 
diff --git a/cassmantle_amd/ops/csrc/gemm_impl.h b/cassmantle_amd/ops/csrc/gemm_impl.h
--- a/cassmantle_amd/ops/csrc/gemm_impl.h
+++ b/cassmantle_amd/ops/csrc/gemm_impl.h
@@ -89,7 +89,7 @@
   return ((long long)img * 2 * p.Ho + 2 * i + (z >> 1)) * (2 * p.Wo) + 2 * j + (z & 1);
 }
 
-template <bool OUTF32>
+template <bool OUTF32, bool STORE = true>
 CM_DEVICE void epilogue4(const GemmArgs& p, int batch, int m, int n, float* o) {
   const int hw = p.Ho * p.Wo;
   const int bimg = (p.chan_bias != nullptr) ? (m / hw) : 0;
@@ -107,6 +107,7 @@
       for (int r = 0; r < 4; ++r) o[r] = apply_act(o[r], p.act);
     }
     if (p.residual) add4(o, *reinterpret_cast<const uint2*>(p.residual + om * p.ldc + n));
+    if constexpr (!STORE) return;
     if (!OUTF32 && kv8_store4(p, m, n, o)) return;
     if constexpr (OUTF32) {
       float* C = reinterpret_cast<float*>(p.C) + (long long)batch * p.sC + om * p.ldc + n;
@@ -882,13 +883,19 @@
   }
 }
 
+inline int splitk_stats_rows(const GemmArgs& p) {
+  static const int adapt = [] { const char* e = getenv("CASSMANTLE_SK_ADAPT"); return e ? atoi(e) : 1; }();
+  const long long cols = (p.N / 4 + SK_QB - 1) / SK_QB;
+  int rb = SK_RB;
+  while (adapt && rb > SK_RL && cols * ((p.M + rb - 1) / rb) * p.batch < 512) rb /= 2;
+  return rb;
+}
+
 template <bool OUTF32>
 void launch_splitk_reduce(const GemmArgs& p, float* ws, int split, hipStream_t s) {
   if (p.stats != nullptr) {
-    static const int adapt = [] { const char* e = getenv("CASSMANTLE_SK_ADAPT"); return e ? atoi(e) : 1; }();
     const long long cols = (p.N / 4 + SK_QB - 1) / SK_QB;
-    int rb = SK_RB;
-    while (adapt && rb > SK_RL && cols * ((p.M + rb - 1) / rb) * p.batch < 512) rb /= 2;
+    const int rb = splitk_stats_rows(p);
     dim3 g2((unsigned)cols, (unsigned)((p.M + rb - 1) / rb), (unsigned)p.batch);
     hipLaunchKernelGGL(splitk_reduce_stats_kernel<OUTF32>, g2, dim3(256), 0, s, p, ws, split, rb);
   } else {
@@ -917,7 +924,7 @@
     (void)once;
   }
   hipLaunchKernelGGL(kfn, grid, dim3(64 * (WM * WN + NP)), lds, s, p, ws);
-  if (split > 1) launch_splitk_reduce<OUTF32>(p, ws, split, s);
+  if (split > 1 && !p.defer_reduce) launch_splitk_reduce<OUTF32>(p, ws, split, s);
 }
 
 template <int I, int CONV, bool GEGLU, bool OUTF32, bool BUF>
diff --git a/cassmantle_amd/ops/csrc/gemm_pp.h b/cassmantle_amd/ops/csrc/gemm_pp.h
--- a/cassmantle_amd/ops/csrc/gemm_pp.h
+++ b/cassmantle_amd/ops/csrc/gemm_pp.h
@@ -480,7 +480,7 @@
   }();
   (void)once;
   hipLaunchKernelGGL(kfn, grid, dim3(512), lds, s, p, ws);
-  if (split > 1) launch_splitk_reduce<false>(p, ws, split, s);
+  if (split > 1 && !p.defer_reduce) launch_splitk_reduce<false>(p, ws, split, s);
 }
 
 template <int I, int CONV, bool GEGLU>
diff --git a/cassmantle_amd/ops/csrc/kernels.h b/cassmantle_amd/ops/csrc/kernels.h
--- a/cassmantle_amd/ops/csrc/kernels.h
+++ b/cassmantle_amd/ops/csrc/kernels.h
@@ -18,6 +18,7 @@
   int act = 0;
   int out_f32 = 0;
   int split = 1;
+  bool defer_reduce = false;
   int cfg = 0;
   int raster = 0;
   int conv = 0, IH = 0, IW = 0, Cin = 0, Ho = 0, Wo = 0, stride = 1, pad = 0, ksize = 1, upsample = 0;
@@ -55,6 +56,18 @@
 std::string gemm_last_key();
 void gemm_last_plan(int* cfg, int* split);
 void launch_gemm(const GemmArgs& p, float* ws, hipStream_t s);
+
+struct GnConsumer {
+  const uint16_t* gamma = nullptr;
+  const uint16_t* beta = nullptr;
+  uint16_t* y = nullptr;
+  int groups = 0;
+  float eps = 0.f;
+  int silu = 0;
+  bool keep_raw = false;
+};
+size_t splitk_reduce_gn_lds(const GemmArgs& p, const GnConsumer& g);
+void launch_splitk_reduce_gn(const GemmArgs& p, const GnConsumer& g, const float* ws, hipStream_t s);
 
 struct AttnArgs {
   const uint16_t* q; const uint16_t* k; const uint16_t* v; uint16_t* o;
diff --git a/cassmantle_amd/ops/csrc/norm.hip b/cassmantle_amd/ops/csrc/norm.hip
--- a/cassmantle_amd/ops/csrc/norm.hip
+++ b/cassmantle_amd/ops/csrc/norm.hip
@@ -278,13 +278,9 @@
       qi += __shfl_xor(qi, o, 64);
     }
     if (g < G && sub == 0) {
-      const double sm = stat_decode(si, 0), q = stat_decode(qi, 1);
-      const double n = (double)S * Cg;
-      const double mean = sm / n;
-      double var = q / n - mean * mean;
-      if (var < 0) var = 0;
-      gst[2 * g] = (float)mean;
-      gst[2 * g + 1] = (float)(1.0 / sqrt(var + (double)eps));
+      const float2 ms = gn_mean_rstd(si, qi, (double)S * Cg, eps);
+      gst[2 * g] = ms.x;
+      gst[2 * g + 1] = ms.y;
     }
   }
   __syncthreads();
@@ -299,18 +295,14 @@
 #pragma unroll
     for (int i = 0; i < 8; ++i) {
       const int g = von[j] ? (v * 8 + i) / Cg : 0;
-      sc[j][i] = ga[i] * gst[2 * g + 1];
-      sf[j][i] = be[i] - gst[2 * g] * sc[j][i];
+      gn_scale_shift(ga[i], be[i], gst[2 * g], gst[2 * g + 1], sc[j][i], sf[j][i]);
     }
   }
   auto emit = [&](long long rr, int j, uint4 w) {
     float f[8];
     unpack8(w, f);
 #pragma unroll
-    for (int i = 0; i < 8; ++i) {
-      const float o = fmaf(f[i], sc[j][i], sf[j][i]);
-      f[i] = silu ? silu_f(o) : o;
-    }
+    for (int i = 0; i < 8; ++i) f[i] = gn_norm(f[i], sc[j][i], sf[j][i], silu);
 #if GN_NT_STORE
     typedef __attribute__((ext_vector_type(4))) unsigned int u32x4_nt;
     const uint4 pk = pack8(f);
diff --git a/cassmantle_amd/ops/csrc/splitk_gn.hip b/cassmantle_amd/ops/csrc/splitk_gn.hip
--- /dev/null
+++ b/cassmantle_amd/ops/csrc/splitk_gn.hip
@@ -0,0 +1,208 @@
+#include <algorithm>
+
+#include "gemm_impl.h"
+
+namespace {
+
+constexpr int GN_RL = SK_RL;
+constexpr size_t GN_LDS_MAX = 65536;
+
+struct GnLds {
+  size_t red, scsf, xs, total;
+};
+__host__ __device__ inline GnLds gn_lds(int S, int Cg, int cp) {
+  GnLds l;
+  l.red = (size_t)16 * Cg;
+  l.scsf = l.red + (size_t)2 * cp * GN_RL * Cg * 4;
+  l.xs = l.scsf + (size_t)8 * Cg;
+  l.total = l.xs + (((size_t)2 * S * Cg + 15) & ~(size_t)15);
+  return l;
+}
+
+constexpr int GN_MAX_THREADS = 768;
+
+template <bool KEEP>
+__global__ void __launch_bounds__(GN_MAX_THREADS) splitk_reduce_gn_kernel(GemmArgs p, GnConsumer gc,
+                                                                 const float* __restrict__ partial, int split, int rb,
+                                                                 int cp) {
+  extern __shared__ __attribute__((aligned(16))) unsigned char gn_smem[];
+  const int S = p.stats_hw, Cg = p.N / gc.groups, quads = Cg / 4;
+  const int lin = xcd_remap(blockIdx.x, gridDim.x);
+  const int g = lin % gc.groups, b = lin / gc.groups;
+  const int tid = threadIdx.x, nthr = blockDim.x;
+  const GnLds l = gn_lds(S, Cg, cp);
+  long long* acc = reinterpret_cast<long long*>(gn_smem);
+  float* red = reinterpret_cast<float*>(gn_smem + l.red);
+  float* scsf = reinterpret_cast<float*>(gn_smem + l.scsf);
+  uint16_t* xs = reinterpret_cast<uint16_t*>(gn_smem + l.xs);
+  const int c0 = g * Cg;
+  const uint16_t gam = tid < Cg ? gc.gamma[c0 + tid] : (uint16_t)0, bet = tid < Cg ? gc.beta[c0 + tid] : (uint16_t)0;
+  for (int c = tid; c < 2 * Cg; c += nthr) acc[c] = 0;
+  const long long slab = (long long)p.M * p.N;
+  const int nch = S / rb;
+  for (int ch0 = 0; ch0 < nch; ch0 += cp) {
+    const int ncp = min(cp, nch - ch0);
+    for (int w = tid; w < ncp * GN_RL * quads; w += nthr) {
+      const int qd = w % quads, rl = (w / quads) % GN_RL, cl = w / (quads * GN_RL);
+      const int n = c0 + qd * 4;
+      const int r0 = (ch0 + cl) * rb;
+      float s4[4] = {0.f, 0.f, 0.f, 0.f}, q4[4] = {0.f, 0.f, 0.f, 0.f};
+      auto finish = [&](int r, float* o) {
+        epilogue4<false, KEEP>(p, 0, b * S + r, n, o);
+        *reinterpret_cast<uint2*>(xs + (long long)r * Cg + qd * 4) = make_uint2(pack2(o[0], o[1]), pack2(o[2], o[3]));
+#pragma unroll
+        for (int e = 0; e < 4; ++e) {
+          const float f = bf2f(f2bf(o[e]));
+          s4[e] += f;
+          q4[e] = fmaf(f, f, q4[e]);
+        }
+      };
+      int r = r0 + rl;
+      for (; r + GN_RL < r0 + rb; r += 2 * GN_RL) {
+        float oa[4] = {0.f, 0.f, 0.f, 0.f}, ob[4] = {0.f, 0.f, 0.f, 0.f};
+        const float* sa = partial + (long long)(b * S + r) * p.N + n;
+        const float* sb = sa + (long long)GN_RL * p.N;
+        int sl = 0;
+        for (; sl + 4 <= split; sl += 4) {
+          const float4 a0 = *reinterpret_cast<const float4*>(sa + (sl + 0) * slab);
+          const float4 a1 = *reinterpret_cast<const float4*>(sa + (sl + 1) * slab);
+          const float4 a2 = *reinterpret_cast<const float4*>(sa + (sl + 2) * slab);
+          const float4 a3 = *reinterpret_cast<const float4*>(sa + (sl + 3) * slab);
+          const float4 b0 = *reinterpret_cast<const float4*>(sb + (sl + 0) * slab);
+          const float4 b1 = *reinterpret_cast<const float4*>(sb + (sl + 1) * slab);
+          const float4 b2 = *reinterpret_cast<const float4*>(sb + (sl + 2) * slab);
+          const float4 b3 = *reinterpret_cast<const float4*>(sb + (sl + 3) * slab);
+          oa[0] += (a0.x + a1.x) + (a2.x + a3.x);
+          oa[1] += (a0.y + a1.y) + (a2.y + a3.y);
+          oa[2] += (a0.z + a1.z) + (a2.z + a3.z);
+          oa[3] += (a0.w + a1.w) + (a2.w + a3.w);
+          ob[0] += (b0.x + b1.x) + (b2.x + b3.x);
+          ob[1] += (b0.y + b1.y) + (b2.y + b3.y);
+          ob[2] += (b0.z + b1.z) + (b2.z + b3.z);
+          ob[3] += (b0.w + b1.w) + (b2.w + b3.w);
+        }
+        for (; sl < split; ++sl) {
+          const float4 va = *reinterpret_cast<const float4*>(sa + sl * slab);
+          const float4 vb = *reinterpret_cast<const float4*>(sb + sl * slab);
+          oa[0] += va.x; oa[1] += va.y; oa[2] += va.z; oa[3] += va.w;
+          ob[0] += vb.x; ob[1] += vb.y; ob[2] += vb.z; ob[3] += vb.w;
+        }
+        finish(r, oa);
+        finish(r + GN_RL, ob);
+      }
+      for (; r < r0 + rb; r += GN_RL) {
+        float o[4] = {0.f, 0.f, 0.f, 0.f};
+        const float* src = partial + (long long)(b * S + r) * p.N + n;
+        int sl = 0;
+        for (; sl + 4 <= split; sl += 4) {
+          const float4 v0 = *reinterpret_cast<const float4*>(src + (sl + 0) * slab);
+          const float4 v1 = *reinterpret_cast<const float4*>(src + (sl + 1) * slab);
+          const float4 v2 = *reinterpret_cast<const float4*>(src + (sl + 2) * slab);
+          const float4 v3 = *reinterpret_cast<const float4*>(src + (sl + 3) * slab);
+          o[0] += (v0.x + v1.x) + (v2.x + v3.x);
+          o[1] += (v0.y + v1.y) + (v2.y + v3.y);
+          o[2] += (v0.z + v1.z) + (v2.z + v3.z);
+          o[3] += (v0.w + v1.w) + (v2.w + v3.w);
+        }
+        for (; sl < split; ++sl) {
+          const float4 v = *reinterpret_cast<const float4*>(src + sl * slab);
+          o[0] += v.x; o[1] += v.y; o[2] += v.z; o[3] += v.w;
+        }
+        finish(r, o);
+      }
+#pragma unroll
+      for (int e = 0; e < 4; ++e) {
+        red[((0 * cp + cl) * GN_RL + rl) * Cg + qd * 4 + e] = s4[e];
+        red[((1 * cp + cl) * GN_RL + rl) * Cg + qd * 4 + e] = q4[e];
+      }
+    }
+    if (ch0 == 0 && tid < Cg) {
+      scsf[tid] = bf2f(gam);
+      scsf[Cg + tid] = bf2f(bet);
+    }
+    __syncthreads();
+    for (int u = tid; u < 2 * ncp * Cg; u += nthr) {
+      const int col = u % Cg, cl = (u / Cg) % ncp, st = u / (Cg * ncp);
+      float a = 0.f;
+#pragma unroll
+      for (int r = 0; r < GN_RL; ++r) a += red[((st * cp + cl) * GN_RL + r) * Cg + col];
+      stat_atomic_add(acc + st * Cg + col, st, a);
+    }
+    __syncthreads();
+  }
+  if (tid < 64) {
+    long long si = 0, qi = 0;
+    for (int c = tid; c < Cg; c += 64) {
+      si += acc[c];
+      qi += acc[Cg + c];
+    }
+#pragma unroll
+    for (int o = 32; o > 0; o >>= 1) {
+      si += __shfl_xor(si, o, 64);
+      qi += __shfl_xor(qi, o, 64);
+    }
+    const float2 ms = gn_mean_rstd(si, qi, (double)S * Cg, gc.eps);
+    for (int c = tid; c < Cg; c += 64) {
+      float sc, sf;
+      gn_scale_shift(scsf[c], scsf[Cg + c], ms.x, ms.y, sc, sf);
+      scsf[c] = sc;
+      scsf[Cg + c] = sf;
+    }
+  } else if (KEEP) {
+    for (int u = tid - 64; u < 2 * Cg; u += nthr - 64) {
+      const int st = u / Cg, col = u % Cg;
+      atomicAdd(reinterpret_cast<unsigned long long*>(p.stats + ((long long)b * p.N + c0 + col) * 2 + st),
+                (unsigned long long)acc[u]);
+    }
+  }
+  __syncthreads();
+  uint16_t* yb = gc.y + (long long)b * S * p.N + c0;
+  for (int u = tid; u < S * quads; u += nthr) {
+    const int r = u / quads, qd = u % quads;
+    const uint2 v = *reinterpret_cast<const uint2*>(xs + (long long)r * Cg + qd * 4);
+    const float4 sc = *reinterpret_cast<const float4*>(scsf + qd * 4);
+    const float4 sf = *reinterpret_cast<const float4*>(scsf + Cg + qd * 4);
+    const float f0 = gn_norm(bf2f(v.x & 0xffff), sc.x, sf.x, gc.silu);
+    const float f1 = gn_norm(bf2f(v.x >> 16), sc.y, sf.y, gc.silu);
+    const float f2 = gn_norm(bf2f(v.y & 0xffff), sc.z, sf.z, gc.silu);
+    const float f3 = gn_norm(bf2f(v.y >> 16), sc.w, sf.w, gc.silu);
+    *reinterpret_cast<uint2*>(yb + (long long)r * p.N + qd * 4) = make_uint2(pack2(f0, f1), pack2(f2, f3));
+  }
+}
+
+int gn_chunks_per_pass(int S, int Cg, int nch) {
+  const size_t fixed = gn_lds(S, Cg, 0).total;
+  if (fixed >= GN_LDS_MAX) return 0;
+  int cp = (int)std::min((size_t)nch, (GN_LDS_MAX - fixed) / ((size_t)2 * GN_RL * Cg * 4));
+  if (cp < 1) return 0;
+  const int passes = (nch + cp - 1) / cp;
+  return (nch + passes - 1) / passes;
+}
+
+}
+
+size_t splitk_reduce_gn_lds(const GemmArgs& p, const GnConsumer& g) {
+  if (p.split <= 1 || g.groups <= 0 || p.N % g.groups != 0 || p.N % 8 != 0 || p.ldc != p.N) return 0;
+  const int Cg = p.N / g.groups, S = p.stats_hw;
+  if (Cg % 4 != 0 || Cg > 256 || S <= 0 || p.M % S != 0) return 0;
+  if (p.batch != 1 || p.parity || p.out_f32 || is_gated(p.act) || p.row_stats != nullptr || p.kv8 != nullptr) return 0;
+  if ((p.ldcb ? p.ldcb : p.N) % 4 != 0) return 0;
+  const int rb = splitk_stats_rows(p);
+  if (S % rb != 0) return 0;
+  const int cp = gn_chunks_per_pass(S, Cg, S / rb);
+  return cp > 0 ? gn_lds(S, Cg, cp).total : 0;
+}
+
+void launch_splitk_reduce_gn(const GemmArgs& p, const GnConsumer& g, const float* ws, hipStream_t s) {
+  const int Cg = p.N / g.groups, S = p.stats_hw;
+  const int rb = splitk_stats_rows(p);
+  const int cp = gn_chunks_per_pass(S, Cg, S / rb);
+  const int items = cp * GN_RL * (Cg / 4);
+  const int threads = std::min(GN_MAX_THREADS, std::max(256, (items + 63) / 64 * 64));
+  const dim3 grid((unsigned)(g.groups * (p.M / S)));
+  const size_t lds = gn_lds(S, Cg, cp).total;
+  if (g.keep_raw)
+    hipLaunchKernelGGL(splitk_reduce_gn_kernel<true>, grid, dim3(threads), lds, s, p, g, ws, p.split, rb, cp);
+  else
+    hipLaunchKernelGGL(splitk_reduce_gn_kernel<false>, grid, dim3(threads), lds, s, p, g, ws, p.split, rb, cp);
+}
```

After: 7.869 images/s (median of 6 runs). Within noise of the previous version (+1.0%).
